# ParaGroup/WindFlow

Measured on AMD Instinct MI355X. Metric: tuples_per_sec, higher is better.
Workload: dtype bf16; 1 GPU; model=keyed_ffat_cb_window, global_batch=16777216, win=1000, slide=100, keys_per_rank=8192, parallelism=keyed-dp1, dense_keys=True

## Files before the change

csrc/engine/bindings.cpp:

```cpp
#include <pybind11/functional.h>
#include <pybind11/numpy.h>
#include <pybind11/pybind11.h>
#include <pybind11/stl.h>

#include "engine.hpp"

namespace py = pybind11;
using namespace wfa;

static py::array col_view(DType dt, void* data, int64_t n) {
    switch (dt) {
        case DType::I64: return py::array_t<int64_t>({n}, {8}, (int64_t*)data, py::none());
        case DType::F64: return py::array_t<double>({n}, {8}, (double*)data, py::none());
        case DType::F32: return py::array_t<float>({n}, {4}, (float*)data, py::none());
        case DType::U64: return py::array_t<uint64_t>({n}, {8}, (uint64_t*)data, py::none());
        case DType::I32: return py::array_t<int32_t>({n}, {4}, (int32_t*)data, py::none());
        case DType::U16: return py::array_t<uint16_t>({n}, {2}, (uint16_t*)data, py::none());
        case DType::U8: return py::array_t<uint8_t>({n}, {1}, (uint8_t*)data, py::none());
    }
    throw std::runtime_error("bad dtype");
}

static py::dict batch_views(Batch* b, RuntimeCtx* ctx = nullptr) {
    py::dict d;
// ... 439 lines not shown
        .value("I64", DType::I64)
        .value("F64", DType::F64)
        .value("F32", DType::F32)
        .value("U64", DType::U64)
        .value("I32", DType::I32)
        .value("U16", DType::U16)
        .value("U8", DType::U8);

    m.def("rccl_unique_id",
          [] { return py::bytes(wfa_rccl_unique_id()); },
          "ncclUniqueId bytes for Engine.set_dist (call on rank 0, broadcast)");

    py::class_<Engine>(m, "Engine")
        .def(py::init<>())
        .def_readwrite("mode", &Engine::mode)
        .def_readwrite("time_policy", &Engine::time_policy)
        .def_readwrite("queue_capacity", &Engine::queue_capacity)
        .def_readwrite("pin_threads", &Engine::pin_threads)
        .def("set_dist",
             [](Engine& e, int rank, int world, py::bytes id) {
                 e.dist_rank = rank;
                 e.dist_world = world;
                 e.rccl_id = std::string(id);
             },
             py::arg("rank"), py::arg("world"), py::arg("rccl_id"))
        .def("add_op",
             [](Engine& e, const std::string& name, int par, const std::string& kind,
                const std::string& spec, std::vector<double> fp, std::vector<int64_t> ip,
                std::vector<int> out_schema, int64_t out_batch, py::object pyfn,
                int device) {
                 OpSpec op;
                 op.id = (int)e.ops.size();
                 op.name = name;
                 op.parallelism = par;
                 op.device = device;
                 int id = op.id;
                 op.stages.push_back(make_stage(e, id, kind, spec, fp, ip, out_schema,
                                                out_batch, pyfn, device));
                 e.ops.push_back(std::move(op));
                 return id;
             },
             py::arg("name"), py::arg("parallelism"), py::arg("kind"), py::arg("spec") = "",
             py::arg("fparams") = std::vector<double>{}, py::arg("iparams") = std::vector<int64_t>{},
             py::arg("out_schema") = std::vector<int>{}, py::arg("out_batch") = 1024,
             py::arg("pyfn") = py::none(), py::arg("device") = -1)
        .def("chain_stage",
             [](Engine& e, int op_id, const std::string& kind, const std::string& spec,
                std::vector<double> fp, std::vector<int64_t> ip, std::vector<int> out_schema,
                int64_t out_batch, py::object pyfn) {
                 e.ops.at(op_id).stages.push_back(
                     make_stage(e, op_id, kind, spec, fp, ip, out_schema, out_batch, pyfn,
                                e.ops.at(op_id).device));
             },
             py::arg("op_id"), py::arg("kind"), py::arg("spec") = "",
             py::arg("fparams") = std::vector<double>{}, py::arg("iparams") = std::vector<int64_t>{},
             py::arg("out_schema") = std::vector<int>{}, py::arg("out_batch") = 1024,
             py::arg("pyfn") = py::none())
        .def("add_edge",
             [](Engine& e, int from, int to, Routing r, CollectorKind ck, int tag) {
                 e.edges.push_back(EdgeSpec{from, to, r, ck, tag});
             },
             py::arg("from_op"), py::arg("to_op"), py::arg("routing") = Routing::FORWARD,
             py::arg("collector") = CollectorKind::WATERMARK, py::arg("stream_tag") = -1)
        .def("run",
             [](Engine& e) {
                 e.build();
                 {
                     py::gil_scoped_release rel;
                     e.start();
                     e.wait();
                 }
             })
        .def("start",
             [](Engine& e) {
                 e.build();
                 e.start();
             })
        .def("start_gated",
             [](Engine& e) {
                 e.build();
                 {
                     py::gil_scoped_release rel;
                     e.start_gated();
                 }
             })
        .def("open_gate_and_wait",
             [](Engine& e) {
                 py::gil_scoped_release rel;
                 e.open_gate();
                 e.wait();
             })
        .def("wait",
             [](Engine& e) {
                 py::gil_scoped_release rel;
                 e.wait();
             })
        .def("abort_now", [](Engine& e) { e.abort.store(true); })
        .def("sink_sum", [](Engine& e, int op) { return e.sink_acc_i64.at(op).load(); })
        .def("sink_sum_f",
             [](Engine& e, int op) {
                 std::lock_guard<std::mutex> g(e.sink_f64_mu);
                 auto it = e.sink_acc_f64.find(op);
                 return it == e.sink_acc_f64.end() ? 0.0 : it->second;
             })
        .def("sink_count", [](Engine& e, int op) { return e.sink_tuples.at(op).load(); })
        .def("dropped", [](Engine& e) { return e.dropped_tuples.load(); })
        .def("sink_latencies",
             [](Engine& e, int op) {
                 auto it = e.sink_latencies.find(op);
                 return it == e.sink_latencies.end() ? std::vector<int64_t>{}
                                                     : it->second;
             })
        .def("stats", [](Engine& e) {
            py::list out;
            for (auto& r : e.replicas) {
                py::dict d;
                d["op"] = r->op_id;
                d["name"] = e.ops[r->op_id].name;
                d["replica"] = r->idx;
                d["inputs"] = r->stats.inputs_received;
                d["tuples_in"] = r->stats.tuples_received;
                d["outputs"] = r->stats.outputs_sent;
                d["tuples_out"] = r->stats.tuples_sent;
                d["svc_us_ewma"] = r->stats.service_time_us_ewma;
                d["start_us"] = r->stats.start_us;
                d["end_us"] = r->stats.end_us;
                d["kernels"] = r->stats.num_kernels;
                d["bytes_h2d"] = r->stats.bytes_h2d;
                d["bytes_d2h"] = r->stats.bytes_d2h;
                out.append(d);
            }
            return out;
        });

    m.def("hash_key", [](uint64_t k) { return KeyByEmitter::mix(k); });

#ifdef WFA_WITH_HIP
    m.def("debug_jit_fold_source",
          [](const std::string& kind, const std::string& spec,
             const std::vector<double>& fp, const std::vector<int64_t>& ip) {
              return debug_jit_fold_source(kind, spec, fp, ip);
          });
    m.def("debug_sort_pairs",
          [](py::array_t<uint32_t> keys, int bits) {
              auto r = debug_sort_pairs_host(keys.data(), keys.shape(0), bits);
              py::array_t<uint32_t> ks((py::ssize_t)r.first.size());
              py::array_t<uint32_t> vs((py::ssize_t)r.second.size());
              memcpy(ks.mutable_data(), r.first.data(), 4 * r.first.size());
              memcpy(vs.mutable_data(), r.second.data(), 4 * r.second.size());
              return py::make_tuple(ks, vs);
          });
    m.def("debug_ffat_stage_times",
          [](int64_t n, int64_t n_keys, int64_t win, int64_t slide, int iters,
             int vik, const std::string& fold_variant) {
              py::dict d;
              for (auto& [k, v] : debug_ffat_stage_times(n, n_keys, win, slide,
                                                         iters, vik, fold_variant))
                  d[py::str(k)] = v;
              return d;
          },
          py::arg("n"), py::arg("n_keys"), py::arg("win") = 1000,
          py::arg("slide") = 100, py::arg("iters") = 20, py::arg("vik") = 0,
          py::arg("fold_variant") = "");
    m.def("debug_tb_stage_times",
          [](int64_t n, int64_t n_keys, int iters, int mono) {
              std::map<std::string, double> m2;
              for (auto& kv : debug_tb_stage_times(n, n_keys, iters, mono))
                  m2[kv.first] = kv.second;
              return m2;
          },
          py::arg("n"), py::arg("n_keys"), py::arg("iters") = 20,
          py::arg("mono") = 1);
    m.def("debug_gram_stage_times",
          [](int64_t n, int64_t n_keys, int64_t win, int iters) {
              std::map<std::string, double> m2;
              for (auto& kv : debug_gram_stage_times(n, n_keys, win, iters))
                  m2[kv.first] = kv.second;
              return m2;
          },
          py::arg("n"), py::arg("n_keys"), py::arg("win") = 32,
          py::arg("iters") = 20);
    m.def("debug_a2a_stage_times",
          [](int64_t n, int64_t n_keys, int iters) {
              py::list out;
              for (auto& [k, v] : debug_a2a_stage_times(n, n_keys, iters))
                  out.append(py::make_tuple(k, v));
              return out;
          },
          py::arg("n"), py::arg("n_keys") = 8192, py::arg("iters") = 20);
    m.def("debug_key_slots",
          [](py::array_t<uint64_t> keys, int64_t max_keys) {
              auto r = debug_key_slots_host(keys.data(), keys.shape(0), max_keys);
              py::array_t<uint32_t> s((py::ssize_t)r.size());
              memcpy(s.mutable_data(), r.data(), 4 * r.size());
              return s;
          });
#endif

    struct StateStore {
        std::shared_ptr<void> holder;
        void* kv = nullptr;
        void* cache = nullptr;
    };
    py::class_<StateStore>(m, "StateStore")
        .def(py::init([](const std::string& path, int64_t cache_cap, bool fresh) {
                 auto s = new StateStore();
                 s->holder =
                     open_state_store(path, cache_cap, &s->kv, &s->cache, fresh);
                 return s;
             }),
             py::arg("path"), py::arg("cache_capacity") = 1 << 16,
             py::arg("fresh") = true)
        .def("erase",
             [](StateStore& s, uint64_t key) {
                 return state_kv_erase(s.kv, s.cache, key);
             })
        .def("get",
             [](StateStore& s, uint64_t key) -> py::object {
                 std::string* v = state_cache_get(s.cache, key);
                 if (!v) return py::none();
                 return py::bytes(*v);
             })
        .def("put",
             [](StateStore& s, uint64_t key, py::bytes val) {
                 state_cache_put(s.cache, key, std::string(val));
             })
        .def("flush", [](StateStore& s) { state_cache_flush(s.cache); })
        .def("__len__", [](StateStore& s) { return state_kv_size(s.kv); });
}
```

csrc/engine/engine.hpp:

```cpp
#pragma once

#include <chrono>
#include <deque>
#include <functional>
#include <thread>
#include <unordered_map>

#include "core.hpp"
#include "queue.hpp"

namespace wfa {

struct Engine;
struct Replica;

inline int64_t now_us() {
    return std::chrono::duration_cast<std::chrono::microseconds>(
               std::chrono::steady_clock::now().time_since_epoch())
        .count();
}

struct StatsRecord {
    int64_t inputs_received = 0;
    int64_t tuples_received = 0;
// ... 243 lines not shown
struct OpSpec {
    int id = 0;
    std::string name;
    int parallelism = 1;
    std::vector<StageSpec> stages;
    int device = -1;
    bool pinned_out = false;
    const StageSpec& last() const { return stages.back(); }
};

struct ChainLogic : OpLogic {
    struct StageEmitter;
    std::vector<std::shared_ptr<OpLogic>> stages;
    std::vector<EmitCtx> ctxs;
    std::vector<std::unique_ptr<Emitter>> glue;
    void wire(const std::vector<Pool*>& pools, EmitCtx& final_ctx, RuntimeCtx& rctx);
    bool is_source() const override { return stages.front()->is_source(); }
    bool accepts_device() const override { return stages.front()->accepts_device(); }
    bool source_step(EmitCtx&, RuntimeCtx& ctx) override {
        return stages.front()->source_step(ctxs[0], ctx);
    }
    void process(Batch* in, EmitCtx&, RuntimeCtx& ctx) override {
        stages.front()->process(in, ctxs[0], ctx);
    }
    bool on_punct(int64_t wm, EmitCtx&, RuntimeCtx& ctx) override;
    void on_eos(EmitCtx&, RuntimeCtx& ctx) override;
    void warm(RuntimeCtx& ctx) override;
    void post_eos() override {
        for (auto& st : stages) st->post_eos();
    }
};

struct EdgeSpec {
    int from = 0, to = 0;
    Routing routing = Routing::FORWARD;
    CollectorKind collector = CollectorKind::WATERMARK;
    int stream_tag = -1;
};

struct Replica {
    Engine* engine = nullptr;
    int op_id = 0;
    int idx = 0;
    std::shared_ptr<OpLogic> logic;
    std::unique_ptr<Collector> collector;
    std::vector<std::unique_ptr<Emitter>> emitters;
    EmitCtx ectx;
    RuntimeCtx rctx;
    StatsRecord stats;
    std::thread th;
    void run();
};

struct Engine {
    ExecMode mode = ExecMode::DEFAULT;
    TimePolicy time_policy = TimePolicy::EVENT_TIME;
    std::vector<OpSpec> ops;
    std::vector<EdgeSpec> edges;

    std::vector<std::unique_ptr<Replica>> replicas;
    std::vector<std::unique_ptr<Pool>> pools;
    std::vector<std::unique_ptr<SpscQueue>> queues;
    std::atomic<bool> abort{false};
    std::atomic<int64_t> dropped_tuples{0};
    std::mutex error_mu;
    std::string first_error;
    std::atomic<int> gate{0};
    std::atomic<int> warmed{0};
    bool use_gate = false;
    std::unordered_map<int, std::atomic<int64_t>> sink_acc_i64;
    std::unordered_map<int, double> sink_acc_f64;
    std::mutex sink_f64_mu;
    std::unordered_map<int, std::atomic<int64_t>> sink_tuples;
    std::unordered_map<int, std::vector<int64_t>> sink_latencies;
    int64_t queue_capacity = 128;
    bool pin_threads = false;
    int dist_rank = 0;
    int dist_world = 1;
    std::string rccl_id;

    Pool* make_pool(const Schema& s, int64_t cap, bool pinned) {
        pools.push_back(std::make_unique<Pool>(s, cap, pinned));
        return pools.back().get();
    }

    void build();
    void start();
    void wait();
    void run() { build(); start(); wait(); }
    void start_gated();
    void open_gate() { gate.store(1, std::memory_order_release); }
};

std::shared_ptr<OpLogic> make_native_logic(const std::string& kind,
                                           const std::string& spec,
                                           const std::vector<double>& fparams,
                                           const std::vector<int64_t>& iparams,
                                           Engine* eng, int op_id);

struct WinRows {
    int64_t n = 0;
    const int64_t* ts = nullptr;
    uint64_t key = 0;
    int64_t gwid = 0;
    const Schema* schema = nullptr;
    std::vector<const char*> cols;
};
using WindowFn = std::function<double(const WinRows&)>;

struct JoinPairs {
    int64_t n = 0;
    const uint64_t* key = nullptr;
    const int64_t* ts_a = nullptr;
    const int64_t* ts_b = nullptr;
    const double* va = nullptr;
    const double* vb = nullptr;
};
using JoinFn =
    std::function<void(const JoinPairs&, uint8_t* keep, double* out)>;

std::shared_ptr<OpLogic> make_window_logic(const std::string& kind,
                                           const std::vector<double>& fp,
                                           const std::vector<int64_t>& ip,
                                           Engine* eng, int op_id,
                                           WindowFn userfn = nullptr,
                                           JoinFn joinfn = nullptr);

std::shared_ptr<OpLogic> make_gpu_logic(const std::string& kind, const std::string& spec,
                                        const std::vector<double>& fp,
                                        const std::vector<int64_t>& ip, Engine* eng,
                                        int op_id, int device, const Schema& os,
                                        int64_t out_batch);

std::shared_ptr<OpLogic> make_persist_logic(const std::string& kind,
                                            const std::string& spec,
                                            const std::vector<double>& fp,
                                            const std::vector<int64_t>& ip,
                                            Engine* eng, int op_id);
std::shared_ptr<void> open_state_store(const std::string& path, int64_t cache_cap,
                                       void** kv_out, void** cache_out,
                                       bool fresh = true);
std::string* state_cache_get(void* cache, uint64_t key);
void state_cache_put(void* cache, uint64_t key, const std::string& v);
void state_cache_flush(void* cache);
int64_t state_kv_size(void* kv);
bool state_kv_erase(void* kv, void* cache, uint64_t key);

std::pair<std::vector<uint32_t>, std::vector<uint32_t>> debug_sort_pairs_host(
    const uint32_t* keys, int64_t n, int bits);
std::vector<uint32_t> debug_key_slots_host(const uint64_t* keys, int64_t n,
                                           int64_t max_keys);
std::vector<std::pair<std::string, double>> debug_ffat_stage_times(
    int64_t n, int64_t n_keys, int64_t win, int64_t slide, int iters, int vik,
    const std::string& fold_variant = "");
std::vector<std::pair<std::string, double>> debug_gram_stage_times(
    int64_t n, int64_t n_keys, int64_t win, int iters);
std::vector<std::pair<std::string, double>> debug_tb_stage_times(
    int64_t n, int64_t n_keys, int iters, int mono);
std::vector<std::pair<std::string, double>> debug_a2a_stage_times(
    int64_t n, int64_t n_keys, int iters);

std::string wfa_rccl_unique_id();

std::string debug_jit_fold_source(const std::string& kind,
                                  const std::string& spec,
                                  const std::vector<double>& fp,
                                  const std::vector<int64_t>& ip);

}
```

csrc/engine/gpu_common.hpp:

```cpp
#pragma once
#ifdef WFA_WITH_HIP

#include <hip/hip_runtime.h>
#include <hip/hiprtc.h>

#include <map>
#include <mutex>
#include <set>
#include <string>
#include <vector>

#include "engine.hpp"

namespace wfa {

#define HIPCHK(x)                                                                  \
    do {                                                                           \
        hipError_t err_ = (x);                                                     \
        if (err_ != hipSuccess)                                                    \
            throw std::runtime_error(std::string("HIP error: ") +                  \
                                     hipGetErrorString(err_) + " at " #x);         \
    } while (0)

#define RTCCHK(x)                                                              \
    do {                                                                       \
        hiprtcResult r_ = (x);                                                 \
        if (r_ != HIPRTC_SUCCESS)                                              \
            throw std::runtime_error(std::string("hiprtc error: ") +           \
                                     hiprtcGetErrorString(r_) + " at " #x);    \
    } while (0)

struct DeviceArena {
    std::mutex mu;
    std::map<size_t, std::vector<void*>> free_by_size;
    int device;
    size_t allocated = 0;

    void* get(size_t bytes) {
        bytes = (bytes + 255) & ~size_t(255);
        {
            std::lock_guard<std::mutex> g(mu);
            auto it = free_by_size.find(bytes);
            if (it != free_by_size.end() && !it->second.empty()) {
                void* p = it->second.back();
                it->second.pop_back();
                return p;
            }
        }
        void* p = nullptr;
        HIPCHK(hipSetDevice(device));
        HIPCHK(hipMalloc(&p, bytes));
        if (getenv("WFA_DEBUG_SYNC"))
            fprintf(stderr, "[alloc] %p..%p (%zu)\n", p, (char*)p + bytes,
                    bytes);
        std::lock_guard<std::mutex> g(mu);
        allocated += bytes;
        return p;
    }
    void put(void* p, size_t bytes) {
        bytes = (bytes + 255) & ~size_t(255);
        std::lock_guard<std::mutex> g(mu);
        free_by_size[bytes].push_back(p);
    }
};

inline DeviceArena g_arena[64];

inline DeviceArena& arena(int dev) {
    g_arena[dev].device = dev;
    return g_arena[dev];
}

inline bool wfa_prof() {
    static int v = -1;
    if (v < 0) v = getenv("WFA_PROF") ? 1 : 0;
    return v;
}

inline bool wfa_debug_sync() {
    static int v = -1;
    if (v < 0) v = getenv("WFA_DEBUG_SYNC") ? 1 : 0;
    return v;
}

inline void dbg_sync(hipStream_t s, const char* where) {
    if (!wfa_debug_sync()) return;
    hipError_t e = hipStreamSynchronize(s);
    hipError_t e2 = hipGetLastError();
    fprintf(stderr, "[dbgsync] %s sync=%s last=%s\n", where,
            hipGetErrorString(e), hipGetErrorString(e2));
    fflush(stderr);
}

struct GpuLogicBase : OpLogic {
    int64_t prof_host_us = 0, prof_calls = 0;
    int device = 0;
    hipStream_t stream = nullptr;
    std::unique_ptr<Pool> dev_pool;
    Schema out_schema;
    int64_t out_cap = 1 << 20;
    bool inited = false;

    virtual void init_device() {}
    void ensure_init() {
        if (inited) return;
        HIPCHK(hipSetDevice(device));
        HIPCHK(hipStreamCreateWithFlags(&stream, hipStreamNonBlocking));
        dev_pool = std::make_unique<Pool>(out_schema, out_cap, false);
        dev_pool->loc = Loc::DEVICE;
        dev_pool->device = device;
        init_device();
        inited = true;
    }
    void post_eos() override { drain_h2d(true); }
    ~GpuLogicBase() override {
        h2d_inflight.clear();
        if (stream) (void)hipStreamDestroy(stream);
    }

    void warm(RuntimeCtx&) override { ensure_init(); }
    bool accepts_device() const override { return true; }

    void wait_ready(Batch* b) {
        if (b->loc == Loc::DEVICE && b->ready_event)
            HIPCHK(hipStreamWaitEvent(stream, (hipEvent_t)b->ready_event, 0));
    }
    void record_ready(Batch* b) {
        b->stream = stream;
        HIPCHK(hipEventRecord((hipEvent_t)b->ready_event, stream));
    }

    void release_after_use(Batch* b) {
        if (b->loc == Loc::DEVICE && b->ready_event &&
            b->refcnt.load(std::memory_order_acquire) == 1)
            HIPCHK(hipEventRecord((hipEvent_t)b->ready_event, stream));
        release(b);
    }

    Batch* get_from(Pool& pool) {
        constexpr int MAX_DEPTH = 8;
        Batch* chosen = nullptr;
        Batch* skipped[MAX_DEPTH];
        int nskip = 0;
        while (nskip < MAX_DEPTH) {
            Batch* b = pool.try_pop();
            if (!b) break;
            if (!b->ready_event ||
                hipEventQuery((hipEvent_t)b->ready_event) == hipSuccess) {
                chosen = b;
                break;
            }
            skipped[nskip++] = b;
        }
        for (int i = 0; i < nskip; ++i) pool.put(skipped[i]);
        if (!chosen) {
            if (nskip > 0 && pool.live.load(std::memory_order_relaxed) >= MAX_DEPTH)
                chosen = pool.get();
            else
                chosen = pool.make_new();
        }
        if (chosen->ready_event)
            HIPCHK(hipStreamWaitEvent(stream, (hipEvent_t)chosen->ready_event, 0));
        return chosen;
    }

    Batch* get_dev() { return get_from(*dev_pool); }

    std::unique_ptr<Pool> in_pool;
    std::vector<std::unique_ptr<Pool>> retired_in_pools;

    Batch* get_in(const Batch* src) {
        if (!in_pool || in_pool->schema.payload != src->schema.payload ||
            in_pool->capacity < src->count) {
            if (in_pool) retired_in_pools.push_back(std::move(in_pool));
            in_pool = std::make_unique<Pool>(
                src->schema, std::max({out_cap, src->capacity, src->count}),
                false);
            in_pool->loc = Loc::DEVICE;
            in_pool->device = device;
        }
        return get_from(*in_pool);
    }

    std::deque<std::pair<Batch*, hipEvent_t>> h2d_inflight;

    void drain_h2d(bool block) {
        while (!h2d_inflight.empty()) {
            auto [old_hb, ev] = h2d_inflight.front();
            if (!block && hipEventQuery(ev) != hipSuccess) break;
            if (block) HIPCHK(hipEventSynchronize(ev));
            release(old_hb);
            h2d_inflight.pop_front();
        }
    }

    Batch* to_device(Batch* hb, RuntimeCtx& ctx) {
        drain_h2d(false);
        Batch* db = get_in(hb);
        int64_t n = hb->count;
        HIPCHK(hipMemcpyAsync(db->ts, hb->ts, 8 * n, hipMemcpyHostToDevice, stream));
        HIPCHK(hipMemcpyAsync(db->key, hb->key, 8 * n, hipMemcpyHostToDevice, stream));
        size_t bytes = 16 * n;
        for (size_t c = 0; c < hb->cols.size() && c < db->cols.size(); ++c) {
            size_t es = dsize(hb->schema.payload[c]);
            HIPCHK(hipMemcpyAsync(db->cols[c], hb->cols[c], es * n,
                                  hipMemcpyHostToDevice, stream));
            bytes += es * n;
        }
        db->count = n;
        db->watermark = ctx.current_wm;
        db->stream_tag = ctx.current_tag;
        db->ts_mono = hb->ts_mono;
        if (ctx.stats) ctx.stats->bytes_h2d += bytes;
        HIPCHK(hipEventRecord((hipEvent_t)db->ready_event, stream));
        h2d_inflight.push_back({hb, (hipEvent_t)db->ready_event});
        if (h2d_inflight.size() > 4) drain_h2d(true);
        return db;
    }

    Batch* input_on_device(Batch* b, RuntimeCtx& ctx) {
        if (b->loc == Loc::HOST) return to_device(b, ctx);
        gpu_resolve_count(b);
        if (b->device != device || force_peer_copy())
            return peer_copy(b, ctx);
        wait_ready(b);
        return b;
    }

    static bool force_peer_copy() {
        static int v = -1;
        if (v < 0) {
            const char* e = getenv("WFA_FORCE_PEER_COPY");
            v = (e && e[0] == '1') ? 1 : 0;
        }
        return v;
    }

    Batch* peer_copy(Batch* b, RuntimeCtx& ctx) {
        drain_h2d(false);
        enable_peer(device, b->device);
        wait_ready(b);
        Batch* db = get_in(b);
        const int64_t n = b->count;
        HIPCHK(hipMemcpyPeerAsync(db->ts, device, b->ts, b->device, 8 * n,
                                  stream));
        HIPCHK(hipMemcpyPeerAsync(db->key, device, b->key, b->device, 8 * n,
                                  stream));
        size_t bytes = 16 * n;
        for (size_t c = 0; c < b->cols.size() && c < db->cols.size(); ++c) {
            size_t es = dsize(b->schema.payload[c]);
            HIPCHK(hipMemcpyPeerAsync(db->cols[c], device, b->cols[c],
                                      b->device, es * n, stream));
            bytes += es * n;
        }
        db->count = n;
        db->watermark = b->watermark;
        db->stream_tag = b->stream_tag;
        db->born_us = b->born_us;
        if (ctx.stats) ctx.stats->bytes_d2h += bytes;
        HIPCHK(hipEventRecord((hipEvent_t)db->ready_event, stream));
        h2d_inflight.push_back({b, (hipEvent_t)db->ready_event});
        if (h2d_inflight.size() > 4) drain_h2d(true);
        return db;
    }

    static void enable_peer(int dst, int src) {
        if (dst == src) return;
        static std::mutex mu;
        static std::set<std::pair<int, int>> done;
        std::lock_guard<std::mutex> g(mu);
        if (!done.insert({dst, src}).second) return;
        int can = 0;
        if (hipDeviceCanAccessPeer(&can, dst, src) == hipSuccess && can) {
            HIPCHK(hipSetDevice(dst));
            hipError_t e = hipDeviceEnablePeerAccess(src, 0);
            if (e != hipSuccess && e != hipErrorPeerAccessAlreadyEnabled)
                (void)hipGetLastError();
        }
    }
};

struct KeyedScratch {
    uint64_t* tab = nullptr;
    uint32_t* d_nslots = nullptr;
    uint64_t* slot_to_key = nullptr;
    uint32_t *slot = nullptr, *idx = nullptr, *slot_t = nullptr, *idx_t = nullptr;
    uint32_t* hist = nullptr;
    uint32_t *seg_start = nullptr, *seg_slot = nullptr;
    int64_t* d_nseg = nullptr;
    float* v_sorted = nullptr;
    float* v_f32 = nullptr;
    int64_t table_cap = 0;
    int64_t max_keys = 0;
    int64_t cap = 0;
    int bits = 20;
    bool dense = false;
    uint32_t* d_overflow = nullptr;
    uint32_t* by_slot = nullptr;

    void alloc(int dev, int64_t cap_, int64_t mk, hipStream_t s);
    void check_dense_overflow();
    void segs(hipStream_t s, const uint32_t* slot_sorted, int64_t n, int shr);

    uint32_t* idx_sorted = nullptr;
    const void* v_as_f32 = nullptr;
    int v_dt = 2;

    void group(hipStream_t s, Batch* db, int vcol, RuntimeCtx& ctx,
               bool want_vik = false, bool want_carry = false);
};

hipModule_t jit_module(const std::string& src, int device);
hipFunction_t jit_fn(hipModule_t mod, const char* name);
std::string jit_type(DType d);

std::shared_ptr<OpLogic> make_gpu_jit_logic(const std::string& kind,
                                            const std::string& spec,
                                            const std::vector<double>& fp,
                                            const std::vector<int64_t>& ip,
                                            Engine* eng, int op_id, int device,
                                            const Schema& os, int64_t out_batch);

}

#endif
```

csrc/engine/gpu_ops.cpp:

```cpp
#include <cstring>
#include <deque>
#include <map>
#include <tuple>

#include "engine.hpp"

#ifdef WFA_WITH_HIP
#include <rccl/rccl.h>

#include "../hip/wfa_kernels.h"
#include "gpu_common.hpp"

namespace wfa {

struct AuxPool {
    std::mutex mu;
    std::vector<std::pair<void*, int64_t*>> free_list;
    std::pair<void*, int64_t*> get(int device) {
        {
            std::lock_guard<std::mutex> g(mu);
            if (!free_list.empty()) {
                auto p = free_list.back();
                free_list.pop_back();
                return p;
// ... 78 lines not shown
    c->watermark = b->watermark;
    c->stream_tag = b->stream_tag;
    c->born_us = b->born_us;
    c->ts_mono = b->ts_mono;
    c->stream = s;
    HIPCHK(hipEventRecord((hipEvent_t)c->ready_event, s));
    return c;
}

struct GpuSourceLogic : GpuLogicBase {
    int64_t len, n_keys, bsz;
    int vdt;
    uint64_t seed;
    int64_t pos = 0;
    GpuSourceLogic(int64_t l, int64_t k, int64_t b, int v, uint64_t sd, int dev,
                   Schema os) {
        len = l; n_keys = k; bsz = b; vdt = v; seed = sd;
        device = dev;
        out_schema = os;
        out_cap = b;
    }
    bool is_source() const override { return true; }
    bool source_step(EmitCtx& out, RuntimeCtx& ctx) override {
        int64_t t0 = now_us();
        ensure_init();
        if (pos >= len) return false;
        Batch* db = get_dev();
        int64_t tg = now_us() - t0;
        if (wfa_prof() && tg > 50)
            fprintf(stderr, "[prof] source get_dev wait %ld us\n", (long)tg);
        int64_t n = std::min<int64_t>(bsz, len - pos);
        wfa_gen_batch(stream, db->ts, db->key, db->cols[0], vdt, n, pos, seed, n_keys);
        dbg_sync(stream, "gen");
        db->count = n;
        db->ts_mono = true;
        db->born_us = now_us();
        pos += n;
        db->watermark = pos - 1;
        record_ready(db);
        if (ctx.stats) ctx.stats->num_kernels++;
        out.emit(db);
        return pos < len;
    }
};

struct GpuMapLogic : GpuLogicBase {
    int spec, col;
    double a, b;
    GpuMapLogic(int sp, int c, double a_, double b_, int dev, Schema os) {
        spec = sp; col = c; a = a_; b = b_;
        device = dev;
        out_schema = os;
    }
    void process(Batch* in, EmitCtx& out, RuntimeCtx& ctx) override {
        ensure_init();
        Batch* db = input_on_device(in, ctx);
        wfa_map_apply(stream, spec, db->cols[col], (int)db->schema.payload[col],
                      db->count, a, b);
        record_ready(db);
        if (ctx.stats) ctx.stats->num_kernels++;
        out.emit(db);
    }
};

struct GpuFilterLogic : GpuLogicBase {
    int spec, col;
    double a, b;
    uint32_t* d_flags = nullptr;
    uint32_t* d_scan = nullptr;
    int64_t* d_cnt = nullptr;
    void** d_colptrs = nullptr;
    int* d_esize = nullptr;
    GpuFilterLogic(int sp, int c, double a_, double b_, int dev, Schema os,
                   int64_t cap) {
        spec = sp; col = c; a = a_; b = b_;
        device = dev;
        out_schema = os;
        out_cap = cap;
    }
    void init_device() override {
        d_flags = (uint32_t*)arena(device).get(4 * out_cap);
        d_scan = (uint32_t*)arena(device).get(4 * (out_cap / 2048 + 2));
        d_cnt = (int64_t*)arena(device).get(64);
        size_t nc = out_schema.payload.size();
        d_colptrs = (void**)arena(device).get(16 * (nc + 1));
        d_esize = (int*)arena(device).get(4 * (nc + 1));
        std::vector<int> es;
        for (auto d : out_schema.payload) es.push_back((int)dsize(d));
        HIPCHK(hipMemcpy(d_esize, es.data(), 4 * nc, hipMemcpyHostToDevice));
    }
    void process(Batch* in, EmitCtx& out, RuntimeCtx& ctx) override {
        ensure_init();
        Batch* db = input_on_device(in, ctx);
        int64_t n = db->count;
        if (n > out_cap)
            throw std::runtime_error("filter input batch > out_batch capacity");
        Batch* ob = get_dev();
        wfa_filter_flags(stream, spec, db->cols[col], (int)db->schema.payload[col], n,
                         a, b, d_flags);
        size_t nc = db->cols.size();
        std::vector<void*> ptrs(2 * nc);
        for (size_t c = 0; c < nc; ++c) {
            ptrs[c] = db->cols[c];
            ptrs[nc + c] = ob->cols[c];
        }
        HIPCHK(hipMemcpyAsync(d_colptrs, ptrs.data(), 8 * 2 * nc,
                              hipMemcpyHostToDevice, stream));
        wfa_compact(stream, n, d_flags, d_scan, db->ts, ob->ts, db->key, ob->key,
                    (const void* const*)d_colptrs, (void* const*)(d_colptrs + nc),
                    d_esize, (int)nc, d_cnt);
        HIPCHK(hipMemcpyAsync(ob->lazy_count, d_cnt, 8, hipMemcpyDeviceToHost, stream));
        ob->count = -1;
        ob->watermark = db->watermark;
        ob->stream_tag = db->stream_tag;
        ob->born_us = db->born_us;
        ob->ts_mono = db->ts_mono;
        if (ctx.stats) ctx.stats->num_kernels += 3;
        release_after_use(db);
        record_ready(ob);
        out.emit(ob);
    }
};

void KeyedScratch::alloc(int dev, int64_t cap_, int64_t mk, hipStream_t s) {
    cap = cap_;
    max_keys = mk;
    table_cap = 1;
    while (table_cap < 2 * mk) table_cap <<= 1;
    bits = 1;
    while ((1ll << bits) < mk + 1) ++bits;
    if (bits < 5) bits = 5;
    auto& A = arena(dev);
    tab = (uint64_t*)A.get(16 * table_cap);
    d_nslots = (uint32_t*)A.get(64);
    slot_to_key = (uint64_t*)A.get(8 * mk);
    slot = (uint32_t*)A.get(4 * cap);
    idx = (uint32_t*)A.get(4 * cap);
    slot_t = (uint32_t*)A.get(4 * cap);
    idx_t = (uint32_t*)A.get(4 * cap);
    hist = (uint32_t*)A.get(4 * wfa_sort_hist_u32(cap));
    seg_start = (uint32_t*)A.get(4 * cap);
    seg_slot = (uint32_t*)A.get(4 * cap);
    d_nseg = (int64_t*)A.get(64);
    v_sorted = (float*)A.get(4 * cap);
    v_f32 = (float*)A.get(4 * cap);
    wfa_fill_u64(s, tab, ~0ULL, 2 * table_cap);
    wfa_fill_u32(s, d_nslots, 0, 1);
    if (dense) {
        d_overflow = (uint32_t*)A.get(64);
        wfa_fill_u32(s, d_overflow, 0, 1);
        wfa_iota_u64(s, slot_to_key, mk);
    }
    if (max_keys <= 65536) by_slot = (uint32_t*)A.get(4 * table_cap);
}

void KeyedScratch::segs(hipStream_t s, const uint32_t* slot_sorted, int64_t n,
                        int shr) {
    if (by_slot)
        wfa_segments_dense(s, slot_sorted, n, by_slot, table_cap, hist,
                           seg_start, seg_slot, d_nseg, shr);
    else
        wfa_segments(s, slot_sorted, n, hist, seg_start, seg_slot, d_nseg, shr);
}

void KeyedScratch::check_dense_overflow() {
    if (!dense) return;
    uint32_t ovf = 0;
    HIPCHK(hipMemcpy(&ovf, d_overflow, 4, hipMemcpyDeviceToHost));
    if (ovf)
        throw std::runtime_error(
            "withDenseKeys: a key >= max_keys arrived — dense mode requires "
            "integer keys in [0, max_keys); use the default hashed mode");
}

void KeyedScratch::group(hipStream_t s, Batch* db, int vcol, RuntimeCtx& ctx,
                         bool want_vik, bool want_carry) {
        int64_t n = db->count;
        if (n > cap)
            throw std::runtime_error("batch larger than keyed scratch capacity — "
                                     "set the GPU op's out_batch >= upstream batch");
        bool vik = want_vik && vcol >= 0 && max_keys <= 65535 &&
                   (int)db->schema.payload[vcol] == 5;
        if (vik) {
            uint32_t *os, *oi;
            if (dense) {
                wfa_key_dense_h(s, db->key, n, max_keys, slot, d_nslots,
                                d_overflow, (const uint16_t*)db->cols[vcol],
                                hist, 16);
                wfa_sort_pairs2_ph(s, slot, idx, slot_t, idx_t, nullptr,
                                   nullptr, hist, n, bits, &os, &oi, nullptr,
                                   1, 16);
            } else {
                wfa_key_to_slot_h(s, db->key, n, tab, d_nslots, table_cap, slot,
                                  slot_to_key, (const uint16_t*)db->cols[vcol],
                                  hist, 16);
                wfa_sort_pairs2_ph(s, slot, idx, slot_t, idx_t, nullptr,
                                   nullptr, hist, n, bits, &os, &oi, nullptr,
                                   1, 16);
            }
            idx_sorted = oi;
            v_as_f32 = os;
            v_dt = 6;
            segs(s, os, n, 16);
            if (ctx.stats) ctx.stats->num_kernels += 5 + 3 * ((bits + 3) / 4);
            return;
        }
        if (dense)
            wfa_key_dense_h(s, db->key, n, max_keys, slot, d_nslots, d_overflow,
                            nullptr, hist, 0);
        else
            wfa_key_to_slot_h(s, db->key, n, tab, d_nslots, table_cap, slot,
                              slot_to_key, nullptr, hist, 0);
        dbg_sync(s, "key_to_slot");
        if (want_carry && vcol >= 0 && (int)db->schema.payload[vcol] == 2) {
            wfa_cast(s, db->cols[vcol], 2, v_f32, 2, n);
            uint32_t *os, *oi, *ov;
            wfa_sort_pairs2_ph(s, slot, idx, slot_t, idx_t, (uint32_t*)v_f32,
                               (uint32_t*)v_sorted, hist, n, bits, &os, &oi,
                               &ov, 1, 0);
            idx_sorted = oi;
            v_as_f32 = ov;
            v_dt = 7;
            segs(s, os, n, 0);
            if (ctx.stats) ctx.stats->num_kernels += 6 + 3 * ((bits + 3) / 4);
            return;
        }
        uint32_t *os, *oi;
        wfa_sort_pairs2_ph(s, slot, idx, slot_t, idx_t, nullptr, nullptr,
                           hist, n, bits, &os, &oi, nullptr,
                           1, 0);
        idx_sorted = oi;
        if (vcol >= 0) {
            int vdt = (int)db->schema.payload[vcol];
            if (vdt == 2 || vdt == 5) {
                v_as_f32 = db->cols[vcol];
                v_dt = vdt;
            } else {
                wfa_cast(s, db->cols[vcol], vdt, v_f32, 2, n);
                v_as_f32 = v_f32;
                v_dt = 2;
            }
        }
        dbg_sync(s, "sort");
        segs(s, os, n, 0);
        dbg_sync(s, "segments");
        if (ctx.stats) ctx.stats->num_kernels += 5 + 3 * ((bits + 3) / 4);
}

hipModule_t jit_module(const std::string& src, int device) {
    static std::mutex mu;
    static std::map<std::string, hipModule_t> cache;
    std::lock_guard<std::mutex> g(mu);
    auto it = cache.find(src);
    if (it != cache.end()) return it->second;
    hiprtcProgram prog;
    RTCCHK(hiprtcCreateProgram(&prog, src.c_str(), "wfa_jit.hip", 0, nullptr,
                               nullptr));
    hipDeviceProp_t props;
    HIPCHK(hipGetDeviceProperties(&props, device));
    std::string arch = std::string("--offload-arch=") + props.gcnArchName;
    const char* opts[] = {arch.c_str(), "-O3"};
    hiprtcResult cr = hiprtcCompileProgram(prog, 2, opts);
    if (cr != HIPRTC_SUCCESS) {
        size_t lsz = 0;
        hiprtcGetProgramLogSize(prog, &lsz);
        std::string log(lsz, '\0');
        hiprtcGetProgramLog(prog, log.data());
        hiprtcDestroyProgram(&prog);
        throw std::runtime_error("JIT device logic failed to compile:\n" + log);
    }
    size_t csz = 0;
    RTCCHK(hiprtcGetCodeSize(prog, &csz));
    std::vector<char> code(csz);
    RTCCHK(hiprtcGetCode(prog, code.data()));
    hiprtcDestroyProgram(&prog);
    hipModule_t mod;
    HIPCHK(hipModuleLoadData(&mod, code.data()));
    cache[src] = mod;
    return mod;
}

hipFunction_t jit_fn(hipModule_t mod, const char* name) {
    hipFunction_t fn;
    HIPCHK(hipModuleGetFunction(&fn, mod, name));
    return fn;
}

std::string jit_type(DType d) {
    switch (d) {
        case DType::I64: return "long long";
        case DType::F64: return "double";
        case DType::F32: return "float";
        case DType::U64: return "unsigned long long";
        case DType::I32: return "int";
        default: throw std::runtime_error("jit: unsupported column dtype");
    }
}

struct JitKernel {
    hipModule_t mod = nullptr;
    hipFunction_t fn = nullptr;
};

static JitKernel jit_compile(const std::string& src, int device) {
    JitKernel k;
    k.mod = jit_module(src, device);
    k.fn = jit_fn(k.mod, "wfa_jit");
    return k;
}

static std::string jit_source(const std::string& expr, DType dt, bool filter) {
    std::string T = jit_type(dt);
    std::string body = filter
        ? "        flags[i] = (" + expr + ") ? 1u : 0u;\n"
        : "        v_[i] = (" + expr + ");\n";
    return "typedef long long i64; typedef unsigned long long u64;\n"
           "extern \"C\" __global__ void wfa_jit(" + T + "* v_, const i64* ts_,\n"
           "        const u64* key_, unsigned int* flags, i64 n) {\n"
           "    for (i64 i = blockIdx.x * (i64)blockDim.x + threadIdx.x; i < n;\n"
           "         i += gridDim.x * (i64)blockDim.x) {\n"
           "        " + T + " v = v_[i]; i64 ts = ts_[i]; u64 key = key_[i];\n"
           "        (void)v; (void)ts; (void)key;\n" + body +
           "    }\n}\n";
}

static void jit_launch(const JitKernel& k, hipStream_t stream, void* col,
                       const int64_t* ts, const uint64_t* key, uint32_t* flags,
                       int64_t n) {
    void* args[] = {&col, (void*)&ts, (void*)&key, &flags, &n};
    unsigned nb = (unsigned)std::min<int64_t>((n + 255) / 256, 2048);
    HIPCHK(hipModuleLaunchKernel(k.fn, nb, 1, 1, 256, 1, 1, 0, stream, args,
                                 nullptr));
}

struct GpuJitMapLogic : GpuLogicBase {
    std::string expr;
    int col;
    JitKernel k;
    GpuJitMapLogic(std::string e, int c, int dev, Schema os) : expr(std::move(e)), col(c) {
        device = dev;
        out_schema = os;
    }
    void init_device() override {
        k = jit_compile(jit_source(expr, out_schema.payload[col], false), device);
    }
    void process(Batch* in, EmitCtx& out, RuntimeCtx& ctx) override {
        ensure_init();
        Batch* db = input_on_device(in, ctx);
        jit_launch(k, stream, db->cols[col], db->ts, db->key, nullptr, db->count);
        record_ready(db);
        if (ctx.stats) ctx.stats->num_kernels++;
        out.emit(db);
    }
};

struct GpuJitFilterLogic : GpuLogicBase {
    std::string expr;
    int col;
    JitKernel k;
    uint32_t* d_flags = nullptr;
    uint32_t* d_scan = nullptr;
    int64_t* d_cnt = nullptr;
    void** d_colptrs = nullptr;
    int* d_esize = nullptr;
    GpuJitFilterLogic(std::string e, int c, int dev, Schema os, int64_t cap)
        : expr(std::move(e)), col(c) {
        device = dev;
        out_schema = os;
        out_cap = cap;
    }
    void init_device() override {
        k = jit_compile(jit_source(expr, out_schema.payload[col], true), device);
        auto& A = arena(device);
        d_flags = (uint32_t*)A.get(4 * out_cap);
        d_scan = (uint32_t*)A.get(4 * (out_cap / 2048 + 2));
        d_cnt = (int64_t*)A.get(64);
        size_t nc = out_schema.payload.size();
        d_colptrs = (void**)A.get(16 * (nc + 1));
        d_esize = (int*)A.get(4 * (nc + 1));
        std::vector<int> es;
        for (auto d : out_schema.payload) es.push_back((int)dsize(d));
        HIPCHK(hipMemcpy(d_esize, es.data(), 4 * nc, hipMemcpyHostToDevice));
    }
    void process(Batch* in, EmitCtx& out, RuntimeCtx& ctx) override {
        ensure_init();
        Batch* db = input_on_device(in, ctx);
        int64_t n = db->count;
        jit_launch(k, stream, db->cols[col], db->ts, db->key, d_flags, n);
        Batch* ob = get_dev();
        size_t nc = db->cols.size();
        std::vector<void*> ptrs(2 * nc);
        for (size_t c = 0; c < nc; ++c) {
            ptrs[c] = db->cols[c];
            ptrs[nc + c] = ob->cols[c];
        }
        HIPCHK(hipMemcpyAsync(d_colptrs, ptrs.data(), 8 * 2 * nc,
                              hipMemcpyHostToDevice, stream));
        wfa_compact(stream, n, d_flags, d_scan, db->ts, ob->ts, db->key, ob->key,
                    (const void* const*)d_colptrs, (void* const*)(d_colptrs + nc),
// ... 210 lines not shown
    int comb, vcol;
    int64_t win, slide, max_keys;
    bool use_tree;
    bool tb = false;
    int64_t lateness = 0;
    int pend_log2 = 16;
    int64_t pane_len, P, S;
    int ring_log2;
    KeyedScratch ks;
    int64_t* st_count = nullptr;
    uint32_t* st_fill = nullptr;
    float* st_acc = nullptr;
    float* ring_or_tree = nullptr;
    uint32_t* st_head = nullptr;
    float* st_wsum = nullptr;
    int64_t* st_last = nullptr;
    int64_t* d_on = nullptr;
    uint32_t* cb_nf = nullptr;
    uint32_t* pw_base = nullptr;
    float* pw_temp = nullptr;
    float* st_acc_new = nullptr;
    float* tb_pend = nullptr;
    int64_t* tb_base = nullptr;
    int64_t* tb_last = nullptr;
    uint32_t* tb_flags = nullptr;
    uint32_t* tb_nf = nullptr;
    uint32_t* tb_span_nf = nullptr;
    int64_t* tb_pfirst = nullptr;
    uint32_t* h_flags = nullptr;
    Engine* eng_ = nullptr;
    int64_t batches = 0;
    bool use_pane2 = false;
    int cb_fold_variant = WFA_CB_FOLD_TILE;
    static int cb_fold_from_env() {
        const char* e = getenv("WFA_CB_FOLD");
        return (e && !strcmp(e, "wave")) ? WFA_CB_FOLD_WAVE : WFA_CB_FOLD_TILE;
    }
    bool pane2_enabled() const {
        static int v = -1;
        if (v < 0) {
            const char* e = getenv("WFA_PANE2");
            v = e ? ((e[0] == '1') ? 1 : 0) : 2;
        }
        if (v == 2)
            return cb_fold_variant == WFA_CB_FOLD_WAVE && max_keys <= 4096;
        return v == 1;
    }

    GpuFfatLogic(int comb_, int vc, int64_t w, int64_t sl, int64_t mk, bool tree,
                 int dev, Schema os, int64_t cap, bool tb_, int64_t lat, int plog2,
                 bool dense = false) {
        ks.dense = dense;
        comb = comb_; vcol = vc; win = w; slide = sl; max_keys = mk; use_tree = tree;
        tb = tb_; lateness = lat;
        if (plog2 > 0) pend_log2 = plog2;
        device = dev;
        out_schema = os;
        out_cap = cap;
        pane_len = std::__gcd(win, slide);
        P = win / pane_len;
        S = slide / pane_len;
        ring_log2 = 1;
        while ((1ll << ring_log2) < P + 2) ++ring_log2;
        if (tb && use_tree) use_tree = false;
        cb_fold_variant = cb_fold_from_env();
    }
    void init_device() override {
        ks.alloc(device, out_cap, max_keys, stream);
        auto& A = arena(device);
        int64_t R = 1ll << ring_log2;
        st_count = (int64_t*)A.get(8 * max_keys);
        st_fill = (uint32_t*)A.get(4 * max_keys);
        st_acc = (float*)A.get(4 * max_keys);
        ring_or_tree = (float*)A.get(4 * max_keys * (use_tree ? 2 * R : R));
        st_head = (uint32_t*)A.get(4 * max_keys);
        st_wsum = (float*)A.get(4 * max_keys);
        st_last = (int64_t*)A.get(8 * max_keys);
        d_on = (int64_t*)A.get(64);
        HIPCHK(hipMemsetAsync(st_count, 0, 8 * max_keys, stream));
        HIPCHK(hipMemsetAsync(st_fill, 0, 4 * max_keys, stream));
        HIPCHK(hipMemsetAsync(st_head, 0, 4 * max_keys, stream));
        HIPCHK(hipMemsetAsync(st_wsum, 0, 4 * max_keys, stream));
        HIPCHK(hipMemsetAsync(st_last, 0, 8 * max_keys, stream));
        float ident = comb == 1 ? INFINITY : (comb == 2 ? -INFINITY : 0.f);
        wfa_fill_f32(stream, st_acc, ident, max_keys);
        wfa_fill_f32(stream, ring_or_tree, ident,
                     max_keys * (use_tree ? 2 * (1ll << ring_log2) : (1ll << ring_log2)));
        cb_nf = (uint32_t*)A.get(4 * (std::max(out_cap, max_keys) + 1));
        if (!tb && !use_tree && pane_len >= 32 && pane_wave_enabled()) {
            int64_t np = out_cap / pane_len + max_keys + 64;
            pw_base = (uint32_t*)A.get(4 * (np + 1));
            pw_temp = (float*)A.get(4 * (np + 1));
            st_acc_new = (float*)A.get(4 * max_keys);
        }
        use_pane2 = !tb && !use_tree && pane2_enabled() && pane_len >= 32;
        if (tb) {
            int64_t Rp = 1ll << pend_log2;
            tb_pend = (float*)A.get(4 * max_keys * Rp);
            tb_base = (int64_t*)A.get(8 * max_keys);
            tb_last = (int64_t*)A.get(8 * max_keys);
            tb_flags = (uint32_t*)A.get(64);
            tb_nf = (uint32_t*)A.get(4 * (max_keys + 1));
            if (max_keys <= 4096) {
                tb_span_nf = (uint32_t*)A.get(4 * (max_keys + 1));
                tb_pfirst = (int64_t*)A.get(8 * (max_keys + 1));
            }
            wfa_fill_f32(stream, tb_pend, ident, max_keys * Rp);
            wfa_fill_u64(stream, (uint64_t*)tb_base, (uint64_t)-1ll, max_keys);
            wfa_fill_u64(stream, (uint64_t*)tb_last, (uint64_t)-1ll, max_keys);
            HIPCHK(hipMemsetAsync(tb_flags, 0, 64, stream));
            HIPCHK(hipHostMalloc((void**)&h_flags, 64, hipHostMallocDefault));
        }
    }
    ~GpuFfatLogic() override {
        if (h_flags) (void)hipHostFree(h_flags);
        destroy_graphs();
    }

    uint32_t dropped_seen = 0;
    void check_tb_flags() {
        HIPCHK(hipMemcpyAsync(h_flags, tb_flags, 8, hipMemcpyDeviceToHost, stream));
        HIPCHK(hipStreamSynchronize(stream));
        if (h_flags[1])
            throw std::runtime_error(
                "gpu_ffat TB pending-pane ring overflow: raise pend_ring_log2 "
                "or lateness is too large for the configured ring");
        if (eng_ && h_flags[0] > dropped_seen) {
            eng_->dropped_tuples.fetch_add(h_flags[0] - dropped_seen,
                                           std::memory_order_relaxed);
            dropped_seen = h_flags[0];
        }
    }

    std::map<std::tuple<const void*, const void*, int64_t>, hipGraphExec_t> graphs;
    static bool graphs_enabled() {
        static int v = -1;
        if (v < 0) {
            const char* e = getenv("WFA_HIPGRAPH");
            v = (e && e[0] == '1') ? 1 : (getenv("WFA_NO_HIPGRAPH") ? 0 : 0);
        }
        return v;
    }

    static bool pane_wave_enabled() {
        static int v = -1;
        if (v < 0) {
            const char* e = getenv("WFA_PANE_WAVE");
            v = (e && e[0] == '1') ? 1 : 0;
        }
        return v;
    }

    void chain_cb(Batch* db, Batch* ob, int64_t n, RuntimeCtx& ctx) {
        ks.group(stream, db, vcol, ctx, !use_tree);
        uint32_t* nf = cb_nf;
        if (pw_base && !use_pane2) {
            wfa_ffat_fire_offsets_pw(stream, ks.seg_start, ks.seg_slot,
                                     ks.d_nseg, n, pane_len, P, S, st_fill,
                                     st_head, nf, d_on, ks.idx_sorted, db->ts,
                                     st_last, pw_base, d_on + 1);
            wfa_ffat_cb_fold_pw(stream, ks.seg_start, ks.seg_slot, ks.d_nseg,
                                d_on + 1, n, ks.v_as_f32, ks.v_dt,
                                ks.idx_sorted, db->ts, pane_len, P, S, comb,
                                ring_log2, st_count, st_fill, st_acc,
                                st_acc_new, ring_or_tree, st_head, st_wsum,
                                ks.slot_to_key, nf, pw_base, pw_temp, ob->key,
                                (float*)ob->cols[0], ob->ts, ob->capacity);
            HIPCHK(hipMemcpyAsync(ob->lazy_count, d_on, 8,
                                  hipMemcpyDeviceToHost, stream));
            return;
        }
        wfa_ffat_fire_offsets(stream, ks.seg_start, ks.seg_slot, ks.d_nseg, n,
                              pane_len, P, S, st_fill, st_head, nf, d_on,
                              ks.idx_sorted, db->ts, st_last);
        if (use_tree)
            wfa_ffat_tree_fold(stream, ks.seg_start, ks.seg_slot, ks.d_nseg, n,
                               ks.v_as_f32, ks.v_dt, ks.idx_sorted, db->ts, pane_len, P, S,
                               comb, ring_log2, st_count, st_fill, st_acc,
                               ring_or_tree, st_head, ks.slot_to_key, nf, ob->key,
                               (float*)ob->cols[0], ob->ts, ob->capacity);
        else if (use_pane2)
            wfa_ffat_cb_fold_fused(stream, ks.seg_start, ks.seg_slot, ks.d_nseg, n,
                                   ks.v_as_f32, ks.v_dt, ks.idx_sorted, db->ts,
                                   pane_len, P, S, comb, ring_log2, st_count,
                                   st_fill, st_acc, ring_or_tree, st_head, st_wsum,
                                   ks.slot_to_key, nf, ob->key,
                                   (float*)ob->cols[0], ob->ts, ob->capacity);
        else
            wfa_ffat_cb_fold(stream, ks.seg_start, ks.seg_slot, ks.d_nseg, n,
                             ks.v_as_f32, ks.v_dt, ks.idx_sorted, db->ts, pane_len, P, S,
                             comb, ring_log2, st_count, st_fill, st_acc,
                             ring_or_tree, st_head, st_wsum, ks.slot_to_key, nf,
                             ob->key, (float*)ob->cols[0], ob->ts, ob->capacity,
                             cb_fold_variant);
        HIPCHK(hipMemcpyAsync(ob->lazy_count, d_on, 8, hipMemcpyDeviceToHost, stream));
    }

    void process(Batch* in, EmitCtx& out, RuntimeCtx& ctx) override {
        ensure_init();
        Batch* db = input_on_device(in, ctx);
        int64_t n = db->count;
        if (tb) {
            ks.group(stream, db, vcol, ctx, true);
            wfa_seg_last_ts(stream, ks.seg_start, ks.seg_slot, ks.d_nseg, n,
                            ks.idx_sorted, db->ts, st_last);
            tb_round_with_count(db, n, db->watermark, out, ctx);
            release_after_use(db);
            return;
        }
        Batch* ob = get_dev();
        auto key = std::make_tuple((const void*)db->ts, (const void*)ob->ts, n);
        auto it = graphs.find(key);
        if (it != graphs.end()) {
            HIPCHK(hipGraphLaunch(it->second, stream));
            if (ctx.stats) ctx.stats->num_kernels += 1;
        } else if (graphs_enabled() && graphs.size() < 64) {
            HIPCHK(hipStreamBeginCapture(stream, hipStreamCaptureModeThreadLocal));
            chain_cb(db, ob, n, ctx);
            hipGraph_t graph;
            HIPCHK(hipStreamEndCapture(stream, &graph));
            hipGraphExec_t exec;
            HIPCHK(hipGraphInstantiate(&exec, graph, nullptr, nullptr, 0));
            HIPCHK(hipGraphDestroy(graph));
            graphs.emplace(key, exec);
            HIPCHK(hipGraphLaunch(exec, stream));
        } else {
            chain_cb(db, ob, n, ctx);
        }
        ob->count = -1;
        ob->watermark = db->watermark;
        ob->born_us = db->born_us;
        release_after_use(db);
        record_ready(ob);
        out.emit(ob);
        if ((++batches & 63) == 0) ks.check_dense_overflow();
    }
    void destroy_graphs() {
        for (auto& [k, e] : graphs) (void)hipGraphExecDestroy(e);
        graphs.clear();
    }

    void tb_round_with_count(Batch* db, int64_t n, int64_t wm, EmitCtx& out,
                             RuntimeCtx& ctx) {
        Batch* ob = get_dev();
        int64_t limit = (wm - lateness) / pane_len - 1;
        wfa_ffat_tb_round(stream, ks.seg_start, ks.seg_slot, ks.d_nseg, n,
                          ks.v_as_f32, ks.v_dt, ks.idx_sorted, db ? db->ts : nullptr,
                          pane_len, P, S, comb, ring_log2, pend_log2, limit,
                          tb_pend, tb_base, tb_last, st_head, st_wsum,
                          ring_or_tree, ks.d_nslots, ks.slot_to_key, tb_nf,
                          tb_flags, tb_flags + 1, ob->key, (float*)ob->cols[0],
                          ob->ts, ob->capacity, d_on,
                          db && db->ts_mono ? 1 : 0, tb_span_nf, tb_pfirst,
                          d_on + 1);
        HIPCHK(hipMemcpyAsync(ob->lazy_count, d_on, 8, hipMemcpyDeviceToHost, stream));
        ob->count = -1;
        ob->watermark = wm - lateness;
        if (ctx.stats) ctx.stats->num_kernels += 4;
        record_ready(ob);
        out.emit(ob);
        if ((++batches & 63) == 0) {
            check_tb_flags();
            ks.check_dense_overflow();
        }
    }

    bool on_punct(int64_t wm, EmitCtx& out, RuntimeCtx& ctx) override {
        if (!tb) return false;
        ensure_init();
        tb_round_with_count(nullptr, 0, wm, out, ctx);
        return false;
    }

    void on_eos(EmitCtx& out, RuntimeCtx& ctx) override {
        ensure_init();
        ks.check_dense_overflow();
        if (tb) {
            tb_round_with_count(nullptr, 0, INT64_MAX / 4, out, ctx);
            check_tb_flags();
            flush_open(nullptr, nullptr, out, ctx);
            return;
        }
        flush_open(st_fill, st_acc, out, ctx);
    }

    void flush_open(const uint32_t* fill, const float* acc, EmitCtx& out,
                    RuntimeCtx& ctx) {
        int64_t R = 1ll << ring_log2;
        wfa_cb_flush_count(stream, ks.d_nslots, P, S, fill, st_head, cb_nf);
        wfa_slot_scan(stream, cb_nf, ks.d_nslots, d_on);
        int64_t total = 0;
        HIPCHK(hipStreamSynchronize(stream));
        HIPCHK(hipMemcpy(&total, d_on, 8, hipMemcpyDeviceToHost));
        for (int64_t base = 0; base < total || base == 0; ) {
            Batch* ob = get_dev();
            int64_t page = std::min(total - base, ob->capacity);
            wfa_ffat_cb_flush_fire(stream, ks.d_nslots, P, S, comb, ring_log2,
                                   fill, acc, ring_or_tree,
                                   use_tree ? 2 * R : R, use_tree ? R : 0,
                                   st_head, st_last, ks.slot_to_key, cb_nf,
                                   base, ob->key, (float*)ob->cols[0], ob->ts,
                                   ob->capacity);
            ob->count = page < 0 ? 0 : page;
            ob->watermark = WM_MAX / 4;
            if (ctx.stats) ctx.stats->num_kernels += 1;
            record_ready(ob);
            out.emit(ob);
            base += ob->capacity;
            if (total == 0) break;
        }
        if (ctx.stats) ctx.stats->num_kernels += 2;
    }
};

struct GpuGramLogic : GpuLogicBase {
    int64_t win, max_keys;
    KeyedScratch ks;
    uint32_t* st_fill = nullptr;
    uint32_t* st_head = nullptr;
    float* st_acc = nullptr;
    uint32_t* nf = nullptr;
    int64_t* d_on = nullptr;
    const float** d_incols = nullptr;
    float** d_outcols = nullptr;
    uint32_t* d_inv = nullptr;
    float* d_staged = nullptr;
    int64_t staged_cap = 0;
// ... 351 lines not shown
                            size_t es = dsize(out_schema.payload[c]);
                            NCCLCHK(ncclRecv((char*)rb->cols[c] + es * roff[p], es * rc,
                                             ncclChar, p, comm, stream));
                        }
                    }
                }
                NCCLCHK(ncclGroupEnd());
            }
            if (send && send->ready_event)
                HIPCHK(hipEventRecord((hipEvent_t)send->ready_event, stream));
        }
        if (ctx.stats) ctx.stats->num_kernels++;
        int64_t out_wm = min_wm == WM_MAX ? cur_wm : min_wm;
        if (rb) {
            if (total > 0) {
                rb->count = total;
                rb->watermark = out_wm;
                record_ready(rb);
                out.emit(rb);
            } else {
                release(rb);
                for (auto* e : out.emitters) e->punct(out_wm);
            }
        } else if (out_wm > cur_wm) {
            for (auto* e : out.emitters) e->punct(out_wm);
        }
        cur_wm = std::max(cur_wm, out_wm);
        return all_done;
    }

    void process(Batch* in, EmitCtx& out, RuntimeCtx& ctx) override {
        int64_t t0 = now_us();
        ensure_init();
        Batch* db = input_on_device(in, ctx);
        int64_t n = db->count;
        int64_t wm = db->watermark;
        if (n > out_cap) throw std::runtime_error("exchange input > out_batch");
        if (world == 1 && !getenv("WFA_XCHG_NO_SELFPASS")) {
            cur_wm = std::max(cur_wm, wm);
            out.emit(db);
            return;
        }
        Batch* sb = send_pool->get();
        int64_t t1 = now_us();
        if (sb->ready_event)
            HIPCHK(hipStreamWaitEvent(stream, (hipEvent_t)sb->ready_event, 0));
        uint32_t* dest = dest2[dest_flip];
        uint32_t* hi = dest_flip ? hist_b : hist;
        hipEvent_t ev_free = ev_dest[dest_flip];
        dest_flip ^= 1;
        if (db->ready_event)
            HIPCHK(hipStreamWaitEvent(meta_stream, (hipEvent_t)db->ready_event, 0));
        HIPCHK(hipStreamWaitEvent(meta_stream, ev_free, 0));
        wfa_bucket_by_key_h(meta_stream, db->key, n, world, dest, hi);
        wfa_count_u32(meta_stream, dest, n, d_counts, world);
        HIPCHK(hipEventRecord(ev_counts, meta_stream));
        start_meta(true, wm, false);
        Meta m = sync_meta(true);
        if (m.remote_in == 0 && m.remote_out == 0 &&
            !getenv("WFA_XCHG_NO_SELFPASS")) {
            release(sb);
            int64_t out_wm = m.min_wm == WM_MAX ? cur_wm : m.min_wm;
            cur_wm = std::max(cur_wm, out_wm);
            db->watermark = out_wm;
            if (ctx.stats) ctx.stats->num_kernels += 3;
            out.emit(db);
            if (wfa_prof())
                fprintf(stderr, "[prof] xchg n=%ld self-forward meta=%ld us\n",
                        (long)n, (long)(now_us() - t1));
            return;
        }
        HIPCHK(hipStreamWaitEvent(stream, ev_counts, 0));
        uint32_t *od, *oi;
        wfa_sort_pairs2_ph(stream, dest, idx, dest_t, idx_t, nullptr, nullptr,
                           hi, n, bits, &od, &oi, nullptr, 1,
                           0);
        HIPCHK(hipEventRecord(ev_free, stream));
        size_t nc = db->cols.size();
        std::vector<void*> ptrs(2 * nc);
        for (size_t c = 0; c < nc; ++c) {
            ptrs[c] = db->cols[c];
            ptrs[nc + c] = sb->cols[c];
        }
        HIPCHK(hipMemcpyAsync(d_colptrs, ptrs.data(), 8 * 2 * nc,
                              hipMemcpyHostToDevice, stream));
        wfa_gather_rows(stream, oi, n, db->ts, sb->ts, db->key, sb->key,
                        (const void* const*)d_colptrs, (void* const*)(d_colptrs + nc),
                        d_esize, (int)nc);
        release_after_use(db);
        if (ctx.stats) ctx.stats->num_kernels += 4;
        int64_t t2 = now_us();
        round(sb, out, ctx);
        release(sb);
        if (wfa_prof())
            fprintf(stderr, "[prof] xchg n=%ld in+get=%ld us bucket=%ld us round=%ld us\n",
                    (long)n, (long)(t1 - t0), (long)(t2 - t1), (long)(now_us() - t2));
    }

    bool on_punct(int64_t, EmitCtx&, RuntimeCtx&) override { return true; }

    void on_eos(EmitCtx& out, RuntimeCtx& ctx) override {
        ensure_init();
        if (world == 1 && !getenv("WFA_XCHG_NO_SELFPASS")) return;
        for (;;) {
            start_meta(false, cur_wm, true);
            if (round(nullptr, out, ctx)) break;
        }
    }
};

std::pair<std::vector<uint32_t>, std::vector<uint32_t>> debug_sort_pairs_host(
    const uint32_t* keys, int64_t n, int bits) {
    HIPCHK(hipSetDevice(0));
    auto& A = arena(0);
    uint32_t* d_k = (uint32_t*)A.get(4 * n);
    uint32_t* d_v = (uint32_t*)A.get(4 * n);
    uint32_t* d_kt = (uint32_t*)A.get(4 * n);
    uint32_t* d_vt = (uint32_t*)A.get(4 * n);
    uint32_t* d_h = (uint32_t*)A.get(4 * wfa_sort_hist_u32(n));
    HIPCHK(hipMemcpy(d_k, keys, 4 * n, hipMemcpyHostToDevice));
    wfa_iota_u32(nullptr, d_v, n);
    uint32_t *ok, *ov;
    wfa_sort_pairs(nullptr, d_k, d_v, d_kt, d_vt, d_h, n, bits, &ok, &ov);
    std::vector<uint32_t> hk(n), hv(n);
    HIPCHK(hipMemcpy(hk.data(), ok, 4 * n, hipMemcpyDeviceToHost));
    HIPCHK(hipMemcpy(hv.data(), ov, 4 * n, hipMemcpyDeviceToHost));
    A.put(d_k, 4 * n); A.put(d_v, 4 * n); A.put(d_kt, 4 * n); A.put(d_vt, 4 * n);
    A.put(d_h, 4 * wfa_sort_hist_u32(n));
    return {std::move(hk), std::move(hv)};
}

std::vector<uint32_t> debug_key_slots_host(const uint64_t* keys, int64_t n,
                                           int64_t max_keys) {
    HIPCHK(hipSetDevice(0));
    auto& A = arena(0);
    int64_t cap = 1;
    while (cap < 2 * max_keys) cap <<= 1;
    uint64_t* d_key = (uint64_t*)A.get(8 * n);
    uint64_t* d_tab = (uint64_t*)A.get(16 * cap);
    uint32_t* d_ns = (uint32_t*)A.get(64);
    uint32_t* d_out = (uint32_t*)A.get(4 * n);
    uint64_t* d_s2k = (uint64_t*)A.get(8 * max_keys);
    HIPCHK(hipMemcpy(d_key, keys, 8 * n, hipMemcpyHostToDevice));
    wfa_fill_u64(nullptr, d_tab, ~0ULL, 2 * cap);
    wfa_fill_u32(nullptr, d_ns, 0, 1);
    wfa_key_to_slot(nullptr, d_key, n, d_tab, d_ns, cap, d_out, d_s2k);
    std::vector<uint32_t> out(n);
    HIPCHK(hipMemcpy(out.data(), d_out, 4 * n, hipMemcpyDeviceToHost));
    A.put(d_key, 8 * n); A.put(d_tab, 16 * cap);
    A.put(d_ns, 64); A.put(d_out, 4 * n); A.put(d_s2k, 8 * max_keys);
    return out;
}

std::shared_ptr<OpLogic> make_gpu_logic(const std::string& kind, const std::string& spec,
                                        const std::vector<double>& fp,
                                        const std::vector<int64_t>& ip, Engine* eng,
                                        int op_id, int device, const Schema& os,
                                        int64_t out_batch) {
    if (kind == "gpu_source")
        return std::make_shared<GpuSourceLogic>(ip[0], ip[1], ip[2], (int)ip[3],
                                                (uint64_t)ip[4], device, os);
    if (kind == "gpu_map")
        return std::make_shared<GpuMapLogic>((int)ip[0], (int)ip[1], fp[0], fp[1],
                                             device, os);
    if (kind == "gpu_filter")
        return std::make_shared<GpuFilterLogic>((int)ip[0], (int)ip[1], fp[0], fp[1],
                                                device, os, out_batch);
    if (kind == "gpu_jit_map")
        return std::make_shared<GpuJitMapLogic>(spec, (int)(ip.empty() ? 0 : ip[0]),
                                                device, os);
    if (kind == "gpu_jit_filter")
        return std::make_shared<GpuJitFilterLogic>(spec, (int)(ip.empty() ? 0 : ip[0]),
                                                   device, os, out_batch);
    if (kind == "gpu_jit_reduce" || kind == "gpu_jit_ffat" ||
        kind == "gpu_jit_stateful" || kind == "gpu_split")
        return make_gpu_jit_logic(kind, spec, fp, ip, eng, op_id, device, os,
                                  out_batch);
    if (kind == "gpu_map_keyed")
        return std::make_shared<GpuStatefulMapLogic>((int)ip[0], (int)ip[1], fp[0],
                                                     fp[1], ip[2], device, os,
                                                     out_batch);
    if (kind == "gpu_filter_keyed")
        return std::make_shared<GpuStatefulFilterLogic>((int)ip[0], (int)ip[1], fp[0],
                                                        fp[1], ip[2], device, os,
                                                        out_batch);
    if (kind == "gpu_reduce_all")
        return std::make_shared<GpuReduceAllLogic>((int)ip[0], (int)ip[1], device,
                                                   os, out_batch);
    if (kind == "gpu_reduce")
        return std::make_shared<GpuReduceLogic>((int)ip[0], (int)ip[1], ip[2], device,
                                                os, out_batch,
                                                ip.size() > 3 && ip[3] != 0);
    if (kind == "gpu_ffat") {
        auto l = std::make_shared<GpuFfatLogic>(
            (int)ip[0], (int)ip[1], ip[2], ip[3], ip[4], ip[5] != 0, device, os,
            out_batch, ip.size() > 6 && ip[6] != 0, ip.size() > 7 ? ip[7] : 0,
            ip.size() > 8 ? (int)ip[8] : 0, ip.size() > 9 && ip[9] != 0);
        l->eng_ = eng;
        return l;
    }
    if (kind == "gpu_gram") {
        auto l = std::make_shared<GpuGramLogic>(ip[0], ip[1], device, os,
                                                out_batch);
        l->ks.dense = ip.size() > 2 && ip[2] != 0;
        return l;
    }
    if (kind == "gpu_exchange")
        return std::make_shared<GpuExchangeLogic>(eng, device, os, out_batch);
    if (kind == "gpu_to_host")
        return std::make_shared<GpuToHostLogic>(device);
    if (kind == "gpu_count_sink") {
        eng->sink_acc_i64[op_id].store(0);
        eng->sink_tuples[op_id].store(0);
        return std::make_shared<GpuCountSink>(eng, op_id, device);
    }
    throw std::runtime_error("unknown gpu logic: " + kind);
}

std::vector<std::pair<std::string, double>> debug_a2a_stage_times(
    int64_t n, int64_t n_keys, int iters) {
    HIPCHK(hipSetDevice(0));
    hipStream_t s = nullptr;
    auto& A = arena(0);
    int world = 1;
    Schema sch;
    sch.payload.push_back(DType::F32);
    int64_t* d_ts = (int64_t*)A.get(8 * n);
    uint64_t* d_key = (uint64_t*)A.get(8 * n);
    float* d_val = (float*)A.get(4 * n);
    int64_t* o_ts = (int64_t*)A.get(8 * n);
    uint64_t* o_key = (uint64_t*)A.get(8 * n);
    float* o_val = (float*)A.get(4 * n);
    int64_t* r_ts = (int64_t*)A.get(8 * n);
    uint64_t* r_key = (uint64_t*)A.get(8 * n);
    float* r_val = (float*)A.get(4 * n);
    uint32_t* dest = (uint32_t*)A.get(4 * n);
    uint32_t* idx = (uint32_t*)A.get(4 * n);
    uint32_t* dest_t = (uint32_t*)A.get(4 * n);
    uint32_t* idx_t = (uint32_t*)A.get(4 * n);
    uint32_t* hist = (uint32_t*)A.get(4 * wfa_sort_hist_u32(n));
    uint32_t* d_counts = (uint32_t*)A.get(64);
    int64_t* d_meta = (int64_t*)A.get(8 * 3);
    int64_t* h_meta = nullptr;
    HIPCHK(hipHostMalloc((void**)&h_meta, 64, hipHostMallocDefault));
    void** d_colptrs = (void**)A.get(64);
    int* d_esize = (int*)A.get(64);
    {
        int es = 4;
        HIPCHK(hipMemcpy(d_esize, &es, 4, hipMemcpyHostToDevice));
        void* ptrs[2] = {d_val, o_val};
        HIPCHK(hipMemcpy(d_colptrs, ptrs, 16, hipMemcpyHostToDevice));
    }
    KeyedScratch ks;
    ks.alloc(0, n, 4 * n_keys, s);
    uint64_t* rk = (uint64_t*)A.get(8 * n);
    float* rv = (float*)A.get(4 * n);
    int64_t* rt = (int64_t*)A.get(8 * n);
    int64_t* d_on = (int64_t*)A.get(64);
    wfa_gen_batch(s, d_ts, d_key, d_val, 2, n, 0, 42, n_keys);

    constexpr int NS = 11;
    const char* names[NS] = {"gen",        "map",    "bucket", "count",
                             "sort_dest",  "gather", "selfD2D", "meta_d2h",
                             "key_to_slot", "sort_slot+seg", "seg_reduce"};
    hipEvent_t ev[NS + 1];
    for (auto& e : ev) HIPCHK(hipEventCreate(&e));
    double acc[NS] = {0};
    for (int it = -2; it < iters; ++it) {
        HIPCHK(hipEventRecord(ev[0], s));
        wfa_gen_batch(s, d_ts, d_key, d_val, 2, n, (int64_t)it * n, 42, n_keys);
        HIPCHK(hipEventRecord(ev[1], s));
        wfa_map_apply(s, 2, d_val, 2, n, 2.0, 0.5);
        HIPCHK(hipEventRecord(ev[2], s));
        wfa_bucket_by_key(s, d_key, n, world, dest);
        HIPCHK(hipEventRecord(ev[3], s));
        wfa_count_u32(s, dest, n, d_counts, world);
        HIPCHK(hipEventRecord(ev[4], s));
        uint32_t *od, *oi;
        wfa_sort_pairs2(s, dest, idx, dest_t, idx_t, nullptr, nullptr, hist, n,
                        1, &od, &oi, nullptr, 1, 0);
        HIPCHK(hipEventRecord(ev[5], s));
        const void* ci[1] = {d_val};
        void* co[1] = {o_val};
        (void)ci; (void)co;
        wfa_gather_rows(s, oi, n, d_ts, o_ts, d_key, o_key,
                        (const void* const*)d_colptrs,
                        (void* const*)(d_colptrs + 1), d_esize, 1);
        HIPCHK(hipEventRecord(ev[6], s));
        HIPCHK(hipMemcpyAsync(r_ts, o_ts, 8 * n, hipMemcpyDeviceToDevice, s));
        HIPCHK(hipMemcpyAsync(r_key, o_key, 8 * n, hipMemcpyDeviceToDevice, s));
        HIPCHK(hipMemcpyAsync(r_val, o_val, 4 * n, hipMemcpyDeviceToDevice, s));
        HIPCHK(hipEventRecord(ev[7], s));
        wfa_pack_meta(s, d_counts, world, 123, 0, d_meta);
        HIPCHK(hipMemcpyAsync(h_meta, d_meta, 24, hipMemcpyDeviceToHost, s));
        HIPCHK(hipEventRecord(ev[8], s));
        wfa_key_to_slot(s, r_key, n, ks.tab, ks.d_nslots, ks.table_cap, ks.slot,
                        ks.slot_to_key);
        HIPCHK(hipEventRecord(ev[9], s));
        uint32_t *os2, *oi2, *ov2;
        wfa_cast(s, r_val, 2, ks.v_f32, 2, n);
        wfa_sort_pairs2(s, ks.slot, ks.idx, ks.slot_t, ks.idx_t,
                        (uint32_t*)ks.v_f32, (uint32_t*)ks.v_sorted, ks.hist, n,
                        ks.bits, &os2, &oi2, &ov2, 1, 0);
        ks.segs(s, os2, n, 0);
        HIPCHK(hipEventRecord(ev[10], s));
        wfa_segment_reduce_wave(s, ks.seg_start, ks.seg_slot, ks.d_nseg, n,
                                ov2, 7, oi2, r_ts, 0, 1,
                                ks.slot_to_key, rk, rv, rt, d_on);
        HIPCHK(hipEventRecord(ev[11], s));
        HIPCHK(hipStreamSynchronize(s));
        if (it >= 0)
            for (int k = 0; k < NS; ++k) {
                float ms = 0;
                HIPCHK(hipEventElapsedTime(&ms, ev[k], ev[k + 1]));
                acc[k] += ms * 1000.0;
            }
    }
    for (auto& e : ev) (void)hipEventDestroy(e);
    (void)hipHostFree(h_meta);
    std::vector<std::pair<std::string, double>> out;
    for (int k = 0; k < NS; ++k) out.push_back({names[k], acc[k] / iters});
    return out;
}

std::vector<std::pair<std::string, double>> debug_ffat_stage_times(
    int64_t n, int64_t n_keys, int64_t win, int64_t slide, int iters, int vik,
    const std::string& fold_variant) {
    int variant;
    if (fold_variant.empty() || fold_variant == "tile") variant = WFA_CB_FOLD_TILE;
    else if (fold_variant == "wave") variant = WFA_CB_FOLD_WAVE;
    else if (fold_variant == "tile512") variant = WFA_CB_FOLD_TILE512;
    else if (fold_variant == "tile2048") variant = WFA_CB_FOLD_TILE2048;
    else throw std::runtime_error("debug_ffat_stage_times: unknown fold_variant '" +
                                  fold_variant + "' (wave|tile|tile512|tile2048)");
    HIPCHK(hipSetDevice(0));
    hipStream_t s = nullptr;
    KeyedScratch ks;
    ks.alloc(0, n, n_keys, s);
    auto& A = arena(0);
    uint64_t* d_key = (uint64_t*)A.get(8 * n);
    int64_t* d_ts = (int64_t*)A.get(8 * n);
    uint16_t* d_val = (uint16_t*)A.get(2 * n);
    {
        std::vector<uint64_t> hk(n);
        std::vector<int64_t> ht(n);
        std::vector<uint16_t> hv(n, 0x3f80);
        uint64_t x = 0x12345;
        for (int64_t i = 0; i < n; ++i) {
            x = x * 6364136223846793005ULL + 1442695040888963407ULL;
            hk[i] = (x >> 33) % (uint64_t)n_keys;
            ht[i] = i;
        }
        HIPCHK(hipMemcpy(d_key, hk.data(), 8 * n, hipMemcpyHostToDevice));
        HIPCHK(hipMemcpy(d_ts, ht.data(), 8 * n, hipMemcpyHostToDevice));
        HIPCHK(hipMemcpy(d_val, hv.data(), 2 * n, hipMemcpyHostToDevice));
    }
    int64_t pane = std::__gcd(win, slide), P = win / pane, S = slide / pane;
    int ring_log2 = 1;
    while ((1ll << ring_log2) < P + 2) ++ring_log2;
    int64_t R = 1ll << ring_log2;
    int64_t fires_cap = n / slide + n_keys + 64;
    int64_t* st_count = (int64_t*)A.get(8 * n_keys);
    uint32_t* st_fill = (uint32_t*)A.get(4 * n_keys);
    float* st_acc = (float*)A.get(4 * n_keys);
    float* ring = (float*)A.get(4 * n_keys * R);
    uint32_t* st_head = (uint32_t*)A.get(4 * n_keys);
    float* st_wsum = (float*)A.get(4 * n_keys);
    uint32_t* nf = (uint32_t*)A.get(4 * (fires_cap + 1));
    uint64_t* o_key = (uint64_t*)A.get(8 * fires_cap);
    float* o_val = (float*)A.get(4 * fires_cap);
    int64_t* o_ts = (int64_t*)A.get(8 * fires_cap);
    int64_t* d_on = (int64_t*)A.get(64);
    HIPCHK(hipMemsetAsync(st_count, 0, 8 * n_keys, s));
    HIPCHK(hipMemsetAsync(st_fill, 0, 4 * n_keys, s));
    HIPCHK(hipMemsetAsync(st_head, 0, 4 * n_keys, s));
    HIPCHK(hipMemsetAsync(st_wsum, 0, 4 * n_keys, s));
    wfa_fill_f32(s, st_acc, 0.f, n_keys);
    wfa_fill_f32(s, ring, 0.f, n_keys * R);

    constexpr int NS = 5;
    const char* names[NS] = {"key_to_slot", "radix_sort", "segments",
                             "fire_offsets", "fold"};
    hipEvent_t ev[NS + 1];
    for (auto& e : ev) HIPCHK(hipEventCreate(&e));
    double acc[NS] = {0};
    for (int it = -2; it < iters; ++it) {
        HIPCHK(hipEventRecord(ev[0], s));
        if (vik)
            wfa_key_to_slot_v(s, d_key, n, ks.tab, ks.d_nslots, ks.table_cap,
                              ks.slot, ks.slot_to_key, d_val);
        else
            wfa_key_to_slot(s, d_key, n, ks.tab, ks.d_nslots, ks.table_cap, ks.slot,
                            ks.slot_to_key);
        HIPCHK(hipEventRecord(ev[1], s));
        uint32_t *os_, *oi;
        wfa_sort_pairs2(s, ks.slot, ks.idx, ks.slot_t, ks.idx_t, nullptr, nullptr,
                        ks.hist, n, ks.bits, &os_, &oi, nullptr, 1, vik ? 16 : 0);
        HIPCHK(hipEventRecord(ev[2], s));
        ks.segs(s, os_, n, vik ? 16 : 0);
        HIPCHK(hipEventRecord(ev[3], s));
        wfa_ffat_fire_offsets(s, ks.seg_start, ks.seg_slot, ks.d_nseg, n, pane, P,
                              S, st_fill, st_head, nf, d_on, nullptr, nullptr,
                              nullptr);
        HIPCHK(hipEventRecord(ev[4], s));
        wfa_ffat_cb_fold(s, ks.seg_start, ks.seg_slot, ks.d_nseg, n,
                         vik ? (const void*)os_ : (const void*)d_val, vik ? 6 : 5,
                         oi, d_ts, pane, P, S, 0, ring_log2, st_count, st_fill,
                         st_acc, ring, st_head, st_wsum, ks.slot_to_key, nf, o_key,
                         o_val, o_ts, fires_cap, variant);
        HIPCHK(hipEventRecord(ev[5], s));
        HIPCHK(hipStreamSynchronize(s));
        if (it >= 0)
            for (int k = 0; k < NS; ++k) {
                float ms = 0;
                HIPCHK(hipEventElapsedTime(&ms, ev[k], ev[k + 1]));
                acc[k] += ms * 1000.0;
            }
    }
    for (auto& e : ev) (void)hipEventDestroy(e);
    std::vector<std::pair<std::string, double>> out;
    for (int k = 0; k < NS; ++k) out.push_back({names[k], acc[k] / iters});
    return out;
}

std::vector<std::pair<std::string, double>> debug_tb_stage_times(
    int64_t n, int64_t n_keys, int iters, int mono) {
    HIPCHK(hipSetDevice(0));
    hipStream_t s = nullptr;
    KeyedScratch ks;
    ks.alloc(0, n, n_keys, s);
    auto& A = arena(0);
    uint64_t* d_key = (uint64_t*)A.get(8 * n);
    int64_t* d_ts = (int64_t*)A.get(8 * n);
    uint16_t* d_val = (uint16_t*)A.get(2 * n);
    wfa_gen_batch(s, d_ts, d_key, d_val, 5, n, 0, 42, n_keys);
    const int64_t pane = 100 * n_keys, P = 10, S = 1;
    int ring_log2 = 5, pend_log2 = 18;
    int64_t R = 1ll << ring_log2;
    int64_t fires_cap = n / pane + n_keys + 64;
    float* pend = (float*)A.get(4 * n_keys * (1ll << pend_log2));
    int64_t* pend_base = (int64_t*)A.get(8 * n_keys);
    int64_t* last_pane = (int64_t*)A.get(8 * n_keys);
    uint32_t* st_head = (uint32_t*)A.get(4 * n_keys);
    float* st_wsum = (float*)A.get(4 * n_keys);
    float* ring = (float*)A.get(4 * n_keys * R);
    uint32_t* nf = (uint32_t*)A.get(4 * (n_keys + 1));
    uint32_t* flags = (uint32_t*)A.get(64);
    uint64_t* o_key = (uint64_t*)A.get(8 * fires_cap);
    float* o_val = (float*)A.get(4 * fires_cap);
    int64_t* o_ts = (int64_t*)A.get(8 * fires_cap);
    int64_t* d_on = (int64_t*)A.get(64);
    wfa_fill_f32(s, pend, 0.f, n_keys * (1ll << pend_log2));
    wfa_fill_f32(s, ring, 0.f, n_keys * R);
    wfa_fill_f32(s, st_wsum, 0.f, n_keys);
    wfa_fill_u64(s, (uint64_t*)pend_base, (uint64_t)-1ll, n_keys);
    wfa_fill_u64(s, (uint64_t*)last_pane, (uint64_t)-1ll, n_keys);
    HIPCHK(hipMemsetAsync(st_head, 0, 4 * n_keys, s));
    HIPCHK(hipMemsetAsync(flags, 0, 64, s));

    constexpr int NS = 4;
    const char* names[NS] = {"group", "lift", "count_scan", "advance"};
    hipEvent_t ev[NS + 1];
    for (auto& e : ev) HIPCHK(hipEventCreate(&e));
    double acc[NS] = {0};
    RuntimeCtx rctx;
    for (int it = -2; it < iters; ++it) {
        wfa_gen_batch(s, d_ts, d_key, d_val, 5, n, (int64_t)(it + 2) * n, 42,
                      n_keys);
        HIPCHK(hipEventRecord(ev[0], s));
        wfa_key_to_slot(s, d_key, n, ks.tab, ks.d_nslots, ks.table_cap,
                        ks.slot, ks.slot_to_key);
        uint32_t *os_, *oi;
        wfa_sort_pairs2(s, ks.slot, ks.idx, ks.slot_t, ks.idx_t, nullptr,
                        nullptr, ks.hist, n, ks.bits, &os_, &oi, nullptr, 1, 0);
        ks.segs(s, os_, n, 0);
        HIPCHK(hipEventRecord(ev[1], s));
        wfa_tb_lift_only(s, ks.seg_start, ks.seg_slot, ks.d_nseg, n, d_val, 5,
                         oi, d_ts, pane, P, S, 0, pend_log2, pend, pend_base,
                         last_pane, flags, flags + 1, mono);
        HIPCHK(hipEventRecord(ev[2], s));
        int64_t limit = ((int64_t)(it + 3) * n) / pane - 1;
        wfa_tb_countscan_only(s, ks.d_nslots, limit, pend_base, last_pane,
                              st_head, P, S, nf, d_on);
        HIPCHK(hipEventRecord(ev[3], s));
        wfa_tb_advance_only(s, ks.d_nslots, limit, pane, P, S, 0, ring_log2,
                            pend_log2, pend, pend_base, last_pane, st_head,
                            st_wsum, ring, ks.slot_to_key, nf, o_key, o_val,
                            o_ts, fires_cap);
        HIPCHK(hipEventRecord(ev[4], s));
        HIPCHK(hipStreamSynchronize(s));
        if (it >= 0)
            for (int k = 0; k < NS; ++k) {
                float ms = 0;
                HIPCHK(hipEventElapsedTime(&ms, ev[k], ev[k + 1]));
                acc[k] += ms * 1000.0;
            }
    }
    for (auto& e : ev) (void)hipEventDestroy(e);
    std::vector<std::pair<std::string, double>> out;
    for (int k = 0; k < NS; ++k) out.push_back({names[k], acc[k] / iters});
    return out;
}

std::vector<std::pair<std::string, double>> debug_gram_stage_times(
    int64_t n, int64_t n_keys, int64_t win, int iters) {
    HIPCHK(hipSetDevice(0));
    hipStream_t s = nullptr;
    KeyedScratch ks;
    ks.alloc(0, n, n_keys, s);
    auto& A = arena(0);
    uint64_t* d_key = (uint64_t*)A.get(8 * n);
    int64_t* d_ts = (int64_t*)A.get(8 * n);
    float* d_cols[16];
    for (int c = 0; c < 16; ++c) {
        d_cols[c] = (float*)A.get(4 * n);
        wfa_gen_batch(s, d_ts, d_key, d_cols[c], 2, n, 0, 1000 + c, n_keys);
    }
    int64_t fires16 = (n / std::max<int64_t>(win, 1) + n_keys + 64) * 16;
    uint32_t* st_fill = (uint32_t*)A.get(4 * n_keys);
    uint32_t* st_head = (uint32_t*)A.get(4 * n_keys);
    float* st_acc = (float*)A.get(4 * n_keys * 256);
    uint32_t* nf = (uint32_t*)A.get(4 * (fires16 + 1));
    uint64_t* o_key = (uint64_t*)A.get(8 * fires16);
    int64_t* o_gwid = (int64_t*)A.get(8 * fires16);
    int64_t* o_ts = (int64_t*)A.get(8 * fires16);
    float* o_cols[16];
    for (int c = 0; c < 16; ++c) o_cols[c] = (float*)A.get(4 * fires16);
    int64_t* d_on = (int64_t*)A.get(64);
    uint32_t* d_inv = (uint32_t*)A.get(4 * n);
    float* d_staged = (float*)A.get(64 * n);
    const float** d_in = (const float**)A.get(16 * 8);
    float** d_out = (float**)A.get(16 * 8);
    HIPCHK(hipMemcpyAsync(d_in, d_cols, 16 * 8, hipMemcpyHostToDevice, s));
    HIPCHK(hipMemcpyAsync(d_out, o_cols, 16 * 8, hipMemcpyHostToDevice, s));
    HIPCHK(hipMemsetAsync(st_fill, 0, 4 * n_keys, s));
    HIPCHK(hipMemsetAsync(st_head, 0, 4 * n_keys, s));
    HIPCHK(hipMemsetAsync(st_acc, 0, 4 * n_keys * 256, s));

    constexpr int NS = 5;
    const char* names[NS] = {"group", "fire_offsets", "stage_rows", "mfma_fold",
                             "gflops"};
    hipEvent_t ev[NS];
    for (auto& e : ev) HIPCHK(hipEventCreate(&e));
    double acc[NS] = {0};
    RuntimeCtx rctx;
    for (int it = -2; it < iters; ++it) {
        HIPCHK(hipEventRecord(ev[0], s));
        wfa_key_to_slot(s, d_key, n, ks.tab, ks.d_nslots, ks.table_cap,
                        ks.slot, ks.slot_to_key);
        uint32_t *os_, *oi;
        wfa_sort_pairs2(s, ks.slot, ks.idx, ks.slot_t, ks.idx_t, nullptr,
                        nullptr, ks.hist, n, ks.bits, &os_, &oi, nullptr, 1, 0);
        ks.segs(s, os_, n, 0);
        HIPCHK(hipEventRecord(ev[1], s));
        wfa_ffat_fire_offsets(s, ks.seg_start, ks.seg_slot, ks.d_nseg, n, win,
                              1, 1, st_fill, st_head, nf, d_on, nullptr,
                              nullptr, nullptr);
        HIPCHK(hipEventRecord(ev[2], s));
        wfa_gram_prep(s, d_in, oi, n, d_inv, d_staged);
        HIPCHK(hipEventRecord(ev[3], s));
        wfa_gram_fold(s, ks.seg_start, ks.seg_slot, ks.d_nseg, n, d_in, oi,
                      d_ts, win, st_fill, st_acc, st_head, ks.slot_to_key, nf,
                      o_key, o_gwid, d_out, o_ts, fires16, d_on, d_inv,
                      d_staged);
        HIPCHK(hipEventRecord(ev[4], s));
        HIPCHK(hipStreamSynchronize(s));
        if (it >= 0)
            for (int k = 0; k < NS - 1; ++k) {
                float ms = 0;
                HIPCHK(hipEventElapsedTime(&ms, ev[k], ev[k + 1]));
                acc[k] += ms * 1000.0;
            }
    }
    for (auto& e : ev) (void)hipEventDestroy(e);
    std::vector<std::pair<std::string, double>> out;
    for (int k = 0; k < NS - 1; ++k) out.push_back({names[k], acc[k] / iters});
    double fold_us = acc[3] / iters;
    out.push_back({"gflops", fold_us > 0 ? (512.0 * n) / (fold_us * 1e3) : 0});
    return out;
}

}

#else

namespace wfa {
Batch* gpu_alloc_batch(Pool&) { throw std::runtime_error("built without HIP"); }
void gpu_free_batch(Batch*) {}
void gpu_resolve_count(Batch*) {}
Batch* gpu_clone_batch(Batch*) { throw std::runtime_error("built without HIP"); }
std::string wfa_rccl_unique_id() { throw std::runtime_error("built without HIP"); }
std::pair<std::vector<uint32_t>, std::vector<uint32_t>> debug_sort_pairs_host(
    const uint32_t*, int64_t, int) {
    throw std::runtime_error("built without HIP");
}
std::vector<uint32_t> debug_key_slots_host(const uint64_t*, int64_t, int64_t) {
    throw std::runtime_error("built without HIP");
}
std::vector<std::pair<std::string, double>> debug_ffat_stage_times(int64_t, int64_t,
                                                                   int64_t, int64_t,
                                                                   int, int,
                                                                   const std::string&) {
    throw std::runtime_error("built without HIP");
}
std::vector<std::pair<std::string, double>> debug_a2a_stage_times(int64_t, int64_t,
                                                                  int) {
    throw std::runtime_error("built without HIP");
}
std::vector<std::pair<std::string, double>> debug_gram_stage_times(int64_t,
                                                                   int64_t,
                                                                   int64_t,
                                                                   int) {
    throw std::runtime_error("built without HIP");
}
std::vector<std::pair<std::string, double>> debug_tb_stage_times(int64_t,
                                                                 int64_t, int,
                                                                 int) {
    throw std::runtime_error("built without HIP");
}
std::shared_ptr<OpLogic> make_gpu_logic(const std::string&, const std::string&,
                                        const std::vector<double>&,
                                        const std::vector<int64_t>&, Engine*, int, int,
                                        const Schema&, int64_t) {
    throw std::runtime_error("built without HIP");
}
}

#endif
```

csrc/hip/sortwin.hip:

```cpp
#include <hip/hip_runtime.h>

#include <cstdio>
#include <cstdlib>

#include "wfa_kernels.h"

static int wfa_sort_dbg() {
    static int v = -1;
    if (v < 0) v = getenv("WFA_DEBUG_SYNC") ? 1 : 0;
    return v;
}
static void sdbg(hipStream_t st, const char* what, int pass) {
    if (!wfa_sort_dbg()) return;
    hipError_t e = hipStreamSynchronize(st);
    hipError_t e2 = hipGetLastError();
    fprintf(stderr, "[sortdbg] p%d %s sync=%s last=%s\n", pass, what,
            hipGetErrorString(e), hipGetErrorString(e2));
    fflush(stderr);
}

#define WFA_THREADS 256
#define WFA_MAX_BLOCKS 2048
#define RS_IPT 8
#define RS_PER_BLOCK (WFA_THREADS * RS_IPT)
// ... 319 lines not shown
                                uint64_t* table_packed, uint32_t* n_slots,
                                int64_t table_cap, uint32_t* slot_out,
                                uint64_t* slot_to_key) {
    hipLaunchKernelGGL(k_key_to_slot, dim3(nblk(n)), dim3(WFA_THREADS), 0,
                       (hipStream_t)s, key, n, table_packed, n_slots,
                       table_cap, slot_out, slot_to_key);
}

extern "C" int64_t wfa_sort_nblocks(int64_t n) {
    return (n + RS_PER_BLOCK - 1) / RS_PER_BLOCK;
}

extern "C" int64_t wfa_sort_hist_u32(int64_t cap) {
    int64_t nb4 = (cap + RS_PER_BLOCK - 1) / RS_PER_BLOCK;
    int64_t nb8 = (cap + RS8_PER_BLOCK - 1) / RS8_PER_BLOCK;
    int64_t a = 16 * nb4 + 16;
    int64_t b = 256 * nb8 + 512;
    return (a > b ? a : b) + 64;
}

__global__ void k_rs_hist(const uint32_t* keys, int64_t n, int shift, uint32_t* hist,
                          int64_t nblocks) {
    __shared__ uint32_t h[16];
    if (threadIdx.x < 16) h[threadIdx.x] = 0;
    __syncthreads();
    int64_t base = (int64_t)blockIdx.x * RS_PER_BLOCK + (int64_t)threadIdx.x * RS_IPT;
#pragma unroll
    for (int j = 0; j < RS_IPT; ++j) {
        int64_t i = base + j;
        if (i < n) atomicAdd(&h[(keys[i] >> shift) & 15], 1u);
    }
    __syncthreads();
    if (threadIdx.x < 16) hist[(int64_t)threadIdx.x * nblocks + blockIdx.x] = h[threadIdx.x];
}

__global__ void k_rs_scan16(uint32_t* hist, int64_t nblocks, uint32_t* dt) {
    uint32_t* a = hist + (int64_t)blockIdx.x * nblocks;
    __shared__ uint32_t tot[256];
    const int64_t chunk = (nblocks + 255) / 256;
    const int64_t b0 = (int64_t)threadIdx.x * chunk;
    const int64_t b1 = min(nblocks, b0 + chunk);
    uint32_t s = 0;
    for (int64_t i = b0; i < b1; ++i) s += a[i];
    tot[threadIdx.x] = s;
    __syncthreads();
    for (int off = 1; off < 256; off <<= 1) {
        uint32_t t = (threadIdx.x >= off) ? tot[threadIdx.x - off] : 0;
        __syncthreads();
        tot[threadIdx.x] += t;
        __syncthreads();
    }
    uint32_t run = tot[threadIdx.x] - s;
    for (int64_t i = b0; i < b1; ++i) {
        uint32_t v = a[i];
        a[i] = run;
        run += v;
    }
    if (threadIdx.x == 255) dt[blockIdx.x] = tot[255];
}

__global__ void k_rs_scan(uint32_t* a, int64_t m) {
    __shared__ uint32_t tot[1024];
    const int64_t chunk = (m + 1023) / 1024;
    const int64_t b0 = (int64_t)threadIdx.x * chunk;
    const int64_t b1 = min(m, b0 + chunk);
    uint32_t s = 0;
    for (int64_t i = b0; i < b1; ++i) s += a[i];
    tot[threadIdx.x] = s;
    __syncthreads();
    for (int off = 1; off < 1024; off <<= 1) {
        uint32_t t = (threadIdx.x >= off) ? tot[threadIdx.x - off] : 0;
        __syncthreads();
        tot[threadIdx.x] += t;
        __syncthreads();
    }
    uint32_t run = tot[threadIdx.x] - s;
    for (int64_t i = b0; i < b1; ++i) {
        uint32_t v = a[i];
        a[i] = run;
        run += v;
    }
}

__global__ void k_rs_scatter(const uint32_t* keys, const uint32_t* vals, int64_t n,
                             int shift, const uint32_t* hist, int64_t nblocks,
                             const uint32_t* dt, uint32_t* keys_out,
                             uint32_t* vals_out, const uint32_t* vals2,
                             uint32_t* vals2_out) {
    __shared__ uint32_t tc[WFA_THREADS][17];
    __shared__ uint32_t gbase[16];
    __shared__ uint32_t dbase[16];
    if (threadIdx.x == 0) {
        uint32_t run = 0;
        for (int d = 0; d < 16; ++d) {
            dbase[d] = run;
            run += dt[d];
        }
    }
    int64_t base = (int64_t)blockIdx.x * RS_PER_BLOCK + (int64_t)threadIdx.x * RS_IPT;
    uint32_t k_[RS_IPT];
    uint32_t v_[RS_IPT];
    uint32_t v2_[RS_IPT];
    int cnt_local[16];
#pragma unroll
    for (int d = 0; d < 16; ++d) cnt_local[d] = 0;
    int nit = 0;
#pragma unroll
    for (int j = 0; j < RS_IPT; ++j) {
        int64_t i = base + j;
        if (i < n) {
            k_[j] = keys[i];
            v_[j] = vals ? vals[i] : (uint32_t)i;
            if (vals2) v2_[j] = vals2[i];
            cnt_local[(k_[j] >> shift) & 15]++;
            nit = j + 1;
        }
    }
#pragma unroll
    for (int d = 0; d < 16; ++d) tc[threadIdx.x][d] = cnt_local[d];
    if (threadIdx.x < 16)
        gbase[threadIdx.x] = hist[(int64_t)threadIdx.x * nblocks + blockIdx.x];
    __syncthreads();
    if (threadIdx.x < 16) gbase[threadIdx.x] += dbase[threadIdx.x];
    __syncthreads();
    for (int off = 1; off < WFA_THREADS; off <<= 1) {
        uint32_t t[16];
#pragma unroll
        for (int d = 0; d < 16; ++d)
            t[d] = (threadIdx.x >= off) ? tc[threadIdx.x - off][d] : 0;
        __syncthreads();
#pragma unroll
        for (int d = 0; d < 16; ++d) tc[threadIdx.x][d] += t[d];
        __syncthreads();
    }
    uint32_t pre[16];
#pragma unroll
    for (int d = 0; d < 16; ++d) pre[d] = tc[threadIdx.x][d] - cnt_local[d];
    for (int j = 0; j < nit; ++j) {
        uint32_t d = (k_[j] >> shift) & 15;
        uint32_t own = 0;
        for (int j2 = 0; j2 < j; ++j2) own += (((k_[j2] >> shift) & 15) == d);
        uint32_t pos = gbase[d] + pre[d] + own;
        keys_out[pos] = k_[j];
        vals_out[pos] = v_[j];
        if (vals2) vals2_out[pos] = v2_[j];
    }
}


extern "C" int64_t wfa_sort8_nblocks(int64_t n) {
    return (n + RS8_PER_BLOCK - 1) / RS8_PER_BLOCK;
}

__global__ void k_rs8_hist(const uint32_t* keys, int64_t n, int shift,
                           uint32_t* hist, int64_t nblocks) {
    __shared__ uint32_t h[WFA_THREADS / 64][256];
    const int wave = threadIdx.x >> 6, lane = threadIdx.x & 63;
    for (int d = threadIdx.x; d < 256; d += blockDim.x)
        for (int w = 0; w < WFA_THREADS / 64; ++w) h[w][d] = 0;
    __syncthreads();
    int64_t waveBase = (int64_t)blockIdx.x * RS8_PER_BLOCK + wave * RS8_PER_WAVE;
#pragma unroll
    for (int j = 0; j < RS8_IPT; ++j) {
        int64_t i = waveBase + j * 64 + lane;
        if (i < n) atomicAdd(&h[wave][(keys[i] >> shift) & 255], 1u);
    }
    __syncthreads();
    for (int d = threadIdx.x; d < 256; d += blockDim.x) {
        uint32_t t = 0;
        for (int w = 0; w < WFA_THREADS / 64; ++w) t += h[w][d];
        hist[(int64_t)d * nblocks + blockIdx.x] = t;
    }
}

__global__ void k_rs8_scan(uint32_t* hist, int64_t nblocks, uint32_t* dt) {
    uint32_t* a = hist + (int64_t)blockIdx.x * nblocks;
    __shared__ uint32_t tot[256];
    const int64_t chunk = (nblocks + 255) / 256;
    const int64_t b0 = (int64_t)threadIdx.x * chunk;
    const int64_t b1 = min(nblocks, b0 + chunk);
    uint32_t s = 0;
    for (int64_t i = b0; i < b1; ++i) s += a[i];
    tot[threadIdx.x] = s;
    __syncthreads();
    for (int off = 1; off < 256; off <<= 1) {
        uint32_t t = (threadIdx.x >= off) ? tot[threadIdx.x - off] : 0;
        __syncthreads();
        tot[threadIdx.x] += t;
        __syncthreads();
    }
    uint32_t run = tot[threadIdx.x] - s;
    for (int64_t i = b0; i < b1; ++i) {
        uint32_t v = a[i];
        a[i] = run;
        run += v;
    }
    if (threadIdx.x == 255) dt[blockIdx.x] = tot[255];
}

__global__ void k_rs8_dbase(const uint32_t* dt, uint32_t* dbase) {
    __shared__ uint32_t tot[256];
    tot[threadIdx.x] = dt[threadIdx.x];
    __syncthreads();
    for (int off = 1; off < 256; off <<= 1) {
        uint32_t t = (threadIdx.x >= off) ? tot[threadIdx.x - off] : 0;
        __syncthreads();
        tot[threadIdx.x] += t;
        __syncthreads();
    }
    dbase[threadIdx.x] = tot[threadIdx.x] - dt[threadIdx.x];
}

__global__ void k_rs8_scatter(const uint32_t* keys, const uint32_t* vals,
                              int64_t n, int shift, const uint32_t* hist,
                              int64_t nblocks, const uint32_t* dbase,
                              uint32_t* keys_out, uint32_t* vals_out,
                              const uint32_t* vals2, uint32_t* vals2_out) {
    __shared__ uint32_t gbase[256];
    __shared__ uint32_t waveCnt[WFA_THREADS / 64][256];
    __shared__ uint32_t wavePre[WFA_THREADS / 64][256];
    const int wave = threadIdx.x >> 6, lane = threadIdx.x & 63;
    const uint64_t lt = ((uint64_t)1 << lane) - 1;
    for (int d = threadIdx.x; d < 256; d += blockDim.x) {
        gbase[d] = hist[(int64_t)d * nblocks + blockIdx.x] + dbase[d];
        for (int w = 0; w < WFA_THREADS / 64; ++w) waveCnt[w][d] = 0;
    }
    __syncthreads();
    int64_t waveBase = (int64_t)blockIdx.x * RS8_PER_BLOCK + wave * RS8_PER_WAVE;
    uint32_t mk[RS8_IPT], mv[RS8_IPT], mr[RS8_IPT];
    uint32_t mv2[RS8_IPT];
    int nit = 0;
#pragma unroll
    for (int j = 0; j < RS8_IPT; ++j) {
        int64_t i = waveBase + j * 64 + lane;
        bool valid = i < n;
        uint32_t k = valid ? keys[i] : 0;
        uint32_t v = valid ? (vals ? vals[i] : (uint32_t)i) : 0;
        uint32_t d = (k >> shift) & 255;
        uint64_t mask = __ballot(valid);
#pragma unroll
        for (int bit = 0; bit < 8; ++bit) {
            uint64_t b = __ballot((d >> bit) & 1);
            mask &= ((d >> bit) & 1) ? b : ~b;
        }
        if (valid) {
            uint32_t pre = waveCnt[wave][d];
            uint32_t rank = pre + (uint32_t)__popcll(mask & lt);
            mk[j] = k;
            mv[j] = v;
            if (vals2) mv2[j] = vals2[i];
            mr[j] = (d << 24) | (rank & 0xFFFFFF);
            if ((mask & lt) == 0) waveCnt[wave][d] = pre + (uint32_t)__popcll(mask);
            nit = j + 1;
        }
    }
    __syncthreads();
    for (int d = threadIdx.x; d < 256; d += blockDim.x) {
        uint32_t run = 0;
        for (int w = 0; w < WFA_THREADS / 64; ++w) {
            wavePre[w][d] = run;
            run += waveCnt[w][d];
        }
    }
    __syncthreads();
    for (int j = 0; j < nit; ++j) {
        uint32_t d = mr[j] >> 24;
        uint32_t pos = gbase[d] + wavePre[wave][d] + (mr[j] & 0xFFFFFF);
        keys_out[pos] = mk[j];
        vals_out[pos] = mv[j];
        if (vals2) vals2_out[pos] = mv2[j];
    }
}

template <bool CARRY2>
__global__ void k_rs8_scatter_lds(const uint32_t* keys, const uint32_t* vals,
                                  int64_t n, int shift, const uint32_t* hist,
                                  int64_t nblocks, const uint32_t* dbase,
                                  uint32_t* keys_out, uint32_t* vals_out,
                                  const uint32_t* vals2, uint32_t* vals2_out) {
    __shared__ uint32_t gbase[256];
    __shared__ uint32_t waveCnt[WFA_THREADS / 64][256];
    __shared__ uint32_t wavePre[WFA_THREADS / 64][256];
    __shared__ uint32_t localBase[256];
    __shared__ uint32_t sk[RS8_PER_BLOCK];
    __shared__ uint32_t sv[RS8_PER_BLOCK];
    __shared__ uint32_t sv2[CARRY2 ? RS8_PER_BLOCK : 1];
    __shared__ uint8_t sd[RS8_PER_BLOCK];
    const int wave = threadIdx.x >> 6, lane = threadIdx.x & 63;
    const uint64_t lt = ((uint64_t)1 << lane) - 1;
    for (int d = threadIdx.x; d < 256; d += blockDim.x) {
        gbase[d] = hist[(int64_t)d * nblocks + blockIdx.x] + dbase[d];
        for (int w = 0; w < WFA_THREADS / 64; ++w) waveCnt[w][d] = 0;
    }
    __syncthreads();
    int64_t blockStart = (int64_t)blockIdx.x * RS8_PER_BLOCK;
    int64_t waveBase = blockStart + wave * RS8_PER_WAVE;
    uint32_t mk[RS8_IPT], mv[RS8_IPT], mv2[RS8_IPT], mr[RS8_IPT];
    int nit = 0;
#pragma unroll
    for (int j = 0; j < RS8_IPT; ++j) {
        int64_t i = waveBase + j * 64 + lane;
        bool valid = i < n;
        uint32_t k = valid ? keys[i] : 0;
        uint32_t v = valid ? (vals ? vals[i] : (uint32_t)i) : 0;
        uint32_t d = (k >> shift) & 255;
        uint64_t mask = __ballot(valid);
#pragma unroll
        for (int bit = 0; bit < 8; ++bit) {
            uint64_t b = __ballot((d >> bit) & 1);
            mask &= ((d >> bit) & 1) ? b : ~b;
        }
        if (valid) {
            uint32_t pre = waveCnt[wave][d];
            uint32_t rank = pre + (uint32_t)__popcll(mask & lt);
            mk[j] = k;
            mv[j] = v;
            if (CARRY2) mv2[j] = vals2[i];
            mr[j] = (d << 24) | (rank & 0xFFFFFF);
            if ((mask & lt) == 0) waveCnt[wave][d] = pre + (uint32_t)__popcll(mask);
            nit = j + 1;
        }
    }
    __syncthreads();
    __shared__ uint32_t blockCnt[256];
    for (int d = threadIdx.x; d < 256; d += blockDim.x) {
        uint32_t run = 0;
        for (int w = 0; w < WFA_THREADS / 64; ++w) {
            wavePre[w][d] = run;
            run += waveCnt[w][d];
        }
        blockCnt[d] = run;
    }
    __syncthreads();
    if (threadIdx.x < 256) {
        __shared__ uint32_t tot[256];
        uint32_t c = blockCnt[threadIdx.x];
        tot[threadIdx.x] = c;
        __syncthreads();
        for (int off = 1; off < 256; off <<= 1) {
            uint32_t t = (threadIdx.x >= off) ? tot[threadIdx.x - off] : 0;
            __syncthreads();
            tot[threadIdx.x] += t;
            __syncthreads();
        }
        localBase[threadIdx.x] = tot[threadIdx.x] - c;
    }
    __syncthreads();
    for (int j = 0; j < nit; ++j) {
        uint32_t d = mr[j] >> 24;
        uint32_t lpos = localBase[d] + wavePre[wave][d] + (mr[j] & 0xFFFFFF);
        sk[lpos] = mk[j];
        sv[lpos] = mv[j];
        if (CARRY2) sv2[lpos] = mv2[j];
        sd[lpos] = (uint8_t)d;
    }
    __syncthreads();
    const int nblk_items = (int)min((int64_t)RS8_PER_BLOCK, n - blockStart);
    for (int p = threadIdx.x; p < nblk_items; p += blockDim.x) {
        uint32_t d = sd[p];
        uint32_t g = gbase[d] + (uint32_t)p - localBase[d];
        keys_out[g] = sk[p];
        vals_out[g] = sv[p];
        if (CARRY2) vals2_out[g] = sv2[p];
    }
}

static void sort_pairs2_impl(wfa_stream_t s, uint32_t* slot, uint32_t* idx,
                             uint32_t* slot_tmp, uint32_t* idx_tmp,
                             uint32_t* val2, uint32_t* val2_tmp,
                             uint32_t* hist, int64_t n, int bits,
                             uint32_t** out_slot, uint32_t** out_idx,
                             uint32_t** out_val2, int implicit_iota,
                             int base_shift, int skip_hist0) {
    hipStream_t st = (hipStream_t)s;
    uint32_t *ka = slot, *va = idx, *kb = slot_tmp, *vb = idx_tmp;
    uint32_t *wa = val2, *wb = val2_tmp;
    bool first = true;
    if (bits > 4) {
        int64_t nb = wfa_sort8_nblocks(n);
        uint32_t* dt = hist + 256 * nb;
        uint32_t* dbase = dt + 256;
        int passes = (bits + 7) / 8;
        for (int p = 0; p < passes; ++p) {
            int shift = base_shift + 8 * p;
            if (!(p == 0 && skip_hist0)) {
                hipLaunchKernelGGL(k_rs8_hist, dim3(nb), dim3(WFA_THREADS), 0, st,
                                   ka, n, shift, hist, nb);
            }
            sdbg(st, "hist", p);
            hipLaunchKernelGGL(k_rs8_scan, dim3(256), dim3(256), 0, st, hist, nb, dt);
            sdbg(st, "scan", p);
            hipLaunchKernelGGL(k_rs8_dbase, dim3(1), dim3(256), 0, st, dt, dbase);
            sdbg(st, "dbase", p);
            uint32_t* va_eff = (first && implicit_iota) ? nullptr : va;
            if (val2)
                hipLaunchKernelGGL(k_rs8_scatter_lds<true>, dim3(nb),
                                   dim3(WFA_THREADS), 0, st, ka, va_eff, n, shift,
                                   hist, nb, dbase, kb, vb, wa, wb);
            else
                hipLaunchKernelGGL(k_rs8_scatter_lds<false>, dim3(nb),
                                   dim3(WFA_THREADS), 0, st, ka, va_eff, n, shift,
                                   hist, nb, dbase, kb, vb, wa, wb);
            sdbg(st, "scatter", p);
            first = false;
            uint32_t* t;
            t = ka; ka = kb; kb = t;
            t = va; va = vb; vb = t;
            t = wa; wa = wb; wb = t;
        }
        *out_slot = ka;
        *out_idx = va;
        if (out_val2) *out_val2 = wa;
        return;
    }
    int64_t nblocks = wfa_sort_nblocks(n);
    uint32_t* dt = hist + 16 * nblocks;
    int passes = (bits + 3) / 4;
    (void)base_shift;
    for (int p = 0; p < passes; ++p) {
        int shift = 4 * p;
        hipLaunchKernelGGL(k_rs_hist, dim3(nblocks), dim3(WFA_THREADS), 0, st, ka, n,
                           shift, hist, nblocks);
        hipLaunchKernelGGL(k_rs_scan16, dim3(16), dim3(256), 0, st, hist, nblocks, dt);
        hipLaunchKernelGGL(k_rs_scatter, dim3(nblocks), dim3(WFA_THREADS), 0, st, ka,
                           (first && implicit_iota) ? nullptr : va, n, shift, hist,
                           nblocks, dt, kb, vb, wa, wb);
        first = false;
        uint32_t* t;
        t = ka; ka = kb; kb = t;
        t = va; va = vb; vb = t;
        t = wa; wa = wb; wb = t;
    }
    *out_slot = ka;
    *out_idx = va;
    if (out_val2) *out_val2 = wa;
}

extern "C" void wfa_sort_pairs2(wfa_stream_t s, uint32_t* slot, uint32_t* idx,
                                uint32_t* slot_tmp, uint32_t* idx_tmp,
                                uint32_t* val2, uint32_t* val2_tmp,
                                uint32_t* hist, int64_t n, int bits,
                                uint32_t** out_slot, uint32_t** out_idx,
                                uint32_t** out_val2, int implicit_iota,
                                int base_shift) {
    sort_pairs2_impl(s, slot, idx, slot_tmp, idx_tmp, val2, val2_tmp, hist, n,
                     bits, out_slot, out_idx, out_val2, implicit_iota,
                     base_shift, 0);
}

extern "C" void wfa_sort_pairs2_ph(wfa_stream_t s, uint32_t* slot, uint32_t* idx,
                                   uint32_t* slot_tmp, uint32_t* idx_tmp,
                                   uint32_t* val2, uint32_t* val2_tmp,
                                   uint32_t* hist, int64_t n, int bits,
                                   uint32_t** out_slot, uint32_t** out_idx,
                                   uint32_t** out_val2, int implicit_iota,
                                   int base_shift) {
    sort_pairs2_impl(s, slot, idx, slot_tmp, idx_tmp, val2, val2_tmp, hist, n,
                     bits, out_slot, out_idx, out_val2, implicit_iota,
                     base_shift, bits > 4 ? 1 : 0);
}

extern "C" void wfa_sort_pairs(wfa_stream_t s, uint32_t* slot, uint32_t* idx,
                               uint32_t* slot_tmp, uint32_t* idx_tmp, uint32_t* hist,
                               int64_t n, int bits, uint32_t** out_slot,
                               uint32_t** out_idx) {
    wfa_sort_pairs2(s, slot, idx, slot_tmp, idx_tmp, nullptr, nullptr, hist, n,
                    bits, out_slot, out_idx, nullptr, 0, 0);
}

__global__ void k_seg_count(const uint32_t* slot, int64_t n, uint32_t* blk_cnt,
                            int shr) {
    int64_t base = (int64_t)blockIdx.x * RS_PER_BLOCK + (int64_t)threadIdx.x * RS_IPT;
    uint32_t c = 0;
#pragma unroll
    for (int j = 0; j < RS_IPT; ++j) {
        int64_t i = base + j;
        if (i < n) c += (i == 0) || ((slot[i] >> shr) != (slot[i - 1] >> shr));
    }
    __shared__ uint32_t red[WFA_THREADS / 64];
    for (int off = 32; off; off >>= 1) c += __shfl_down(c, off, 64);
    if ((threadIdx.x & 63) == 0) red[threadIdx.x >> 6] = c;
    __syncthreads();
    if (threadIdx.x == 0) {
        uint32_t t = 0;
        for (int w = 0; w < WFA_THREADS / 64; ++w) t += red[w];
        blk_cnt[blockIdx.x] = t;
    }
}

__global__ void k_seg_scatter(const uint32_t* slot, int64_t n, const uint32_t* blk_off,
                              uint32_t* seg_start, uint32_t* seg_slot, int shr) {
    int64_t base = (int64_t)blockIdx.x * RS_PER_BLOCK + (int64_t)threadIdx.x * RS_IPT;
    uint32_t c = 0;
#pragma unroll
    for (int j = 0; j < RS_IPT; ++j) {
        int64_t i = base + j;
        if (i < n) c += (i == 0) || ((slot[i] >> shr) != (slot[i - 1] >> shr));
    }
    __shared__ uint32_t tc[WFA_THREADS];
    tc[threadIdx.x] = c;
    __syncthreads();
    for (int off = 1; off < WFA_THREADS; off <<= 1) {
        uint32_t t = (threadIdx.x >= off) ? tc[threadIdx.x - off] : 0;
        __syncthreads();
        tc[threadIdx.x] += t;
        __syncthreads();
    }
    uint32_t w = blk_off[blockIdx.x] + tc[threadIdx.x] - c;
    for (int j = 0; j < RS_IPT; ++j) {
        int64_t i = base + j;
        if (i >= n) continue;
        if ((i == 0) || ((slot[i] >> shr) != (slot[i - 1] >> shr))) {
            seg_start[w] = (uint32_t)i;
            seg_slot[w] = slot[i] >> shr;
            ++w;
        }
    }
}

__global__ void k_nseg_total(const uint32_t* slot_sorted, int64_t n,
                             const uint32_t* scan_tmp, int64_t nb, int64_t* d_nseg,
                             int shr) {
    if (blockIdx.x == 0 && threadIdx.x < 64) {
        int64_t base = (nb - 1) * (int64_t)RS_PER_BLOCK;
        uint32_t c = 0;
        for (int64_t i = base + threadIdx.x; i < n; i += 64)
            c += (i == 0) || ((slot_sorted[i] >> shr) != (slot_sorted[i - 1] >> shr));
        for (int off = 32; off; off >>= 1) c += __shfl_down(c, off, 64);
        if (threadIdx.x == 0) *d_nseg = (int64_t)scan_tmp[nb - 1] + c;
    }
}

__global__ void k_seg_by_slot(const uint32_t* slot, int64_t n, uint32_t* by_slot,
                              int shr) {
    for (int64_t i = blockIdx.x * (int64_t)blockDim.x + threadIdx.x; i < n;
         i += gridDim.x * (int64_t)blockDim.x) {
        uint32_t sl = slot[i] >> shr;
        if (i == 0 || (slot[i - 1] >> shr) != sl) by_slot[sl] = (uint32_t)i;
    }
}

#define SEGC_BLOCKS 32
__global__ void k_seg_count_dense(const uint32_t* by_slot, int64_t max_slots,
                                  uint32_t* blk_tot) {
    const int64_t per = (max_slots + SEGC_BLOCKS - 1) / SEGC_BLOCKS;
    const int64_t lo = blockIdx.x * per;
    const int64_t hi = min(lo + per, max_slots);
    uint32_t c = 0;
    for (int64_t s = lo + threadIdx.x; s < hi; s += blockDim.x)
        c += by_slot[s] != 0xFFFFFFFFu;
    __shared__ uint32_t red[WFA_THREADS / 64];
    for (int off = 32; off; off >>= 1) c += __shfl_down(c, off, 64);
    if ((threadIdx.x & 63) == 0) red[threadIdx.x >> 6] = c;
    __syncthreads();
    if (threadIdx.x == 0) {
        uint32_t t = 0;
        for (int w = 0; w < (int)blockDim.x / 64; ++w) t += red[w];
        blk_tot[blockIdx.x] = t;
    }
}

__global__ void k_seg_scan_dense(uint32_t* blk_tot, int64_t* d_nseg) {
    if (threadIdx.x == 0) {
        uint32_t acc = 0;
        for (int b = 0; b < SEGC_BLOCKS; ++b) {
            uint32_t t = blk_tot[b];
            blk_tot[b] = acc;
            acc += t;
        }
        *d_nseg = (int64_t)acc;
    }
}

__global__ void k_seg_write_dense(const uint32_t* by_slot, int64_t max_slots,
                                  const uint32_t* blk_base, uint32_t* seg_start,
                                  uint32_t* seg_slot) {
    const int64_t per = (max_slots + SEGC_BLOCKS - 1) / SEGC_BLOCKS;
    const int64_t lo = blockIdx.x * per;
    const int64_t hi = min(lo + per, max_slots);
    __shared__ uint32_t wsum[WFA_THREADS / 64 + 1];
    __shared__ uint32_t base;
    const int lane = threadIdx.x & 63;
    const int wid = threadIdx.x >> 6;
    const int nw = (int)blockDim.x / 64;
    if (threadIdx.x == 0) base = blk_base[blockIdx.x];
    __syncthreads();
    for (int64_t c = lo; c < hi; c += blockDim.x) {
        int64_t s = c + threadIdx.x;
        uint32_t v = (s < hi) ? by_slot[s] : 0xFFFFFFFFu;
        bool pred = v != 0xFFFFFFFFu;
        uint64_t m = __ballot(pred);
        uint32_t before = __popcll(m & ((1ULL << lane) - 1));
        if (lane == 0) wsum[wid] = (uint32_t)__popcll(m);
        __syncthreads();
        if (threadIdx.x == 0) {
            uint32_t acc = 0;
            for (int w = 0; w < nw; ++w) {
                uint32_t t = wsum[w];
                wsum[w] = acc;
                acc += t;
            }
            wsum[nw] = acc;
        }
        __syncthreads();
        if (pred) {
            uint32_t w = base + wsum[wid] + before;
            seg_start[w] = v;
            seg_slot[w] = (uint32_t)s;
        }
        __syncthreads();
        if (threadIdx.x == 0) base += wsum[nw];
        __syncthreads();
// ... 70 lines not shown
    }
    if (blockIdx.x == 0 && threadIdx.x == 0) *d_out_n = nseg;
}

extern "C" void wfa_segment_reduce(wfa_stream_t s, const uint32_t* seg_start,
                                   const uint32_t* seg_slot, const int64_t* d_nseg,
                                   int64_t n, const void* v_orig,
                                   const uint32_t* idx_sorted,
                                   const int64_t* ts_orig, int vdt, int comb,
                                   const uint64_t* slot_to_key, uint64_t* out_key,
                                   void* out_val, int64_t* out_ts, int64_t* d_out_n) {
    hipLaunchKernelGGL(k_seg_reduce, dim3(WFA_MAX_BLOCKS / 8), dim3(WFA_THREADS), 0,
                       (hipStream_t)s, seg_start, seg_slot, d_nseg, n, v_orig,
                       idx_sorted, ts_orig, vdt, comb, slot_to_key, out_key, out_val,
                       out_ts, d_out_n);
}

__global__ void k_seg_reduce_wave(const uint32_t* seg_start, const uint32_t* seg_slot,
                                  const int64_t* d_nseg, int64_t n,
                                  const void* v_orig, const uint32_t* idx_sorted,
                                  const int64_t* ts_orig, int vdt, int comb,
                                  int ts_last, const uint64_t* slot_to_key,
                                  uint64_t* out_key,
                                  void* out_val, int64_t* out_ts, int64_t* d_out_n) {
    const int64_t nseg = *d_nseg;
    const int lane = threadIdx.x & 63;
    const int64_t wid = ((int64_t)blockIdx.x * blockDim.x + threadIdx.x) >> 6;
    const int64_t nw = ((int64_t)gridDim.x * blockDim.x) >> 6;
    for (int64_t j = wid; j < nseg; j += nw) {
        const int64_t b = seg_start[j];
        const int64_t e = (j + 1 < nseg) ? seg_start[j + 1] : n;
        float acc = (comb == 1) ? INFINITY : (comb == 2 ? -INFINITY : 0.f);
        int64_t tmax = INT64_MIN;
        for (int64_t i = b + lane; i < e; i += 64) {
            const uint32_t r = idx_sorted[i];
            float x = wfa_val_at(v_orig, vdt, vdt >= 6 ? i : r);
            acc = (comb == 0 || comb == 3)
                      ? acc + x
                      : (comb == 1 ? fminf(acc, x) : fmaxf(acc, x));
            if (ts_orig && !ts_last) tmax = max(tmax, ts_orig[r]);
        }
        for (int o = 32; o; o >>= 1) {
            float ov = __shfl_down(acc, o, 64);
            acc = (comb == 0 || comb == 3)
                      ? acc + ov
                      : (comb == 1 ? fminf(acc, ov) : fmaxf(acc, ov));
            tmax = max(tmax, __shfl_down(tmax, o, 64));
        }
        if (lane == 0) {
            ((float*)out_val)[j] = (comb == 3) ? (float)(e - b) : acc;
            out_key[j] = slot_to_key ? slot_to_key[seg_slot[j]] : (uint64_t)seg_slot[j];
            if (out_ts)
                out_ts[j] = (ts_orig && ts_last) ? ts_orig[idx_sorted[e - 1]]
                                                 : tmax;
        }
    }
    if (blockIdx.x == 0 && threadIdx.x == 0) *d_out_n = nseg;
}

extern "C" void wfa_segment_reduce_wave(
    wfa_stream_t s, const uint32_t* seg_start, const uint32_t* seg_slot,
    const int64_t* d_nseg, int64_t n, const void* v_orig, int vdt,
    const uint32_t* idx_sorted, const int64_t* ts_orig, int comb, int ts_last,
    const uint64_t* slot_to_key, uint64_t* out_key, void* out_val,
    int64_t* out_ts, int64_t* d_out_n) {
    hipLaunchKernelGGL(k_seg_reduce_wave, dim3(WFA_MAX_BLOCKS), dim3(WFA_THREADS), 0,
                       (hipStream_t)s, seg_start, seg_slot, d_nseg, n, v_orig,
                       idx_sorted, ts_orig, vdt, comb, ts_last, slot_to_key,
                       out_key, out_val, out_ts, d_out_n);
}


__global__ void k_fire_count(const uint32_t* seg_start, const uint32_t* seg_slot,
                             const int64_t* d_nseg, int64_t n, int64_t pane_len,
                             int64_t P, int64_t S, const uint32_t* st_fill,
                             const uint32_t* st_head, uint32_t* nf,
                             const uint32_t* idx_sorted, const int64_t* ts_orig,
                             int64_t* st_last, uint32_t* pane_nf) {
    const int64_t nseg = *d_nseg;
    for (int64_t j = blockIdx.x * (int64_t)blockDim.x + threadIdx.x; j < nseg;
         j += gridDim.x * (int64_t)blockDim.x) {
        const uint32_t slot = seg_slot[j];
        const int64_t b = seg_start[j];
        const int64_t e = (j + 1 < nseg) ? seg_start[j + 1] : n;
        const uint64_t fill = st_fill[slot];
        const uint64_t head0 = st_head[slot];
        const uint64_t ncomp = (fill + (uint64_t)(e - b)) / (uint64_t)pane_len;
        auto F = [&](uint64_t x) {
            return x < (uint64_t)P ? 0ull : (x - (uint64_t)P) / (uint64_t)S + 1ull;
        };
        nf[j] = (uint32_t)(F(head0 + ncomp) - F(head0));
        if (pane_nf) pane_nf[j] = (uint32_t)ncomp;
        if (st_last) {
            const int64_t t = ts_orig[idx_sorted[e - 1]];
            if (t > st_last[slot]) st_last[slot] = t;
        }
    }
}

__global__ void k_fire_scan(uint32_t* nf, const int64_t* d_nseg, int64_t* d_out_n) {
    const int64_t m = *d_nseg;
    __shared__ uint32_t tot[1024];
    const int64_t chunk = (m + 1023) / 1024;
    const int64_t b0 = (int64_t)threadIdx.x * chunk;
    const int64_t b1 = min(m, b0 + chunk);
    uint32_t s = 0;
    for (int64_t i = b0; i < b1; ++i) s += nf[i];
    tot[threadIdx.x] = s;
    __syncthreads();
    for (int off = 1; off < 1024; off <<= 1) {
        uint32_t t = (threadIdx.x >= off) ? tot[threadIdx.x - off] : 0;
        __syncthreads();
        tot[threadIdx.x] += t;
        __syncthreads();
    }
    uint32_t run = tot[threadIdx.x] - s;
    for (int64_t i = b0; i < b1; ++i) {
        uint32_t v = nf[i];
        nf[i] = run;
        run += v;
    }
    if (threadIdx.x == 1023 && d_out_n) *d_out_n = tot[1023];
}

extern "C" void wfa_ffat_fire_offsets(wfa_stream_t s, const uint32_t* seg_start,
                                      const uint32_t* seg_slot, const int64_t* d_nseg,
                                      int64_t n, int64_t pane_len, int64_t P,
                                      int64_t S, const uint32_t* st_fill,
                                      const uint32_t* st_head, uint32_t* nf,
                                      int64_t* d_out_n, const uint32_t* idx_sorted,
                                      const int64_t* ts_orig, int64_t* st_last) {
    hipStream_t st = (hipStream_t)s;
    hipLaunchKernelGGL(k_fire_count, dim3(WFA_MAX_BLOCKS / 8), dim3(WFA_THREADS), 0,
                       st, seg_start, seg_slot, d_nseg, n, pane_len, P, S, st_fill,
                       st_head, nf, idx_sorted, ts_orig, st_last,
                       (uint32_t*)nullptr);
    hipLaunchKernelGGL(k_fire_scan, dim3(1), dim3(1024), 0, st, nf, d_nseg, d_out_n);
}

extern "C" void wfa_ffat_fire_offsets_pw(
    wfa_stream_t s, const uint32_t* seg_start, const uint32_t* seg_slot,
    const int64_t* d_nseg, int64_t n, int64_t pane_len, int64_t P, int64_t S,
    const uint32_t* st_fill, const uint32_t* st_head, uint32_t* nf,
    int64_t* d_out_n, const uint32_t* idx_sorted, const int64_t* ts_orig,
    int64_t* st_last, uint32_t* pane_base, int64_t* d_total_panes) {
    hipStream_t st = (hipStream_t)s;
    hipLaunchKernelGGL(k_fire_count, dim3(WFA_MAX_BLOCKS / 8), dim3(WFA_THREADS),
                       0, st, seg_start, seg_slot, d_nseg, n, pane_len, P, S,
                       st_fill, st_head, nf, idx_sorted, ts_orig, st_last,
                       pane_base);
    hipLaunchKernelGGL(k_fire_scan, dim3(1), dim3(1024), 0, st, nf, d_nseg, d_out_n);
    hipLaunchKernelGGL(k_fire_scan, dim3(1), dim3(1024), 0, st, pane_base, d_nseg,
                       d_total_panes);
}

__global__ void k_ffat_cb(const uint32_t* seg_start, const uint32_t* seg_slot,
                          const int64_t* d_nseg, int64_t n, const void* v_f32,
                          int vdt, const uint32_t* idx_sorted, const int64_t* ts_orig,
                          int64_t pane_len, int64_t P,
                          int64_t S, int comb, int ring_log2, int64_t* st_count,
                          uint32_t* st_fill, float* st_acc, float* ring,
                          uint32_t* st_head, float* st_wsum,
                          const uint64_t* slot_to_key, const uint32_t* fire_base,
                          uint64_t* out_key,
                          float* out_val, int64_t* out_ts,
                          int64_t out_cap) {
    const int64_t nseg = *d_nseg;
    const uint32_t R = 1u << ring_log2;
    const uint32_t Rm = R - 1;
    const float ident = (comb == 1) ? INFINITY : (comb == 2 ? -INFINITY : 0.f);
    for (int64_t j = blockIdx.x * (int64_t)blockDim.x + threadIdx.x; j < nseg;
         j += gridDim.x * (int64_t)blockDim.x) {
        const uint32_t slot = seg_slot[j];
        int64_t i = seg_start[j];
        const int64_t e = (j + 1 < nseg) ? seg_start[j + 1] : n;
        uint32_t fill = st_fill[slot];
        float acc = st_acc[slot];
        uint32_t head = st_head[slot];
        float wsum = st_wsum[slot];
        int64_t w = fire_base[j];
        float* rg = ring + (size_t)slot * R;
        for (; i < e; ++i) {
            float x = (comb == 3) ? 1.0f
                                  : wfa_val_at(v_f32, vdt, vdt == 6 ? i : idx_sorted[i]);
            acc = (comb == 1) ? fminf(acc, x)
                              : (comb == 2 ? fmaxf(acc, x) : acc + x);
            if (++fill == (uint32_t)pane_len) {
                if (comb == 0 || comb == 3) {
                    wsum += acc;
                    if (head >= (uint32_t)P) wsum -= rg[(head - (uint32_t)P) & Rm];
                }
                rg[head & Rm] = acc;
                acc = ident;
                fill = 0;
                ++head;
                if (head >= (uint32_t)P && ((head - (uint32_t)P) % (uint32_t)S) == 0) {
                    float res;
                    if (comb == 0 || comb == 3) {
                        res = wsum;
                    } else {
                        res = rg[(head - 1) & Rm];
                        for (uint32_t q = 2; q <= (uint32_t)P; ++q) {
                            float pv = rg[(head - q) & Rm];
                            res = (comb == 1) ? fminf(res, pv) : fmaxf(res, pv);
                        }
                    }
                    if (w < out_cap) {
                        out_key[w] = slot_to_key[slot];
                        out_val[w] = res;
                        out_ts[w] = ts_orig ? ts_orig[idx_sorted[i]] : 0;
                    }
                    ++w;
                }
            }
        }
        st_fill[slot] = fill;
        st_acc[slot] = acc;
        st_head[slot] = head;
        st_wsum[slot] = wsum;
        st_count[slot] += e - seg_start[j];
    }
}

__global__ void k_ffat_cb_wave(const uint32_t* seg_start, const uint32_t* seg_slot,
                               const int64_t* d_nseg, int64_t n,
                               const void* v_f32, int vdt,
                               const uint32_t* idx_sorted,
                               const int64_t* ts_orig,
                               int64_t pane_len, int64_t P, int64_t S, int comb,
                               int ring_log2, int64_t* st_count, uint32_t* st_fill,
                               float* st_acc, float* ring, uint32_t* st_head,
                               float* st_wsum, const uint64_t* slot_to_key,
                               const uint32_t* fire_base,
                               uint64_t* out_key, float* out_val, int64_t* out_ts,
                               int64_t out_cap) {
    const int64_t nseg = *d_nseg;
    const uint32_t R = 1u << ring_log2;
    const uint32_t Rm = R - 1;
    const float ident = (comb == 1) ? INFINITY : (comb == 2 ? -INFINITY : 0.f);
    const int lane = threadIdx.x & 63;
    const int64_t wid = ((int64_t)blockIdx.x * blockDim.x + threadIdx.x) >> 6;
    const int64_t nw = ((int64_t)gridDim.x * blockDim.x) >> 6;
    const uint32_t L = (uint32_t)pane_len;
#define WCOMB(a, b) ((comb == 1) ? fminf(a, b) : (comb == 2 ? fmaxf(a, b) : (a) + (b)))
    for (int64_t j = wid; j < nseg; j += nw) {
        const uint32_t slot = seg_slot[j];
        const int64_t i0 = seg_start[j];
        const int64_t e = (j + 1 < nseg) ? seg_start[j + 1] : n;
        uint32_t fill = st_fill[slot];
        float acc = st_acc[slot];
        uint32_t head = st_head[slot];
        float wsum = st_wsum[slot];
        int64_t w = fire_base[j];
        float* rg = ring + (size_t)slot * R;
        for (int64_t pos = i0; pos < e; pos += 64) {
            const uint32_t nchunk = (uint32_t)min((int64_t)64, e - pos);
            float v = (lane < (int)nchunk)
                          ? ((comb == 3)
                                 ? 1.0f
                                 : wfa_val_at(v_f32, vdt,
                                              vdt == 6 ? pos + lane
                                                       : idx_sorted[pos + lane]))
                          : ident;
            uint32_t rel = (lane < (int)nchunk) ? (fill + (uint32_t)lane) / L : ~0u;
            const uint32_t maxrel = (fill + nchunk - 1) / L;
            const uint32_t ncomplete = (fill + nchunk) / L;
            for (uint32_t r = 0; r <= maxrel; ++r) {
                float pv = (rel == r) ? v : ident;
                for (int o = 32; o; o >>= 1) pv = WCOMB(pv, __shfl_xor(pv, o, 64));
                acc = WCOMB(acc, pv);
                if (r < ncomplete) {
                    if (lane == 0) rg[head & Rm] = acc;
                    if (comb == 0 || comb == 3) {
                        wsum += acc;
                        if (head >= (uint32_t)P) wsum -= rg[(head - (uint32_t)P) & Rm];
                    }
                    ++head;
                    const float closed = acc;
                    acc = ident;
                    if (head >= (uint32_t)P &&
                        ((head - (uint32_t)P) % (uint32_t)S) == 0) {
                        float res;
                        if (comb == 0 || comb == 3) {
                            res = wsum;
                        } else {
                            float part = ident;
                            for (uint32_t q = lane; q < (uint32_t)P; q += 64) {
                                float x = (q == 0) ? closed : rg[(head - 1 - q) & Rm];
                                part = WCOMB(part, x);
                            }
                            for (int o = 32; o; o >>= 1)
                                part = WCOMB(part, __shfl_xor(part, o, 64));
                            res = part;
                        }
                        if (lane == 0 && w < out_cap) {
                            out_key[w] = slot_to_key[slot];
                            out_val[w] = res;
                            int64_t last = pos + (int64_t)((r + 1) * L - fill) - 1;
                            out_ts[w] = ts_orig ? ts_orig[idx_sorted[last]] : 0;
                        }
                        ++w;
                    }
                }
            }
            fill = fill + nchunk - ncomplete * L;
        }
// ... 1584 lines not shown
```

csrc/hip/wfa_kernels.h:

```cpp
#pragma once
#include <cstdint>

typedef void* wfa_stream_t;

extern "C" {

void wfa_gen_batch(wfa_stream_t s, int64_t* ts, uint64_t* key, void* val, int vdt,
                   int64_t n, int64_t start, uint64_t seed, uint64_t n_keys);

void wfa_map_apply(wfa_stream_t s, int spec, void* col, int dt, int64_t n,
                   double a, double b);

void wfa_filter_flags(wfa_stream_t s, int spec, const void* col, int dt, int64_t n,
                      double a, double b, uint32_t* flags);

void wfa_compact(wfa_stream_t s, int64_t n, const uint32_t* flags,
                 uint32_t* scan_tmp,
                 const int64_t* ts_in, int64_t* ts_out,
                 const uint64_t* key_in, uint64_t* key_out,
                 const void* const* cols_in, void* const* cols_out,
                 const int* col_esize, int n_cols, int64_t* d_count);

void wfa_key_to_slot_v(wfa_stream_t s, const uint64_t* key, int64_t n,
                       uint64_t* table_packed, uint32_t* n_slots,
                       int64_t table_cap, uint32_t* slot_out,
                       uint64_t* slot_to_key, const uint16_t* val);
void wfa_key_to_slot(wfa_stream_t s, const uint64_t* key, int64_t n,
                     uint64_t* table_packed, uint32_t* n_slots,
                     int64_t table_cap, uint32_t* slot_out,
                     uint64_t* slot_to_key);
void wfa_key_dense(wfa_stream_t s, const uint64_t* key, int64_t n,
                   int64_t max_keys, uint32_t* slot_out, uint32_t* n_slots,
                   uint32_t* overflow, const uint16_t* val);
void wfa_key_to_slot_h(wfa_stream_t s, const uint64_t* key, int64_t n,
                       uint64_t* table_packed, uint32_t* n_slots,
                       int64_t table_cap, uint32_t* slot_out,
                       uint64_t* slot_to_key, const uint16_t* val,
                       uint32_t* hist, int shift);
void wfa_key_dense_h(wfa_stream_t s, const uint64_t* key, int64_t n,
                     int64_t max_keys, uint32_t* slot_out, uint32_t* n_slots,
                     uint32_t* overflow, const uint16_t* val, uint32_t* hist,
                     int shift);
void wfa_iota_u64(wfa_stream_t s, uint64_t* p, int64_t n);
void wfa_bucket_by_key_h(wfa_stream_t s, const uint64_t* key, int64_t n,
                         int world, uint32_t* dest, uint32_t* hist);

void wfa_sort_pairs(wfa_stream_t s, uint32_t* slot, uint32_t* idx,
                    uint32_t* slot_tmp, uint32_t* idx_tmp, uint32_t* hist,
                    int64_t n, int bits,
                    uint32_t** out_slot, uint32_t** out_idx);
void wfa_sort_pairs2(wfa_stream_t s, uint32_t* slot, uint32_t* idx,
                     uint32_t* slot_tmp, uint32_t* idx_tmp,
                     uint32_t* val2, uint32_t* val2_tmp, uint32_t* hist,
                     int64_t n, int bits, uint32_t** out_slot,
                     uint32_t** out_idx, uint32_t** out_val2,
                     int implicit_iota, int base_shift);
void wfa_sort_pairs2_ph(wfa_stream_t s, uint32_t* slot, uint32_t* idx,
                        uint32_t* slot_tmp, uint32_t* idx_tmp,
                        uint32_t* val2, uint32_t* val2_tmp, uint32_t* hist,
                        int64_t n, int bits, uint32_t** out_slot,
                        uint32_t** out_idx, uint32_t** out_val2,
                        int implicit_iota, int base_shift);
int64_t wfa_sort_nblocks(int64_t n);
int64_t wfa_sort_hist_u32(int64_t cap);

void wfa_gather(wfa_stream_t s, const uint32_t* idx, int64_t n,
                const void* v_in, void* v_out, int esize,
                const int64_t* ts_in, int64_t* ts_out);

void wfa_segments(wfa_stream_t s, const uint32_t* slot_sorted, int64_t n,
                  uint32_t* scan_tmp, uint32_t* seg_start, uint32_t* seg_slot,
                  int64_t* d_nseg, int shr);
void wfa_segments_dense(wfa_stream_t s, const uint32_t* slot_sorted, int64_t n,
                        uint32_t* by_slot, int64_t max_slots,
                        uint32_t* scratch32, uint32_t* seg_start,
                        uint32_t* seg_slot, int64_t* d_nseg, int shr);

void wfa_segment_reduce(wfa_stream_t s, const uint32_t* seg_start,
                        const uint32_t* seg_slot, const int64_t* d_nseg, int64_t n,
                        const void* v_orig, const uint32_t* idx_sorted,
                        const int64_t* ts_orig, int vdt,
                        int comb, const uint64_t* slot_to_key,
                        uint64_t* out_key, void* out_val, int64_t* out_ts,
                        int64_t* d_out_n);
void wfa_segment_reduce_wave(
    wfa_stream_t s, const uint32_t* seg_start, const uint32_t* seg_slot,
    const int64_t* d_nseg, int64_t n, const void* v_orig, int vdt,
    const uint32_t* idx_sorted, const int64_t* ts_orig, int comb, int ts_last,
    const uint64_t* slot_to_key, uint64_t* out_key, void* out_val,
    int64_t* out_ts, int64_t* d_out_n);

void wfa_ffat_fire_offsets(wfa_stream_t s, const uint32_t* seg_start,
                           const uint32_t* seg_slot, const int64_t* d_nseg,
                           int64_t n, int64_t pane_len, int64_t P, int64_t S,
                           const uint32_t* st_fill, const uint32_t* st_head,
                           uint32_t* nf, int64_t* d_out_n,
                           const uint32_t* idx_sorted, const int64_t* ts_orig,
                           int64_t* st_last);

void wfa_ffat_fire_offsets_pw(
    wfa_stream_t s, const uint32_t* seg_start, const uint32_t* seg_slot,
    const int64_t* d_nseg, int64_t n, int64_t pane_len, int64_t P, int64_t S,
    const uint32_t* st_fill, const uint32_t* st_head, uint32_t* nf,
    int64_t* d_out_n, const uint32_t* idx_sorted, const int64_t* ts_orig,
    int64_t* st_last, uint32_t* pane_base, int64_t* d_total_panes);
void wfa_ffat_cb_fold_pw(
    wfa_stream_t s, const uint32_t* seg_start, const uint32_t* seg_slot,
    const int64_t* d_nseg, const int64_t* d_total_panes, int64_t n,
    const void* v_f32, int vdt, const uint32_t* idx_sorted,
    const int64_t* ts_orig, int64_t pane_len, int64_t P, int64_t S, int comb,
    int ring_log2, int64_t* st_count, uint32_t* st_fill, float* st_acc,
    float* st_acc_new, float* ring, uint32_t* st_head, float* st_wsum,
    const uint64_t* slot_to_key, const uint32_t* fire_base,
    const uint32_t* pane_base, float* temp, uint64_t* out_key, float* out_val,
    int64_t* out_ts, int64_t out_cap);

enum {
    WFA_CB_FOLD_WAVE = 0,
    WFA_CB_FOLD_TILE = 1,
    WFA_CB_FOLD_TILE512 = 2,
    WFA_CB_FOLD_TILE2048 = 3,
};
void wfa_ffat_cb_fold(wfa_stream_t s, const uint32_t* seg_start,
                      const uint32_t* seg_slot, const int64_t* d_nseg, int64_t n,
                      const void* v_f32, int vdt, const uint32_t* idx_sorted,
                      const int64_t* ts_orig,
                      int64_t pane_len, int64_t P, int64_t S, int comb,
                      int ring_log2,
                      int64_t* st_count, uint32_t* st_fill, float* st_acc,
                      float* ring, uint32_t* st_head, float* st_wsum,
                      const uint64_t* slot_to_key, const uint32_t* fire_base,
                      uint64_t* out_key, float* out_val, int64_t* out_ts,
                      int64_t out_cap, int variant);

void wfa_ffat_cb_fold_fused(
    wfa_stream_t s, const uint32_t* seg_start, const uint32_t* seg_slot,
    const int64_t* d_nseg, int64_t n, const void* v_f32, int vdt,
    const uint32_t* idx_sorted, const int64_t* ts_orig, int64_t pane_len,
    int64_t P, int64_t S, int comb, int ring_log2, int64_t* st_count,
    uint32_t* st_fill, float* st_acc, float* ring, uint32_t* st_head,
    float* st_wsum, const uint64_t* slot_to_key, const uint32_t* fire_base,
    uint64_t* out_key, float* out_val, int64_t* out_ts, int64_t out_cap);

void wfa_gram_prep(wfa_stream_t s, const float* const* colp,
                   const uint32_t* idx_sorted, int64_t n,
                   uint32_t* inv_scratch, float* staged);
void wfa_gram_fold(wfa_stream_t s, const uint32_t* seg_start,
                   const uint32_t* seg_slot, const int64_t* d_nseg,
                   int64_t n, const float* const* colp,
                   const uint32_t* idx_sorted, const int64_t* ts_orig,
                   int64_t win, uint32_t* st_fill, float* st_acc,
                   uint32_t* st_head, const uint64_t* slot_to_key,
                   const uint32_t* fire_base, uint64_t* out_key,
                   int64_t* out_gwid, float* const* out_colp,
                   int64_t* out_ts, int64_t out_cap, int64_t* d_out_n, uint32_t* inv_scratch,
                   float* staged);

void wfa_stateful_apply(wfa_stream_t s, const uint32_t* seg_start,
                        const uint32_t* seg_slot, const int64_t* d_nseg,
                        int64_t n, const uint32_t* idx_sorted, void* col,
                        int dt, int spec, int is_filter, double a, double b,
                        double* state, uint32_t* flags);

void wfa_tb_lift_only(wfa_stream_t s, const uint32_t* seg_start,
                      const uint32_t* seg_slot, const int64_t* d_nseg,
                      int64_t n, const void* v_f32, int vdt,
                      const uint32_t* idx_sorted, const int64_t* ts_orig,
                      int64_t pane_len, int64_t P, int64_t S, int comb,
                      int pend_log2, float* pend, int64_t* pend_base,
                      int64_t* last_pane, uint32_t* ignored,
                      uint32_t* overflow, int ts_mono);
void wfa_tb_countscan_only(wfa_stream_t s, const uint32_t* n_slots,
                           int64_t limit_pane, int64_t* pend_base,
                           int64_t* last_pane, uint32_t* st_head, int64_t P,
                           int64_t S, uint32_t* nf, int64_t* d_out_n);
void wfa_tb_advance_only(wfa_stream_t s, const uint32_t* n_slots,
                         int64_t limit_pane, int64_t pane_len, int64_t P,
                         int64_t S, int comb, int ring_log2, int pend_log2,
                         float* pend, int64_t* pend_base, int64_t* last_pane,
                         uint32_t* st_head, float* st_wsum, float* ring,
                         const uint64_t* slot_to_key, uint32_t* nf,
                         uint64_t* out_key, float* out_val, int64_t* out_ts,
                         int64_t out_cap);
void wfa_ffat_tb_round(
    wfa_stream_t s, const uint32_t* seg_start, const uint32_t* seg_slot,
    const int64_t* d_nseg, int64_t n, const void* v_f32, int vdt,
    const uint32_t* idx_sorted, const int64_t* ts_orig, int64_t pane_len,
    int64_t P, int64_t S, int comb, int ring_log2, int pend_log2,
    int64_t limit_pane, float* pend, int64_t* pend_base, int64_t* last_pane,
    uint32_t* st_head, float* st_wsum, float* ring, const uint32_t* n_slots,
    const uint64_t* slot_to_key, uint32_t* nf, uint32_t* ignored,
    uint32_t* overflow, uint64_t* out_key, float* out_val, int64_t* out_ts,
    int64_t out_cap, int64_t* d_out_n, int ts_mono, uint32_t* span_nf,
                       int64_t* pfirst, int64_t* d_total_spans);

void wfa_ffat_tree_fold(wfa_stream_t s, const uint32_t* seg_start,
                        const uint32_t* seg_slot, const int64_t* d_nseg, int64_t n,
                        const void* v_f32, int vdt, const uint32_t* idx_sorted,
                        const int64_t* ts_orig,
                        int64_t pane_len, int64_t P, int64_t S, int comb,
                        int ring_log2,
                        int64_t* st_count, uint32_t* st_fill, float* st_acc,
                        float* tree, uint32_t* st_head,
                        const uint64_t* slot_to_key, const uint32_t* fire_base,
                        uint64_t* out_key, float* out_val, int64_t* out_ts,
                        int64_t out_cap);

void wfa_seg_last_ts(wfa_stream_t s, const uint32_t* seg_start,
                     const uint32_t* seg_slot, const int64_t* d_nseg, int64_t n,
                     const uint32_t* idx_sorted, const int64_t* ts_orig,
                     int64_t* st_last);

void wfa_ffat_cb_flush_fire(wfa_stream_t s, const uint32_t* n_slots, int64_t P,
                            int64_t S, int comb, int ring_log2,
                            const uint32_t* st_fill, const float* st_acc,
                            const float* cells, int64_t slot_stride,
                            int64_t cell_off, const uint32_t* st_head,
                            const int64_t* st_last,
                            const uint64_t* slot_to_key, const uint32_t* nf,
                            int64_t out_base, uint64_t* out_key,
                            float* out_val, int64_t* out_ts, int64_t out_cap);

void wfa_slot_scan(wfa_stream_t s, uint32_t* nf, const uint32_t* n_slots,
                   int64_t* d_out_n);

void wfa_cb_flush_count(wfa_stream_t s, const uint32_t* n_slots, int64_t P,
                        int64_t S, const uint32_t* st_fill,
                        const uint32_t* st_head, uint32_t* nf);
void wfa_tb_count(wfa_stream_t s, const uint32_t* n_slots, int64_t limit_pane,
// ... 34 lines not shown
```

Before: 31.88 billion tuples/s.

## Derive keyed segments from radix-sort histograms and fuse with fire offsets

Adds a histogram-based segment builder. It reuses per-digit counts produced by the radix sort (wfa_sort_pairs2_cnt) to compute per-slot counts, so segment starts no longer need a scan over the sorted slot array. In the count-based FFAT path the segment construction is fused with fire-offset computation, replacing the separate dense-segments and fire-offsets kernels with two slot-sized kernels. This adds a persistent count table, an env switch (WFA_SEGS) and debug entry points, at the cost of more complex sort bookkeeping.

```diff
diff --git a/csrc/engine/bindings.cpp b/csrc/engine/bindings.cpp
--- a/csrc/engine/bindings.cpp
+++ b/csrc/engine/bindings.cpp
@@ -615,16 +615,45 @@
           });
     m.def("debug_ffat_stage_times",
           [](int64_t n, int64_t n_keys, int64_t win, int64_t slide, int iters,
-             int vik, const std::string& fold_variant) {
+             int vik, const std::string& fold_variant,
+             const std::string& front) {
               py::dict d;
               for (auto& [k, v] : debug_ffat_stage_times(n, n_keys, win, slide,
-                                                         iters, vik, fold_variant))
+                                                         iters, vik, fold_variant,
+                                                         front))
                   d[py::str(k)] = v;
               return d;
           },
           py::arg("n"), py::arg("n_keys"), py::arg("win") = 1000,
           py::arg("slide") = 100, py::arg("iters") = 20, py::arg("vik") = 0,
-          py::arg("fold_variant") = "");
+          py::arg("fold_variant") = "", py::arg("front") = "");
+    m.def("debug_keyed_segments",
+          [](py::array_t<uint64_t, py::array::c_style | py::array::forcecast> keys,
+             int64_t max_keys, bool dense, py::object vals,
+             const std::string& mode) {
+              const uint16_t* vp = nullptr;
+              py::array_t<uint16_t, py::array::c_style | py::array::forcecast> va;
+              if (!vals.is_none()) {
+                  va = vals.cast<py::array_t<uint16_t, py::array::c_style |
+                                                           py::array::forcecast>>();
+                  if (va.size() != keys.size())
+                      throw std::runtime_error(
+                          "debug_keyed_segments: vals and keys differ in length");
+                  vp = va.data();
+              }
+              auto r = debug_keyed_segments_host(keys.data(), keys.size(),
+                                                 max_keys, dense, vp, mode);
+              py::tuple out(4);
+              for (int k = 0; k < 4; ++k) {
+                  py::array_t<uint32_t> a((py::ssize_t)r[k].size());
+                  if (!r[k].empty())
+                      memcpy(a.mutable_data(), r[k].data(), 4 * r[k].size());
+                  out[k] = a;
+              }
+              return out;
+          },
+          py::arg("keys"), py::arg("max_keys"), py::arg("dense"),
+          py::arg("vals") = py::none(), py::arg("mode") = "hist");
     m.def("debug_tb_stage_times",
           [](int64_t n, int64_t n_keys, int iters, int mono) {
               std::map<std::string, double> m2;
diff --git a/csrc/engine/engine.hpp b/csrc/engine/engine.hpp
--- a/csrc/engine/engine.hpp
+++ b/csrc/engine/engine.hpp
@@ -419,7 +419,10 @@
                                            int64_t max_keys);
 std::vector<std::pair<std::string, double>> debug_ffat_stage_times(
     int64_t n, int64_t n_keys, int64_t win, int64_t slide, int iters, int vik,
-    const std::string& fold_variant = "");
+    const std::string& fold_variant = "", const std::string& front = "");
+std::vector<std::vector<uint32_t>> debug_keyed_segments_host(
+    const uint64_t* keys, int64_t n, int64_t max_keys, bool dense,
+    const uint16_t* vals, const std::string& mode);
 std::vector<std::pair<std::string, double>> debug_gram_stage_times(
     int64_t n, int64_t n_keys, int64_t win, int iters);
 std::vector<std::pair<std::string, double>> debug_tb_stage_times(
diff --git a/csrc/engine/gpu_common.hpp b/csrc/engine/gpu_common.hpp
--- a/csrc/engine/gpu_common.hpp
+++ b/csrc/engine/gpu_common.hpp
@@ -10,6 +10,7 @@
 #include <string>
 #include <vector>
 
+#include "../hip/wfa_kernels.h"
 #include "engine.hpp"
 
 namespace wfa {
@@ -297,17 +298,31 @@
     bool dense = false;
     uint32_t* d_overflow = nullptr;
     uint32_t* by_slot = nullptr;
+    int segs_mode = -1;
+    bool hist_segs = false;
+    uint32_t* cnt_tab = nullptr;
+    wfa_slot_counts_t cnt_ready{};
+    const uint32_t* slot_sorted = nullptr;
+    int sorted_shr = 0;
 
     void alloc(int dev, int64_t cap_, int64_t mk, hipStream_t s);
     void check_dense_overflow();
-    void segs(hipStream_t s, const uint32_t* slot_sorted, int64_t n, int shr);
+    void sort(hipStream_t s, uint32_t* val2, uint32_t* val2_tmp, int64_t n,
+              int base_shift, uint32_t** os, uint32_t** oi, uint32_t** ov,
+              int skip_hist0 = 1);
+    int segs(hipStream_t s, const uint32_t* slot_sorted, int64_t n, int shr);
+    int segs_fire(hipStream_t s, int64_t n, int64_t pane_len, int64_t P,
+                  int64_t S, const uint32_t* st_fill, const uint32_t* st_head,
+                  uint32_t* nf, int64_t* d_out_n, const int64_t* ts_orig,
+                  int64_t* st_last);
 
     uint32_t* idx_sorted = nullptr;
     const void* v_as_f32 = nullptr;
     int v_dt = 2;
 
     void group(hipStream_t s, Batch* db, int vcol, RuntimeCtx& ctx,
-               bool want_vik = false, bool want_carry = false);
+               bool want_vik = false, bool want_carry = false,
+               bool defer_segs = false);
 };
 
 hipModule_t jit_module(const std::string& src, int device);
diff --git a/csrc/engine/gpu_ops.cpp b/csrc/engine/gpu_ops.cpp
--- a/csrc/engine/gpu_ops.cpp
+++ b/csrc/engine/gpu_ops.cpp
@@ -254,15 +254,65 @@
         wfa_iota_u64(s, slot_to_key, mk);
     }
     if (max_keys <= 65536) by_slot = (uint32_t*)A.get(4 * table_cap);
-}
-
-void KeyedScratch::segs(hipStream_t s, const uint32_t* slot_sorted, int64_t n,
-                        int shr) {
-    if (by_slot)
-        wfa_segments_dense(s, slot_sorted, n, by_slot, table_cap, hist,
-                           seg_start, seg_slot, d_nseg, shr);
-    else
-        wfa_segments(s, slot_sorted, n, hist, seg_start, seg_slot, d_nseg, shr);
+    if (segs_mode < 0) {
+        const char* e = getenv("WFA_SEGS");
+        if (e && *e && strcmp(e, "scan") != 0 && strcmp(e, "hist") != 0)
+            throw std::runtime_error(std::string("WFA_SEGS: unknown value '") +
+                                     e + "' (scan|hist)");
+        segs_mode = (e && strcmp(e, "scan") == 0) ? 0 : 1;
+    }
+    hist_segs = segs_mode == 1 && by_slot && bits <= 16;
+    if (hist_segs) {
+        cnt_tab = (uint32_t*)A.get(4 * WFA_CNT_TAB_U32);
+        HIPCHK(hipMemsetAsync(cnt_tab, 0, 4 * WFA_CNT_TAB_U32, s));
+    }
+}
+
+void KeyedScratch::sort(hipStream_t s, uint32_t* val2, uint32_t* val2_tmp,
+                        int64_t n, int base_shift, uint32_t** os,
+                        uint32_t** oi, uint32_t** ov, int skip_hist0) {
+    wfa_sort_pairs2_cnt(s, slot, idx, slot_t, idx_t, val2, val2_tmp, hist, n,
+                        bits, os, oi, ov, 1, base_shift,
+                        skip_hist0, hist_segs ? cnt_tab : nullptr, &cnt_ready);
+}
+
+int KeyedScratch::segs(hipStream_t s, const uint32_t* sorted, int64_t n,
+                       int shr) {
+    slot_sorted = sorted;
+    sorted_shr = shr;
+    if (cnt_ready.cnt) {
+        wfa_segments_cnt(s, &cnt_ready, d_nslots, max_keys, n, seg_start,
+                         seg_slot, d_nseg);
+        cnt_ready.cnt = nullptr;
+        return 2;
+    }
+    if (by_slot) {
+        wfa_segments_dense(s, sorted, n, by_slot, table_cap, hist, seg_start,
+                           seg_slot, d_nseg, shr);
+        return 4;
+    }
+    wfa_segments(s, sorted, n, hist, seg_start, seg_slot, d_nseg, shr);
+    return 4;
+}
+
+int KeyedScratch::segs_fire(hipStream_t s, int64_t n, int64_t pane_len,
+                            int64_t P, int64_t S, const uint32_t* st_fill,
+                            const uint32_t* st_head, uint32_t* nf,
+                            int64_t* d_out_n, const int64_t* ts_orig,
+                            int64_t* st_last) {
+    if (cnt_ready.cnt) {
+        wfa_segments_cnt_fire(s, &cnt_ready, d_nslots, max_keys, n, seg_start,
+                              seg_slot, d_nseg, pane_len, P, S, st_fill,
+                              st_head, nf, d_out_n, idx_sorted, ts_orig,
+                              st_last);
+        cnt_ready.cnt = nullptr;
+        return 2;
+    }
+    int k = segs(s, slot_sorted, n, sorted_shr);
+    wfa_ffat_fire_offsets(s, seg_start, seg_slot, d_nseg, n, pane_len, P, S,
+                          st_fill, st_head, nf, d_out_n, idx_sorted, ts_orig,
+                          st_last);
+    return k + 2;
 }
 
 void KeyedScratch::check_dense_overflow() {
@@ -276,35 +326,42 @@
 }
 
 void KeyedScratch::group(hipStream_t s, Batch* db, int vcol, RuntimeCtx& ctx,
-                         bool want_vik, bool want_carry) {
+                         bool want_vik, bool want_carry, bool defer_segs) {
         int64_t n = db->count;
         if (n > cap)
             throw std::runtime_error("batch larger than keyed scratch capacity — "
                                      "set the GPU op's out_batch >= upstream batch");
         bool vik = want_vik && vcol >= 0 && max_keys <= 65535 &&
                    (int)db->schema.payload[vcol] == 5;
+        auto finish = [&](const uint32_t* sorted, int shr, int front) {
+            int k = 0;
+            if (defer_segs) {
+                slot_sorted = sorted;
+                sorted_shr = shr;
+            } else {
+                k = segs(s, sorted, n, shr);
+            }
+            if (ctx.stats) ctx.stats->num_kernels += front + k + 3 * ((bits + 3) / 4);
+        };
         if (vik) {
             uint32_t *os, *oi;
             if (dense) {
                 wfa_key_dense_h(s, db->key, n, max_keys, slot, d_nslots,
                                 d_overflow, (const uint16_t*)db->cols[vcol],
                                 hist, 16);
-                wfa_sort_pairs2_ph(s, slot, idx, slot_t, idx_t, nullptr,
-                                   nullptr, hist, n, bits, &os, &oi, nullptr,
-                                   1, 16);
+                sort(s, nullptr, nullptr, n, 16, &os, &oi,
+                     nullptr);
             } else {
                 wfa_key_to_slot_h(s, db->key, n, tab, d_nslots, table_cap, slot,
                                   slot_to_key, (const uint16_t*)db->cols[vcol],
                                   hist, 16);
-                wfa_sort_pairs2_ph(s, slot, idx, slot_t, idx_t, nullptr,
-                                   nullptr, hist, n, bits, &os, &oi, nullptr,
-                                   1, 16);
+                sort(s, nullptr, nullptr, n, 16, &os, &oi,
+                     nullptr);
             }
             idx_sorted = oi;
             v_as_f32 = os;
             v_dt = 6;
-            segs(s, os, n, 16);
-            if (ctx.stats) ctx.stats->num_kernels += 5 + 3 * ((bits + 3) / 4);
+            finish(os, 16, 1);
             return;
         }
         if (dense)
@@ -317,20 +374,16 @@
         if (want_carry && vcol >= 0 && (int)db->schema.payload[vcol] == 2) {
             wfa_cast(s, db->cols[vcol], 2, v_f32, 2, n);
             uint32_t *os, *oi, *ov;
-            wfa_sort_pairs2_ph(s, slot, idx, slot_t, idx_t, (uint32_t*)v_f32,
-                               (uint32_t*)v_sorted, hist, n, bits, &os, &oi,
-                               &ov, 1, 0);
+            sort(s, (uint32_t*)v_f32, (uint32_t*)v_sorted, n, 0,
+                 &os, &oi, &ov);
             idx_sorted = oi;
             v_as_f32 = ov;
             v_dt = 7;
-            segs(s, os, n, 0);
-            if (ctx.stats) ctx.stats->num_kernels += 6 + 3 * ((bits + 3) / 4);
+            finish(os, 0, 2);
             return;
         }
         uint32_t *os, *oi;
-        wfa_sort_pairs2_ph(s, slot, idx, slot_t, idx_t, nullptr, nullptr,
-                           hist, n, bits, &os, &oi, nullptr,
-                           1, 0);
+        sort(s, nullptr, nullptr, n, 0, &os, &oi, nullptr);
         idx_sorted = oi;
         if (vcol >= 0) {
             int vdt = (int)db->schema.payload[vcol];
@@ -344,9 +397,8 @@
             }
         }
         dbg_sync(s, "sort");
-        segs(s, os, n, 0);
+        finish(os, 0, 1);
         dbg_sync(s, "segments");
-        if (ctx.stats) ctx.stats->num_kernels += 5 + 3 * ((bits + 3) / 4);
 }
 
 hipModule_t jit_module(const std::string& src, int device) {
@@ -863,9 +915,11 @@
     }
 
     void chain_cb(Batch* db, Batch* ob, int64_t n, RuntimeCtx& ctx) {
-        ks.group(stream, db, vcol, ctx, !use_tree);
+        const bool pw = pw_base && !use_pane2;
+        ks.group(stream, db, vcol, ctx, !use_tree,
+                 false, !pw);
         uint32_t* nf = cb_nf;
-        if (pw_base && !use_pane2) {
+        if (pw) {
             wfa_ffat_fire_offsets_pw(stream, ks.seg_start, ks.seg_slot,
                                      ks.d_nseg, n, pane_len, P, S, st_fill,
                                      st_head, nf, d_on, ks.idx_sorted, db->ts,
@@ -881,9 +935,9 @@
                                   hipMemcpyDeviceToHost, stream));
             return;
         }
-        wfa_ffat_fire_offsets(stream, ks.seg_start, ks.seg_slot, ks.d_nseg, n,
-                              pane_len, P, S, st_fill, st_head, nf, d_on,
-                              ks.idx_sorted, db->ts, st_last);
+        int k = ks.segs_fire(stream, n, pane_len, P, S, st_fill, st_head, nf,
+                             d_on, db->ts, st_last);
+        if (ctx.stats) ctx.stats->num_kernels += k + 1;
         if (use_tree)
             wfa_ffat_tree_fold(stream, ks.seg_start, ks.seg_slot, ks.d_nseg, n,
                                ks.v_as_f32, ks.v_dt, ks.idx_sorted, db->ts, pane_len, P, S,
@@ -1541,6 +1595,59 @@
     return out;
 }
 
+std::vector<std::vector<uint32_t>> debug_keyed_segments_host(
+    const uint64_t* keys, int64_t n, int64_t max_keys, bool dense,
+    const uint16_t* vals, const std::string& mode) {
+    if (mode != "scan" && mode != "hist")
+        throw std::runtime_error("debug_keyed_segments: mode must be scan|hist");
+    if (n < 1 || max_keys < 1)
+        throw std::runtime_error("debug_keyed_segments: empty batch / key space");
+    if (vals && max_keys > 65535)
+        throw std::runtime_error("debug_keyed_segments: value-in-key needs "
+                                 "max_keys <= 65535");
+    HIPCHK(hipSetDevice(0));
+    hipStream_t s = nullptr;
+    auto& A = arena(0);
+    KeyedScratch ks;
+    ks.dense = dense;
+    ks.segs_mode = mode == "hist" ? 1 : 0;
+    ks.alloc(0, n, max_keys, s);
+    uint64_t* d_key = (uint64_t*)A.get(8 * n);
+    uint16_t* d_val = vals ? (uint16_t*)A.get(2 * n) : nullptr;
+    HIPCHK(hipMemcpy(d_key, keys, 8 * n, hipMemcpyHostToDevice));
+    if (vals) HIPCHK(hipMemcpy(d_val, vals, 2 * n, hipMemcpyHostToDevice));
+    const int shr = vals ? 16 : 0;
+    if (dense)
+        wfa_key_dense_h(s, d_key, n, max_keys, ks.slot, ks.d_nslots,
+                        ks.d_overflow, d_val, ks.hist, shr);
+    else
+        wfa_key_to_slot_h(s, d_key, n, ks.tab, ks.d_nslots, ks.table_cap,
+                          ks.slot, ks.slot_to_key, d_val, ks.hist, shr);
+    uint32_t *os, *oi;
+    ks.sort(s, nullptr, nullptr, n, shr, &os, &oi, nullptr);
+    ks.segs(s, os, n, shr);
+    int64_t nseg = 0;
+    HIPCHK(hipStreamSynchronize(s));
+    HIPCHK(hipMemcpy(&nseg, ks.d_nseg, 8, hipMemcpyDeviceToHost));
+    std::vector<std::vector<uint32_t>> out(4);
+    out[0].resize(n);
+    out[1].resize(n);
+    out[2].resize(nseg);
+    out[3].resize(nseg);
+    HIPCHK(hipMemcpy(out[0].data(), os, 4 * n, hipMemcpyDeviceToHost));
+    HIPCHK(hipMemcpy(out[1].data(), oi, 4 * n, hipMemcpyDeviceToHost));
+    if (nseg) {
+        HIPCHK(hipMemcpy(out[2].data(), ks.seg_start, 4 * nseg,
+                         hipMemcpyDeviceToHost));
+        HIPCHK(hipMemcpy(out[3].data(), ks.seg_slot, 4 * nseg,
+                         hipMemcpyDeviceToHost));
+    }
+    for (auto& v : out[0]) v >>= shr;
+    A.put(d_key, 8 * n);
+    if (d_val) A.put(d_val, 2 * n);
+    return out;
+}
+
 std::shared_ptr<OpLogic> make_gpu_logic(const std::string& kind, const std::string& spec,
                                         const std::vector<double>& fp,
                                         const std::vector<int64_t>& ip, Engine* eng,
@@ -1714,7 +1821,11 @@
 
 std::vector<std::pair<std::string, double>> debug_ffat_stage_times(
     int64_t n, int64_t n_keys, int64_t win, int64_t slide, int iters, int vik,
-    const std::string& fold_variant) {
+    const std::string& fold_variant, const std::string& front) {
+    if (!front.empty() && front != "scan" && front != "hist")
+        throw std::runtime_error("debug_ffat_stage_times: unknown front '" +
+                                 front + "' (''|scan|hist)");
+    const bool prod = !front.empty();
     int variant;
     if (fold_variant.empty() || fold_variant == "tile") variant = WFA_CB_FOLD_TILE;
     else if (fold_variant == "wave") variant = WFA_CB_FOLD_WAVE;
@@ -1725,6 +1836,8 @@
     HIPCHK(hipSetDevice(0));
     hipStream_t s = nullptr;
     KeyedScratch ks;
+    ks.dense = prod;
+    ks.segs_mode = front == "hist" ? 1 : 0;
     ks.alloc(0, n, n_keys, s);
     auto& A = arena(0);
     uint64_t* d_key = (uint64_t*)A.get(8 * n);
@@ -1760,10 +1873,12 @@
     float* o_val = (float*)A.get(4 * fires_cap);
     int64_t* o_ts = (int64_t*)A.get(8 * fires_cap);
     int64_t* d_on = (int64_t*)A.get(64);
+    int64_t* st_last = prod ? (int64_t*)A.get(8 * n_keys) : nullptr;
     HIPCHK(hipMemsetAsync(st_count, 0, 8 * n_keys, s));
     HIPCHK(hipMemsetAsync(st_fill, 0, 4 * n_keys, s));
     HIPCHK(hipMemsetAsync(st_head, 0, 4 * n_keys, s));
     HIPCHK(hipMemsetAsync(st_wsum, 0, 4 * n_keys, s));
+    if (prod) HIPCHK(hipMemsetAsync(st_last, 0, 8 * n_keys, s));
     wfa_fill_f32(s, st_acc, 0.f, n_keys);
     wfa_fill_f32(s, ring, 0.f, n_keys * R);
 
@@ -1775,23 +1890,45 @@
     double acc[NS] = {0};
     for (int it = -2; it < iters; ++it) {
         HIPCHK(hipEventRecord(ev[0], s));
-        if (vik)
-            wfa_key_to_slot_v(s, d_key, n, ks.tab, ks.d_nslots, ks.table_cap,
-                              ks.slot, ks.slot_to_key, d_val);
-        else
-            wfa_key_to_slot(s, d_key, n, ks.tab, ks.d_nslots, ks.table_cap, ks.slot,
-                            ks.slot_to_key);
-        HIPCHK(hipEventRecord(ev[1], s));
         uint32_t *os_, *oi;
-        wfa_sort_pairs2(s, ks.slot, ks.idx, ks.slot_t, ks.idx_t, nullptr, nullptr,
-                        ks.hist, n, ks.bits, &os_, &oi, nullptr, 1, vik ? 16 : 0);
-        HIPCHK(hipEventRecord(ev[2], s));
-        ks.segs(s, os_, n, vik ? 16 : 0);
-        HIPCHK(hipEventRecord(ev[3], s));
-        wfa_ffat_fire_offsets(s, ks.seg_start, ks.seg_slot, ks.d_nseg, n, pane, P,
-                              S, st_fill, st_head, nf, d_on, nullptr, nullptr,
-                              nullptr);
-        HIPCHK(hipEventRecord(ev[4], s));
+        if (prod) {
+            wfa_key_dense_h(s, d_key, n, n_keys, ks.slot, ks.d_nslots,
+                            ks.d_overflow, vik ? d_val : nullptr, ks.hist,
+                            vik ? 16 : 0);
+            HIPCHK(hipEventRecord(ev[1], s));
+            ks.sort(s, nullptr, nullptr, n, vik ? 16 : 0, &os_, &oi, nullptr);
+            ks.idx_sorted = oi;
+            HIPCHK(hipEventRecord(ev[2], s));
+            if (ks.cnt_ready.cnt) {
+                ks.segs_fire(s, n, pane, P, S, st_fill, st_head, nf, d_on, d_ts,
+                             st_last);
+                HIPCHK(hipEventRecord(ev[3], s));
+            } else {
+                ks.segs(s, os_, n, vik ? 16 : 0);
+                HIPCHK(hipEventRecord(ev[3], s));
+                wfa_ffat_fire_offsets(s, ks.seg_start, ks.seg_slot, ks.d_nseg, n,
+                                      pane, P, S, st_fill, st_head, nf, d_on, oi,
+                                      d_ts, st_last);
+            }
+            HIPCHK(hipEventRecord(ev[4], s));
+        } else {
+            if (vik)
+                wfa_key_to_slot_v(s, d_key, n, ks.tab, ks.d_nslots, ks.table_cap,
+                                  ks.slot, ks.slot_to_key, d_val);
+            else
+                wfa_key_to_slot(s, d_key, n, ks.tab, ks.d_nslots, ks.table_cap, ks.slot,
+                                ks.slot_to_key);
+            HIPCHK(hipEventRecord(ev[1], s));
+            wfa_sort_pairs2(s, ks.slot, ks.idx, ks.slot_t, ks.idx_t, nullptr, nullptr,
+                            ks.hist, n, ks.bits, &os_, &oi, nullptr, 1, vik ? 16 : 0);
+            HIPCHK(hipEventRecord(ev[2], s));
+            ks.segs(s, os_, n, vik ? 16 : 0);
+            HIPCHK(hipEventRecord(ev[3], s));
+            wfa_ffat_fire_offsets(s, ks.seg_start, ks.seg_slot, ks.d_nseg, n, pane, P,
+                                  S, st_fill, st_head, nf, d_on, nullptr, nullptr,
+                                  nullptr);
+            HIPCHK(hipEventRecord(ev[4], s));
+        }
         wfa_ffat_cb_fold(s, ks.seg_start, ks.seg_slot, ks.d_nseg, n,
                          vik ? (const void*)os_ : (const void*)d_val, vik ? 6 : 5,
                          oi, d_ts, pane, P, S, 0, ring_log2, st_count, st_fill,
@@ -1986,9 +2123,14 @@
 std::vector<uint32_t> debug_key_slots_host(const uint64_t*, int64_t, int64_t) {
     throw std::runtime_error("built without HIP");
 }
+std::vector<std::vector<uint32_t>> debug_keyed_segments_host(
+    const uint64_t*, int64_t, int64_t, bool, const uint16_t*, const std::string&) {
+    throw std::runtime_error("built without HIP");
+}
 std::vector<std::pair<std::string, double>> debug_ffat_stage_times(int64_t, int64_t,
                                                                    int64_t, int64_t,
                                                                    int, int,
+                                                                   const std::string&,
                                                                    const std::string&) {
     throw std::runtime_error("built without HIP");
 }
diff --git a/csrc/hip/sortwin.hip b/csrc/hip/sortwin.hip
--- a/csrc/hip/sortwin.hip
+++ b/csrc/hip/sortwin.hip
@@ -495,12 +495,24 @@
     return (n + RS8_PER_BLOCK - 1) / RS8_PER_BLOCK;
 }
 
+template <bool CNT>
 __global__ void k_rs8_hist(const uint32_t* keys, int64_t n, int shift,
-                           uint32_t* hist, int64_t nblocks) {
+                           uint32_t* hist, int64_t nblocks, uint32_t* rem) {
     __shared__ uint32_t h[WFA_THREADS / 64][256];
+    __shared__ uint32_t hrun[WFA_THREADS / 64][CNT ? 256 : 1];
     const int wave = threadIdx.x >> 6, lane = threadIdx.x & 63;
+    const int lsh = shift - 8;
+    bool blk_uniform = true;
+    if (CNT) {
+        const int64_t b0 = (int64_t)blockIdx.x * RS8_PER_BLOCK;
+        const int64_t b1 = min(n, b0 + (int64_t)RS8_PER_BLOCK) - 1;
+        blk_uniform = ((keys[b0] >> lsh) & 255) == ((keys[b1] >> lsh) & 255);
+    }
     for (int d = threadIdx.x; d < 256; d += blockDim.x)
-        for (int w = 0; w < WFA_THREADS / 64; ++w) h[w][d] = 0;
+        for (int w = 0; w < WFA_THREADS / 64; ++w) {
+            h[w][d] = 0;
+            if (CNT) hrun[w][d] = 0;
+        }
     __syncthreads();
     int64_t waveBase = (int64_t)blockIdx.x * RS8_PER_BLOCK + wave * RS8_PER_WAVE;
 #pragma unroll
@@ -514,6 +526,55 @@
         for (int w = 0; w < WFA_THREADS / 64; ++w) t += h[w][d];
         hist[(int64_t)d * nblocks + blockIdx.x] = t;
     }
+    if (!CNT || blk_uniform) return;
+    if (waveBase >= n) return;
+    const int64_t w1 = min(n, waveBase + (int64_t)RS8_PER_WAVE) - 1;
+    const uint32_t wlo = (keys[waveBase] >> lsh) & 255;
+    if (wlo == ((keys[w1] >> lsh) & 255)) {
+        for (int d = lane; d < 256; d += 64) {
+            const uint32_t t = h[wave][d];
+            if (t) atomicAdd(&rem[(wlo << 8) | d], t);
+        }
+        return;
+    }
+    uint32_t kk[RS8_IPT];
+#pragma unroll
+    for (int j = 0; j < RS8_IPT; ++j) {
+        const int64_t i = waveBase + j * 64 + lane;
+        kk[j] = i < n ? keys[i] : 0;
+    }
+    uint32_t* run = hrun[wave];
+    uint32_t cur = wlo;
+    bool pending = false;
+    auto flush = [&]() {
+        for (int d = lane; d < 256; d += 64) {
+            const uint32_t t = run[d];
+            if (t) {
+                atomicAdd(&rem[(cur << 8) | d], t);
+                run[d] = 0;
+            }
+        }
+        pending = false;
+    };
+#pragma unroll
+    for (int j = 0; j < RS8_IPT; ++j) {
+        const int64_t i = waveBase + j * 64 + lane;
+        const bool valid = i < n;
+        if (__ballot(valid) == 0) break;
+        const uint32_t k = kk[j];
+        const uint32_t lo = (k >> lsh) & 255, d = (k >> shift) & 255;
+        const uint32_t lo0 = (uint32_t)__builtin_amdgcn_readfirstlane((int)lo);
+        if (__ballot(valid && lo != lo0) == 0) {
+            if (pending && lo0 != cur) flush();
+            cur = lo0;
+            if (valid) atomicAdd(&run[d], 1u);
+            pending = true;
+        } else {
+            if (pending) flush();
+            if (valid) atomicAdd(&rem[(lo << 8) | d], 1u);
+        }
+    }
+    if (pending) flush();
 }
 
 __global__ void k_rs8_scan(uint32_t* hist, int64_t nblocks, uint32_t* dt) {
@@ -714,8 +775,11 @@
                              uint32_t* hist, int64_t n, int bits,
                              uint32_t** out_slot, uint32_t** out_idx,
                              uint32_t** out_val2, int implicit_iota,
-                             int base_shift, int skip_hist0) {
+                             int base_shift, int skip_hist0,
+                             uint32_t* cnt_tab = nullptr,
+                             wfa_slot_counts_t* out_cnt = nullptr) {
     hipStream_t st = (hipStream_t)s;
+    if (out_cnt) *out_cnt = wfa_slot_counts_t{};
     uint32_t *ka = slot, *va = idx, *kb = slot_tmp, *vb = idx_tmp;
     uint32_t *wa = val2, *wb = val2_tmp;
     bool first = true;
@@ -724,11 +788,18 @@
         uint32_t* dt = hist + 256 * nb;
         uint32_t* dbase = dt + 256;
         int passes = (bits + 7) / 8;
+        const bool take_cnt = cnt_tab && out_cnt && passes <= 2;
+        uint32_t* low_base = take_cnt ? cnt_tab + WFA_CNT_REM : nullptr;
         for (int p = 0; p < passes; ++p) {
             int shift = base_shift + 8 * p;
-            if (!(p == 0 && skip_hist0)) {
-                hipLaunchKernelGGL(k_rs8_hist, dim3(nb), dim3(WFA_THREADS), 0, st,
-                                   ka, n, shift, hist, nb);
+            dbase = (take_cnt && passes == 2 && p == 0) ? low_base : dt + 256;
+            if (p == 1 && take_cnt) {
+                hipLaunchKernelGGL(k_rs8_hist<true>, dim3(nb), dim3(WFA_THREADS),
+                                   0, st, ka, n, shift, hist, nb, cnt_tab);
+            } else if (!(p == 0 && skip_hist0)) {
+                hipLaunchKernelGGL(k_rs8_hist<false>, dim3(nb), dim3(WFA_THREADS),
+                                   0, st, ka, n, shift, hist, nb,
+                                   (uint32_t*)nullptr);
             }
             sdbg(st, "hist", p);
             hipLaunchKernelGGL(k_rs8_scan, dim3(256), dim3(256), 0, st, hist, nb, dt);
@@ -754,6 +825,17 @@
         *out_slot = ka;
         *out_idx = va;
         if (out_val2) *out_val2 = wa;
+        if (take_cnt) {
+            out_cnt->cnt = passes == 1 ? dt : cnt_tab;
+            out_cnt->cap = passes == 1 ? 256 : WFA_CNT_REM;
+            if (passes == 2) {
+                out_cnt->hist = hist;
+                out_cnt->dt = dt;
+                out_cnt->low_base = low_base;
+                out_cnt->nb = nb;
+            }
+            out_cnt->work = cnt_tab + WFA_CNT_WORK;
+        }
         return;
     }
     int64_t nblocks = wfa_sort_nblocks(n);
@@ -801,6 +883,21 @@
     sort_pairs2_impl(s, slot, idx, slot_tmp, idx_tmp, val2, val2_tmp, hist, n,
                      bits, out_slot, out_idx, out_val2, implicit_iota,
                      base_shift, bits > 4 ? 1 : 0);
+}
+
+extern "C" void wfa_sort_pairs2_cnt(wfa_stream_t s, uint32_t* slot, uint32_t* idx,
+                                    uint32_t* slot_tmp, uint32_t* idx_tmp,
+                                    uint32_t* val2, uint32_t* val2_tmp,
+                                    uint32_t* hist, int64_t n, int bits,
+                                    uint32_t** out_slot, uint32_t** out_idx,
+                                    uint32_t** out_val2, int implicit_iota,
+                                    int base_shift, int skip_hist0,
+                                    uint32_t* cnt_tab,
+                                    wfa_slot_counts_t* out_cnt) {
+    sort_pairs2_impl(s, slot, idx, slot_tmp, idx_tmp, val2, val2_tmp, hist, n,
+                     bits, out_slot, out_idx, out_val2, implicit_iota,
+                     base_shift, (skip_hist0 && bits > 4) ? 1 : 0, cnt_tab,
+                     out_cnt);
 }
 
 extern "C" void wfa_sort_pairs(wfa_stream_t s, uint32_t* slot, uint32_t* idx,
@@ -1177,6 +1274,221 @@
     hipLaunchKernelGGL(k_fire_scan, dim3(1), dim3(1024), 0, st, nf, d_nseg, d_out_n);
     hipLaunchKernelGGL(k_fire_scan, dim3(1), dim3(1024), 0, st, pane_base, d_nseg,
                        d_total_panes);
+}
+
+#define SEGH_THREADS 256
+#define SEGH_SPB 512
+
+__device__ __forceinline__ uint32_t wfa_fire_nf(uint64_t fill, uint64_t head0,
+                                                uint64_t cnt, uint64_t pane_len,
+                                                uint64_t P, uint64_t S) {
+    if (((fill + cnt) | (head0 + (fill + cnt)) | pane_len | P | S) >> 32 == 0) {
+        const uint32_t p32 = (uint32_t)P, s32 = (uint32_t)S;
+        const uint32_t ncomp = (uint32_t)(fill + cnt) / (uint32_t)pane_len;
+        auto F = [&](uint32_t x) { return x < p32 ? 0u : (x - p32) / s32 + 1u; };
+        return F((uint32_t)head0 + ncomp) - F((uint32_t)head0);
+    }
+    const uint64_t ncomp = (fill + cnt) / pane_len;
+    auto F = [&](uint64_t x) { return x < P ? 0ull : (x - P) / S + 1ull; };
+    return (uint32_t)(F(head0 + ncomp) - F(head0));
+}
+
+template <int NV>
+__device__ __forceinline__ void wfa_block_sum(uint32_t* v, uint32_t (*red)[SEGH_THREADS / 64]) {
+    const int lane = threadIdx.x & 63, wid = threadIdx.x >> 6;
+#pragma unroll
+    for (int k = 0; k < NV; ++k) {
+        for (int o = 32; o; o >>= 1) v[k] += __shfl_down(v[k], o, 64);
+        if (lane == 0) red[k][wid] = v[k];
+    }
+    __syncthreads();
+    if (threadIdx.x == 0) {
+#pragma unroll
+        for (int k = 0; k < NV; ++k) {
+            v[k] = 0;
+            for (int w = 0; w < SEGH_THREADS / 64; ++w) v[k] += red[k][w];
+        }
+    }
+}
+
+template <bool FIRE>
+__global__ void __launch_bounds__(SEGH_THREADS)
+k_slot_counts(wfa_slot_counts_t sc, const uint32_t* __restrict__ d_nslots,
+              int64_t n, int64_t pane_len, int64_t P, int64_t S,
+              const uint32_t* __restrict__ st_fill,
+              const uint32_t* __restrict__ st_head) {
+    constexpr int NV = FIRE ? 3 : 2, PT = SEGH_SPB / SEGH_THREADS;
+    __shared__ uint32_t red[NV][SEGH_THREADS / 64];
+    const uint32_t L = min(*d_nslots, (uint32_t)sc.cap);
+    uint32_t* slot_c = sc.work + WFA_CNT_WORK_C;
+    uint32_t* slot_f = sc.work + WFA_CNT_WORK_F;
+    uint32_t v[3] = {0, 0, 0};
+#pragma unroll
+    for (int i = 0; i < PT; ++i) {
+        const uint32_t sl = blockIdx.x * SEGH_SPB + i * SEGH_THREADS + threadIdx.x;
+        if (sl >= L) continue;
+        uint32_t c;
+        if (!sc.hist) {
+            c = sc.cnt[sl];
+        } else {
+            const uint32_t l = sl & 255, d = sl >> 8;
+            uint32_t* rem = &sc.cnt[(l << 8) | d];
+            c = *rem;
+            if (c) *rem = 0;
+            const int64_t ls = sc.low_base[l];
+            const int64_t le = l < 255 ? (int64_t)sc.low_base[l + 1] : n;
+            const int64_t bs = (ls + RS8_PER_BLOCK - 1) / RS8_PER_BLOCK;
+            const int64_t be = le == n ? sc.nb : le / RS8_PER_BLOCK;
+            if (be > bs) {
+                const uint32_t* row = sc.hist + (int64_t)d * sc.nb;
+                c += (be < sc.nb ? row[be] : sc.dt[d]) - row[bs];
+            }
+        }
+        slot_c[sl] = c;
+        v[0] += c != 0;
+        v[1] += c;
+        if (FIRE) {
+            const uint32_t f =
+                c ? wfa_fire_nf(st_fill[sl], st_head[sl], c, (uint64_t)pane_len,
+                                (uint64_t)P, (uint64_t)S)
+                  : 0;
+            slot_f[sl] = f;
+            v[2] += f;
+        }
+    }
+    wfa_block_sum<NV>(v, red);
+    if (threadIdx.x == 0) {
+#pragma unroll
+        for (int k = 0; k < NV; ++k)
+            sc.work[WFA_CNT_WORK_TOT + blockIdx.x * 3 + k] = v[k];
+    }
+}
+
+template <bool FIRE>
+__global__ void __launch_bounds__(SEGH_THREADS)
+k_seg_from_cnt(const uint32_t* __restrict__ work,
+               const uint32_t* __restrict__ d_nslots, uint32_t cap,
+               uint32_t* __restrict__ seg_start, uint32_t* __restrict__ seg_slot,
+               int64_t* __restrict__ d_nseg, uint32_t* __restrict__ nf,
+               int64_t* __restrict__ d_out_n,
+               const uint32_t* __restrict__ idx_sorted,
+               const int64_t* __restrict__ ts_orig,
+               int64_t* __restrict__ st_last) {
+    constexpr int NV = FIRE ? 3 : 2, NW = SEGH_THREADS / 64;
+    constexpr int PT = SEGH_SPB / SEGH_THREADS;
+    __shared__ uint32_t base[NV], total[NV], wtot[NV][NW];
+    const int lane = threadIdx.x & 63, wid = threadIdx.x >> 6;
+    const uint32_t L = min(*d_nslots, cap);
+    const uint32_t* slot_c = work + WFA_CNT_WORK_C;
+    const uint32_t* slot_f = work + WFA_CNT_WORK_F;
+    const uint32_t s0 = blockIdx.x * SEGH_SPB + threadIdx.x * PT;
+    uint32_t c[PT], f[PT], v[3] = {0, 0, 0};
+#pragma unroll
+    for (int i = 0; i < PT; ++i) {
+        const bool ok = s0 + i < L;
+        c[i] = ok ? slot_c[s0 + i] : 0;
+        f[i] = (FIRE && ok) ? slot_f[s0 + i] : 0;
+        v[0] += c[i] != 0;
+        v[1] += c[i];
+        v[2] += f[i];
+    }
+    if (wid == 0) {
+#pragma unroll
+        for (int k = 0; k < NV; ++k) {
+            uint32_t before = 0, all = 0;
+            for (uint32_t b = lane; b < gridDim.x; b += 64) {
+                const uint32_t t = work[WFA_CNT_WORK_TOT + b * 3 + k];
+                if (b < blockIdx.x) before += t;
+                all += t;
+            }
+            for (int o = 32; o; o >>= 1) {
+                before += __shfl_down(before, o, 64);
+                all += __shfl_down(all, o, 64);
+            }
+            if (lane == 0) {
+                base[k] = before;
+                total[k] = all;
+            }
+        }
+    }
+    uint32_t ex[3] = {0, 0, 0};
+#pragma unroll
+    for (int k = 0; k < NV; ++k) {
+        uint32_t x = v[k];
+        for (int o = 1; o < 64; o <<= 1) {
+            const uint32_t t = __shfl_up(x, o, 64);
+            if (lane >= o) x += t;
+        }
+        ex[k] = x - v[k];
+        if (lane == 63) wtot[k][wid] = x;
+    }
+    __syncthreads();
+#pragma unroll
+    for (int k = 0; k < NV; ++k) {
+        ex[k] += base[k];
+        for (int w = 0; w < wid; ++w) ex[k] += wtot[k][w];
+    }
+    uint32_t j = ex[0], start = ex[1], fo = ex[2];
+#pragma unroll
+    for (int i = 0; i < PT; ++i) {
+        if (!c[i]) continue;
+        const uint32_t sl = s0 + i;
+        seg_slot[j] = sl;
+        seg_start[j] = start;
+        if (FIRE) {
+            nf[j] = fo;
+            fo += f[i];
+            if (st_last) {
+                const int64_t t = ts_orig[idx_sorted[start + c[i] - 1]];
+                if (t > st_last[sl]) st_last[sl] = t;
+            }
+        }
+        ++j;
+        start += c[i];
+    }
+    if (blockIdx.x == 0 && threadIdx.x == 0) {
+        *d_nseg = (int64_t)total[0];
+        if (FIRE && d_out_n) *d_out_n = (int64_t)total[NV - 1];
+    }
+}
+
+static inline int segh_blocks(const wfa_slot_counts_t* sc, int64_t max_slots) {
+    int64_t m = max_slots < sc->cap ? max_slots : sc->cap;
+    int64_t b = (m + SEGH_SPB - 1) / SEGH_SPB;
+    return (int)(b < 1 ? 1 : b);
+}
+
+extern "C" void wfa_segments_cnt(wfa_stream_t s, const wfa_slot_counts_t* sc,
+                                 const uint32_t* d_nslots, int64_t max_slots,
+                                 int64_t n, uint32_t* seg_start,
+                                 uint32_t* seg_slot, int64_t* d_nseg) {
+    hipStream_t st = (hipStream_t)s;
+    const int nb = segh_blocks(sc, max_slots);
+    hipLaunchKernelGGL(k_slot_counts<false>, dim3(nb), dim3(SEGH_THREADS), 0, st,
+                       *sc, d_nslots, n, (int64_t)1, (int64_t)1, (int64_t)1,
+                       (const uint32_t*)nullptr, (const uint32_t*)nullptr);
+    hipLaunchKernelGGL(k_seg_from_cnt<false>, dim3(nb), dim3(SEGH_THREADS), 0, st,
+                       (const uint32_t*)sc->work, d_nslots, (uint32_t)sc->cap,
+                       seg_start, seg_slot, d_nseg, (uint32_t*)nullptr,
+                       (int64_t*)nullptr, (const uint32_t*)nullptr,
+                       (const int64_t*)nullptr, (int64_t*)nullptr);
+}
+
+extern "C" void wfa_segments_cnt_fire(
+    wfa_stream_t s, const wfa_slot_counts_t* sc, const uint32_t* d_nslots,
+    int64_t max_slots, int64_t n, uint32_t* seg_start, uint32_t* seg_slot,
+    int64_t* d_nseg, int64_t pane_len, int64_t P, int64_t S,
+    const uint32_t* st_fill, const uint32_t* st_head, uint32_t* nf,
+    int64_t* d_out_n, const uint32_t* idx_sorted, const int64_t* ts_orig,
+    int64_t* st_last) {
+    hipStream_t st = (hipStream_t)s;
+    const int nb = segh_blocks(sc, max_slots);
+    hipLaunchKernelGGL(k_slot_counts<true>, dim3(nb), dim3(SEGH_THREADS), 0, st,
+                       *sc, d_nslots, n, pane_len, P, S, st_fill, st_head);
+    hipLaunchKernelGGL(k_seg_from_cnt<true>, dim3(nb), dim3(SEGH_THREADS), 0, st,
+                       (const uint32_t*)sc->work, d_nslots, (uint32_t)sc->cap,
+                       seg_start, seg_slot, d_nseg, nf, d_out_n, idx_sorted,
+                       ts_orig, st_last);
 }
 
 __global__ void k_ffat_cb(const uint32_t* seg_start, const uint32_t* seg_slot,
diff --git a/csrc/hip/wfa_kernels.h b/csrc/hip/wfa_kernels.h
--- a/csrc/hip/wfa_kernels.h
+++ b/csrc/hip/wfa_kernels.h
@@ -61,6 +61,28 @@
                         int64_t n, int bits, uint32_t** out_slot,
                         uint32_t** out_idx, uint32_t** out_val2,
                         int implicit_iota, int base_shift);
+#define WFA_CNT_REM 65536
+#define WFA_CNT_WORK (WFA_CNT_REM + 256)
+#define WFA_CNT_WORK_C 0
+#define WFA_CNT_WORK_F WFA_CNT_REM
+#define WFA_CNT_WORK_TOT (2 * WFA_CNT_REM)
+#define WFA_CNT_TAB_U32 (WFA_CNT_WORK + WFA_CNT_WORK_TOT + 3 * 128)
+typedef struct {
+    uint32_t* cnt;
+    int64_t cap;
+    const uint32_t* hist;
+    const uint32_t* dt;
+    const uint32_t* low_base;
+    int64_t nb;
+    uint32_t* work;
+} wfa_slot_counts_t;
+void wfa_sort_pairs2_cnt(wfa_stream_t s, uint32_t* slot, uint32_t* idx,
+                         uint32_t* slot_tmp, uint32_t* idx_tmp,
+                         uint32_t* val2, uint32_t* val2_tmp, uint32_t* hist,
+                         int64_t n, int bits, uint32_t** out_slot,
+                         uint32_t** out_idx, uint32_t** out_val2,
+                         int implicit_iota, int base_shift, int skip_hist0,
+                         uint32_t* cnt_tab, wfa_slot_counts_t* out_cnt);
 int64_t wfa_sort_nblocks(int64_t n);
 int64_t wfa_sort_hist_u32(int64_t cap);
 
@@ -75,6 +97,17 @@
                         uint32_t* by_slot, int64_t max_slots,
                         uint32_t* scratch32, uint32_t* seg_start,
                         uint32_t* seg_slot, int64_t* d_nseg, int shr);
+
+void wfa_segments_cnt(wfa_stream_t s, const wfa_slot_counts_t* sc,
+                      const uint32_t* d_nslots, int64_t max_slots, int64_t n,
+                      uint32_t* seg_start, uint32_t* seg_slot, int64_t* d_nseg);
+void wfa_segments_cnt_fire(
+    wfa_stream_t s, const wfa_slot_counts_t* sc, const uint32_t* d_nslots,
+    int64_t max_slots, int64_t n, uint32_t* seg_start, uint32_t* seg_slot,
+    int64_t* d_nseg,
+    int64_t pane_len, int64_t P, int64_t S, const uint32_t* st_fill,
+    const uint32_t* st_head, uint32_t* nf, int64_t* d_out_n,
+    const uint32_t* idx_sorted, const int64_t* ts_orig, int64_t* st_last);
 
 void wfa_segment_reduce(wfa_stream_t s, const uint32_t* seg_start,
                         const uint32_t* seg_slot, const int64_t* d_nseg, int64_t n,
```

New measurement: 33.42 billion tuples/s (median of 6 runs). 1.05x the previous value.
